# skim0119/gym-softrobot

Measured on AMD Instinct MI355X. Metric: env_steps_per_sec, higher is better.
Workload: dtype f64

## Files before the change

### gym_softrobot_amd/_capi.py

```python
from __future__ import annotations

import ctypes as C
import os
from pathlib import Path

ABI_VERSION = 17

FEAT_GRAVITY = 1 << 0
FEAT_POINT_FORCE_NODE0_X = 1 << 1
FEAT_PENDULUM_BC = 1 << 2
FEAT_ANALYTICAL_DAMPER = 1 << 3
FEAT_FIXED_BC = 1 << 4
FEAT_TIP_FORCE = 1 << 5
FEAT_MOVING_BASE_BC = 1 << 6
FEAT_LAPLACE_FILTER = 1 << 7
FEAT_PLANE_CONTACT_ANISO = 1 << 8
FEAT_REST_KAPPA_ACTION = 1 << 9
FEAT_OCTO_HEAD = 1 << 10
FEAT_SPLINE_MUSCLE_TORQUES = 1 << 11
FEAT_SUCKER_CONSTRAINT = 1 << 12
FEAT_COOMM_MUSCLES = 1 << 13
MAX_SUCKERS = 4
MAX_MUSCLES = 4
MUSCLE_LONGITUDINAL = 0
# ... 886 lines not shown
            raise ValueError(f"{what}: {name} must hold integers, got dtype {a.dtype}")
        if a.ndim > 1:
            raise ValueError(f"{what}: {name} must be a scalar or one-dimensional, got shape {a.shape}")
        if a.size and (a.min() < -2**31 or a.max() >= 2**31):
            raise ValueError(f"{what}: {name} does not fit an int32")
        out.append(a.astype(np.int32))
    s, d = out
    if d.ndim == 0:
        d = d.reshape(1)
    if s.ndim == 0:
        s = np.full(d.shape, s, np.int32)
    if s.shape != d.shape:
        raise ValueError(f"{what}: {names[0]} has {s.size} entries, {names[1]} has {d.size}")
    return np.ascontiguousarray(s), np.ascontiguousarray(d)


_VP = C.c_void_p
_EXPORTS = {
    "softrod_abi_version": (C.c_int, []),
    "softrod_source_hash": (C.c_char_p, []),
    "softrod_action_dim": (C.c_int, [C.c_int]),
    "softrod_obs_dim": (C.c_int, [C.c_int]),
    "softrod_aux_dim": (C.c_int, [C.c_int]),
    "softrod_config_softpendulum": (C.c_int, [C.POINTER(SoftrodConfig), C.c_int]),
    "softrod_config_softpendulum3d": (C.c_int, [C.POINTER(SoftrodConfig), C.c_int]),
    "softrod_config_arm_single": (C.c_int, [C.POINTER(SoftrodConfig), C.c_int]),
    "softrod_config_octo_flat": (C.c_int, [C.POINTER(SoftrodConfig), C.c_int]),
    "softrod_config_soft_arm": (C.c_int, [C.POINTER(SoftrodConfig), C.c_int]),
    "softrod_config_arm_push": (C.c_int, [C.POINTER(SoftrodConfig), C.c_int, C.c_int]),
    "softrod_config_arm_pull_weight": (C.c_int, [C.POINTER(SoftrodConfig), C.c_int]),
    "softrod_config_muscle_octopus": (C.c_int, [C.POINTER(SoftrodConfig), C.c_int, C.c_int]),
    "softrod_set_muscle_layers": (C.c_int, [_VP, _VP, _VP]),
    "softrod_set_spline_table": (C.c_int, [_VP, _VP, _VP]),
    "softrod_config_action_dim": (C.c_int, [C.POINTER(SoftrodConfig)]),
    "softrod_config_obs_dim": (C.c_int, [C.POINTER(SoftrodConfig)]),
    "softrod_reset_octo": (C.c_int, [_VP, _VP, _VP, _VP, _VP, _VP]),
    "softrod_autoreset_enable": (C.c_int, [_VP, C.c_int]),
    "softrod_autoreset_same_step": (C.c_int, [_VP, C.c_int]),
    "softrod_final_view": (C.c_int, [_VP, C.POINTER(C.c_void_p), C.POINTER(C.c_void_p), C.POINTER(C.c_void_p)]),
    "softrod_queue_push": (C.c_int, [_VP, _VP, _VP, C.c_int, _VP]),
    "softrod_queue_push_straight": (C.c_int, [_VP, _VP, _VP, _VP, _VP, C.c_int, _VP]),
    "softrod_queue_push_octo": (C.c_int, [_VP, _VP, _VP, _VP, _VP, C.c_int, _VP]),
    "softrod_queue_status": (C.c_int, [_VP, _VP, _VP, _VP]),
    "softrod_queue_status_begin": (C.c_int, [_VP, _VP]),
    "softrod_queue_status_poll": (C.c_int, [_VP, C.c_int, _VP, _VP]),
    "softrod_queue_advance": (C.c_int, [_VP, _VP, _VP]),
    "softrod_set_action_basis": (C.c_int, [_VP, _VP]),
    "softrod_set_radius_profile": (C.c_int, [_VP, _VP]),
    "softrod_create": (C.c_int, [C.POINTER(SoftrodConfig), C.c_int, C.POINTER(C.c_void_p)]),
    "softrod_reset": (C.c_int, [_VP, _VP, _VP, _VP]),
    "softrod_reset_straight": (C.c_int, [_VP, _VP, _VP, _VP, _VP, _VP]),
    "softrod_step": (C.c_int, [_VP, _VP, _VP, _VP, _VP, _VP, _VP, _VP]),
    "softrod_step_packed": (C.c_int, [_VP, _VP, _VP, _VP, _VP]),
    "softrod_scatter_rows": (C.c_int, [_VP, _VP, _VP, C.c_int, C.c_int, C.c_int64, C.c_int64, C.c_uint32, _VP]),
    "softrod_exchange_alloc": (C.c_int, [C.c_int, C.c_uint64, C.POINTER(C.c_void_p), _VP, C.POINTER(C.c_int)]),
    "softrod_exchange_open": (C.c_int, [C.c_int, _VP, C.c_int, C.POINTER(C.c_void_p)]),
    "softrod_exchange_close": (C.c_int, [C.c_int, _VP]),
    "softrod_exchange_free": (C.c_int, [C.c_int, _VP]),
    "softrod_observe": (C.c_int, [_VP, _VP, _VP, _VP]),
    "softrod_rod_energies": (C.c_int, [_VP, _VP, _VP]),
    "softrod_ground_reaction": (C.c_int, [_VP, _VP, _VP]),
    "softrod_rod_strains": (C.c_int, [_VP, _VP, _VP]),
    "softrod_muscle_loads": (C.c_int, [_VP, _VP, _VP]),
    "softrod_joint_loads": (C.c_int, [_VP, _VP, _VP]),
    "softrod_rod_dynamics": (C.c_int, [_VP, _VP, _VP]),
    "softrod_set_env_material": (C.c_int, [_VP, _VP, _VP, _VP]),
    "softrod_set_env_contact": (C.c_int, [_VP, _VP, _VP, _VP]),
    "softrod_copy_envs": (C.c_int, [_VP, _VP, _VP, C.c_int, _VP]),
    "softrod_bank_create": (C.c_int, [_VP, C.c_int]),
    "softrod_bank_save": (C.c_int, [_VP, _VP, _VP, C.c_int, _VP]),
    "softrod_bank_load": (C.c_int, [_VP, _VP, _VP, C.c_int, _VP]),
    "softrod_bank_info": (C.c_int, [_VP, C.POINTER(C.c_int32), C.POINTER(C.c_uint64), _VP]),
    "softrod_camera_default": (C.c_int, [C.POINTER(SoftrodConfig), C.POINTER(SoftrodCamera)]),
    "softrod_camera_check": (C.c_int, [C.POINTER(SoftrodCamera)]),
    "softrod_render": (C.c_int, [_VP, C.POINTER(SoftrodCamera), _VP, _VP, _VP]),
    "softrod_rod_clearance": (C.c_int, [_VP, C.c_int, _VP, _VP]),
    "softrod_set_rod_shape": (C.c_int, [_VP, _VP, _VP, _VP, _VP, _VP, _VP]),
    "softrod_set_reset_shapes": (C.c_int, [_VP, C.c_int, _VP, _VP, _VP, _VP, C.c_uint64, _VP]),
    "softrod_apply_reset_shapes": (C.c_int, [_VP, _VP, _VP]),
    "softrod_reset_shapes_view": (C.c_int, [_VP, C.POINTER(C.c_void_p), C.POINTER(C.c_void_p)]),
    "softrod_reset_shape_index": (C.c_uint32, [C.c_uint64, C.c_uint32, C.c_uint32, C.c_uint32]),
    "softrod_substeps": (C.c_int, [_VP, _VP, C.c_int, _VP]),
    "softrod_state_view_get": (C.c_int, [_VP, C.POINTER(SoftrodStateView)]),
    "softrod_set_timing": (C.c_int, [_VP, C.c_int]),
    "softrod_kernel_times_ms": (C.c_int, [_VP, _VP, C.c_int, C.POINTER(C.c_int)]),
    "softrod_last_kernel_ms": (C.c_int, [_VP, C.POINTER(C.c_float)]),
    "softrod_kernel_tier": (C.c_char_p, [_VP]),
    "softrod_last_error": (C.c_char_p, [_VP]),
    "softrod_destroy": (C.c_int, [_VP]),
}

EXPORTED_SYMBOLS = tuple(_EXPORTS)

_lib = None


def library_path() -> Path:
    env = os.environ.get("SOFTROD_HIP_LIB")
    if env:
        return Path(env)
    return Path(__file__).resolve().parent / "csrc" / "libsoftrod_hip.so"


def load_library() -> C.CDLL:
    global _lib
    if _lib is not None:
        return _lib
    try:
        import torch
    except ImportError:
        pass
    path = library_path()
    if not path.exists():
        raise SoftrodError(
            f"{path} not found: build it with `python __graft_entry__.py build` "
            "(hipcc --offload-arch=gfx950).  There is no CPU fallback."
        )
    lib = C.CDLL(str(path))
    for name, (restype, argtypes) in _EXPORTS.items():
        fn = getattr(lib, name)
        fn.restype = restype
        fn.argtypes = argtypes
    if lib.softrod_abi_version() != ABI_VERSION:
        raise SoftrodError("libsoftrod_hip.so ABI version mismatch")
    _lib = lib
    return lib


def library_source_hash() -> str:
    return load_library().softrod_source_hash().decode()


def source_hash() -> str:
    import hashlib

    csrc = Path(__file__).resolve().parent / "csrc"
    files = sorted(csrc.glob("*.hpp"), key=lambda f: f.name) + [csrc / "softrod_capi.hip",
                                                                 csrc.parents[1] / "include" / "softrod.h"]
    h = hashlib.sha256()
    for f in files:
        h.update(f.read_bytes())
    return h.hexdigest()[:16]


def check(rc: int, handle=None) -> None:
    if rc == 0:
        return
    msg = ""
    if _lib is not None:
        raw = _lib.softrod_last_error(handle)
        msg = raw.decode() if raw else ""
    raise SoftrodError(f"softrod call failed with code {rc}: {msg}")
```

### gym_softrobot_amd/backend.py

```python
from __future__ import annotations

import ctypes as C
from typing import Dict, Optional, Tuple

import numpy as np
import torch

from . import _capi
from ._capi import LANE_STRIDE, SoftrodConfig, SoftrodStateView, check, load_library
from .diagnostics import (JointLoads, MuscleLoads, RodClearance, RodDynamics, RodStrains, joint_loads_views,
                          muscle_loads_views, rod_clearance_views, rod_dynamics_views, rod_strains_views)


class _DevArray:

    def __init__(self, ptr: int, shape, typestr: str, owner):
        self._owner = owner
        self.__cuda_array_interface__ = {
            "shape": tuple(shape),
            "typestr": typestr,
            "data": (int(ptr), False),
            "version": 2,
            "strides": None,
        }


def _set_env_table(self, name: str, width: int, values, mask) -> None:
    why = getattr(_capi, f"env_{name}_refusal")(self.cfg, tapered="radius_profile" in self._tables)
    if why is not None:
        raise NotImplementedError(why)
    v = np.ascontiguousarray(values, dtype=np.float64).reshape(self.n_envs, width)
    k = None if mask is None else np.ascontiguousarray(mask, dtype=np.uint8).reshape(self.n_envs)
    check(getattr(self._lib, f"softrod_set_env_{name}")(self._h, v.ctypes.data, None if k is None else k.ctypes.data,
                                                        self._stream()), self._h)
    cur = _env_table(self, name)
    setattr(self, f"_env_{name}", np.where(k[:, None] != 0, v, cur) if k is not None else v.copy())

def _env_table(self, name: str) -> np.ndarray:
    cur = getattr(self, f"_env_{name}", None)
    if cur is None:
        return np.tile(getattr(_capi, f"env_{name}_defaults")(self.cfg), (self.n_envs, 1))
    return cur.copy()


class HipRodBackend:

    def __init__(self, cfg: SoftrodConfig, device: int = 0):
        if not torch.cuda.is_available():
            raise _capi.SoftrodError(
                "HipRodBackend needs a ROCm device (torch.cuda.is_available() is False); "
                "the hot path has no CPU fallback"
            )
        self._lib = load_library()
        self.cfg = cfg.copy()
        self.n_envs = int(cfg.n_envs)
        self.action_dim = _capi.config_action_dim(cfg)
        self.obs_dim = _capi.config_obs_dim(cfg)
        self.is_octo = bool(cfg.features & _capi.FEAT_OCTO_HEAD) and int(cfg.env_kind) == _capi.ENV_OCTO_FLAT
        self.is_mocto = int(cfg.env_kind) in _capi.MUSCLE_OCTOPUS_ENVS
        self.aux_dim = _capi.aux_dim(cfg.env_kind)
        self.device_index = int(device)
        self.device = torch.device("cuda", self.device_index)
        self._h = C.c_void_p()
        self._tables: Dict[str, bytes] = {}
        self._readouts: Dict[str, torch.Tensor] = {}
        self._frames: Dict[tuple, torch.Tensor] = {}
        check(self._lib.softrod_create(C.byref(self.cfg), self.device_index, C.byref(self._h)))
        if self.cfg.features & _capi.FEAT_REST_KAPPA_ACTION:
            if self.is_octo:
                basis = _capi.octo_action_basis(int(cfg.n_elem), int(cfg.n_knots))
            else:
                basis = _capi.action_basis(int(cfg.n_elem), self.action_dim)
            check(self._lib.softrod_set_action_basis(self._h, basis.ctypes.data), self._h)
            self._tables["action_basis"] = basis.tobytes()
        if int(cfg.env_kind) == _capi.ENV_ARM_TWO:
            basis, _ = _capi.arm_two_activation_basis(int(cfg.n_elem), 3)
            check(self._lib.softrod_set_action_basis(self._h, basis.ctypes.data), self._h)
            self._tables["action_basis"] = basis.tobytes()
        if self.cfg.features & _capi.FEAT_SPLINE_MUSCLE_TORQUES:
            breaks, coef = _capi.spline_table(float(cfg.base_length), int(cfg.n_ctrl))
            if len(breaks) != int(cfg.n_spline_pieces) + 1:
                raise _capi.SoftrodError("n_spline_pieces does not match the interpolant")
            check(self._lib.softrod_set_spline_table(self._h, breaks.ctypes.data, coef.ctypes.data), self._h)
            self._tables["spline_table"] = breaks.tobytes() + coef.tobytes()
# ... 352 lines not shown
            z = self._frames.get(key + ("depth",))
            if z is None:
                z = self._frames[key + ("depth",)] = torch.empty((self.n_envs, h, w), dtype=torch.float32, device=self.device)
        check(self._lib.softrod_render(self._h, C.byref(camera), rgb.data_ptr(), z.data_ptr() if depth else None,
                                       self._stream()), self._h)
        return (rgb, z) if depth else rgb

    def time_limit(self) -> torch.Tensor:
        return self.state()["env_aux"][0] != 0.0

    def step_packed(self, actions, out: Optional[torch.Tensor] = None) -> torch.Tensor:
        from .distributed import packed_width

        a = self._actions(actions)
        if out is None:
            if getattr(self, "packed", None) is None:
                self.packed = torch.empty((self.n_envs, packed_width(self.obs_dim)), dtype=torch.float32,
                                          device=self.device)
            out = self.packed
        check(
            self._lib.softrod_step_packed(
                self._h, a.data_ptr(), out.data_ptr(),
                self.aux.data_ptr() if self.aux is not None else None, self._stream(),
            ),
            self._h,
        )
        return out

    def scatter_rows(self, packed: torch.Tensor, peer_ptrs, first_row: int, tag_word: int = -1, tag: int = 0) -> None:
        tab = np.ascontiguousarray(peer_ptrs, dtype=np.uint64)
        check(
            self._lib.softrod_scatter_rows(
                self._h, packed.data_ptr(), tab.ctypes.data, int(tab.size), int(packed.shape[1]), int(first_row),
                int(tag_word), int(tag) & 0xFFFFFFFF, self._stream(),
            ),
            self._h,
        )

    def exchange_alloc(self, n_words: int):
        ptr, kind = C.c_void_p(), C.c_int()
        handle = (C.c_uint8 * 64)()
        check(self._lib.softrod_exchange_alloc(self.device_index, int(n_words) * 4, C.byref(ptr), handle, C.byref(kind)))
        t = torch.as_tensor(_DevArray(ptr.value, (int(n_words),), "<f4", self), device=self.device)
        return t, int(ptr.value), bytes(handle), {1: "uncached", 2: "fine-grained"}[int(kind.value)]

    def exchange_open(self, handle: bytes, owner_device: int) -> int:
        ptr = C.c_void_p()
        buf = (C.c_uint8 * 64).from_buffer_copy(handle)
        check(self._lib.softrod_exchange_open(self.device_index, buf, int(owner_device), C.byref(ptr)))
        return int(ptr.value)

    def exchange_close(self, ptr: int) -> None:
        check(self._lib.softrod_exchange_close(self.device_index, C.c_void_p(ptr)))

    def exchange_free(self, ptr: int) -> None:
        check(self._lib.softrod_exchange_free(self.device_index, C.c_void_p(ptr)))

    def substeps(self, actions, n: int) -> None:
        a = self._actions(actions) if actions is not None else None
        check(
            self._lib.softrod_substeps(
                self._h, a.data_ptr() if a is not None else None, int(n), self._stream()
            ),
            self._h,
        )

    def set_timing(self, n_launches: int) -> None:
        check(self._lib.softrod_set_timing(self._h, int(n_launches)), self._h)

    def kernel_times_ms(self) -> np.ndarray:
        cap = 1 << 16
        out = np.zeros(cap, np.float32)
        cnt = C.c_int()
        check(self._lib.softrod_kernel_times_ms(self._h, out.ctypes.data, cap, C.byref(cnt)), self._h)
        return out[: cnt.value].copy()

    def last_kernel_ms(self) -> float:
        ms = C.c_float()
        check(self._lib.softrod_last_kernel_ms(self._h, C.byref(ms)), self._h)
        return float(ms.value)

    def prev_action_rows(self) -> torch.Tensor:
        if getattr(self, "_prev_rows", None) is None:
            self._prev_rows = self.state()["prev_action"]
            if not self.is_octo and not self.is_mocto:
                self._prev_rows = self._prev_rows[:, : self.action_dim]
        return self._prev_rows

    def state(self) -> Dict[str, torch.Tensor]:
        v = SoftrodStateView()
        check(self._lib.softrod_state_view_get(self._h, C.byref(v)), self._h)
        n, s = self.n_envs, int(v.lane_stride)

        def view(ptr, comps):
            return torch.as_tensor(_DevArray(ptr, (comps, n, s), "<f8", self), device=self.device)

        extra = {}
        ns = n * (int(self.cfg.n_arm) if self.is_mocto else 1)
        if v.env_aux:
            extra["env_aux"] = torch.as_tensor(_DevArray(v.env_aux, (8, n), "<f8", self), device=self.device)
        if v.prev_kappa:
            extra["prev_kappa"] = torch.as_tensor(
                _DevArray(v.prev_kappa, (n, int(self.cfg.n_arm) * (int(self.cfg.n_elem) - 1)), "<f4", self), device=self.device)
        if v.muscle_activation:
            extra["muscle_activation"] = torch.as_tensor(
                _DevArray(v.muscle_activation, (_capi.MAX_MUSCLES, n, s), "<f8", self), device=self.device)
        return {
            **extra,
            "sucker_index": torch.as_tensor(_DevArray(v.sucker_index, (_capi.MAX_SUCKERS, ns), "<i4", self),
                                            device=self.device),
            "position": view(v.position, 3),
            "velocity": view(v.velocity, 3),
            "director": view(v.director, 9),
            "omega": view(v.omega, 3),
            "tangents": view(v.tangents, 3),
            "time": torch.as_tensor(_DevArray(v.time, (n,), "<f8", self), device=self.device),
            "control": torch.as_tensor(_DevArray(v.control, (4, n), "<f8", self), device=self.device),
            "kappa": view(v.kappa, 3),
            "rest_kappa": view(v.rest_kappa, 3),
            "env_memory": torch.as_tensor(_DevArray(v.env_memory, (n, s), "<f8", self), device=self.device),
            "prev_action": torch.as_tensor(_DevArray(v.prev_action, (n, max(7, self.action_dim)), "<f4", self),
                                           device=self.device),
            "head": torch.as_tensor(_DevArray(v.head, (20, n), "<f8", self), device=self.device),
            "bc_targets": torch.as_tensor(_DevArray(v.bc_targets, (12, n), "<f8", self), device=self.device),
            "sucker_ratio": torch.as_tensor(_DevArray(v.sucker_ratio, (_capi.MAX_SUCKERS, ns), "<f8", self),
                                            device=self.device),
            "arm_stride": int(v.arm_stride),
        }

    _SNAPSHOT_KEYS = ("position", "velocity", "director", "omega", "tangents", "time", "control", "kappa",
                      "rest_kappa", "env_memory", "prev_action", "head", "bc_targets", "sucker_ratio", "sucker_index")

    def _snapshot_keys(self):
        return (self._SNAPSHOT_KEYS + (("muscle_activation",) if self.cfg.features & _capi.FEAT_COOMM_MUSCLES else ())
                + (("env_aux", "prev_kappa") if self.is_mocto else ()))

    def config_fingerprint(self) -> bytes:
        import hashlib

        c = self.cfg.copy()
        c.n_envs = 0
        d = hashlib.sha256()
        for k in sorted(self._tables):
            d.update(k.encode() + b"\0" + self._tables[k])
        return bytes([_capi.ABI_VERSION]) + bytes(memoryview(c).cast("B")) + d.digest()

    def snapshot(self) -> Dict[str, torch.Tensor]:
        if getattr(self, "queue_depth", 0):
            raise _capi.SoftrodError("snapshot/restore of a handle with device-side auto-reset is not supported: "
                                     "the pending-reset flags and the staged queue are not part of the state view")
        st = self.state()
        torch.cuda.synchronize(self.device)
        snap = {k: st[k].cpu().clone() for k in self._snapshot_keys()}
        if getattr(self, "_env_material", None) is not None:
            snap["env_material"] = torch.from_numpy(self._env_material.copy())
        if getattr(self, "_env_contact", None) is not None:
            snap["env_contact"] = torch.from_numpy(self._env_contact.copy())
        if self.reset_shapes_count:
            snap["reset_shape_index"] = self.reset_shape_index.cpu().clone()
            snap["reset_shape_episode"] = self.reset_shape_episode.cpu().clone()
        snap["config_fingerprint"] = torch.frombuffer(bytearray(self.config_fingerprint()), dtype=torch.uint8).clone()
        return snap

    def restore(self, snap: Dict[str, torch.Tensor]) -> None:
        if getattr(self, "queue_depth", 0):
            raise _capi.SoftrodError("snapshot/restore of a handle with device-side auto-reset is not supported: "
                                     "stale needs_reset / skip flags would reset or skip the wrong envs")
        fp = snap.get("config_fingerprint")
        if fp is None or bytes(fp.numpy().tobytes()) != self.config_fingerprint():
            raise ValueError("snapshot was taken under a different softrod_config / ABI version / table set "
                             "(dt, n_substeps, features, env_kind, material, radius profile, spline table, "
                             "action basis ...): refusing to load it")
        st = self.state()
        for k in self._snapshot_keys():
            if tuple(snap[k].shape) != tuple(st[k].shape):
                raise ValueError(f"snapshot field {k!r} has shape {tuple(snap[k].shape)}, expected {tuple(st[k].shape)}")
            st[k].copy_(snap[k].to(self.device))
        if "env_material" in snap:
            self.set_env_material(snap["env_material"].numpy())
        elif getattr(self, "_env_material", None) is not None:
            self.set_env_material(np.tile(_capi.env_material_defaults(self.cfg), (self.n_envs, 1)))
        if self.reset_shapes_count and "reset_shape_index" in snap:
            self.reset_shape_index.copy_(snap["reset_shape_index"].to(self.device))
            self.reset_shape_episode.copy_(snap["reset_shape_episode"].to(self.device))
        if "env_contact" in snap:
            self.set_env_contact(snap["env_contact"].numpy())
        elif getattr(self, "_env_contact", None) is not None:
            self.set_env_contact(np.tile(_capi.env_contact_defaults(self.cfg), (self.n_envs, 1)))
        torch.cuda.synchronize(self.device)

    def rod_snapshot(self, env_indices) -> Dict[str, np.ndarray]:
        st = self.state()
        idx = torch.as_tensor(list(env_indices), dtype=torch.long, device=self.device)
        ne = int(self.cfg.n_elem)

        def rows(name, width):
            return st[name].index_select(1, idx)[:, :, :width].permute(1, 0, 2).cpu().numpy()

        return {
            "x": rows("position", ne + 1), "v": rows("velocity", ne + 1), "w": rows("omega", ne),
            "Q": rows("director", ne).reshape(len(env_indices), 3, 3, ne),
            "time": st["time"].index_select(0, idx).cpu().numpy(),
        }

    def kernel_tier(self) -> str:
        return self._lib.softrod_kernel_tier(self._h).decode()

    def octo_state_numpy(self) -> Dict[str, np.ndarray]:
        st = self.state()
        ne, na, seg = int(self.cfg.n_elem), int(self.cfg.n_arm), int(st["arm_stride"])
        torch.cuda.synchronize(self.device)

        def arms(t, comps, width):
            a = t[:, :, : na * seg].reshape(comps, self.n_envs, na, seg)[..., :width]
            return a.permute(1, 2, 0, 3).cpu().numpy()

        hd = st["head"].cpu().numpy()
        return {
            "x": arms(st["position"], 3, ne + 1),
            "v": arms(st["velocity"], 3, ne + 1),
            "w": arms(st["omega"], 3, ne),
            "Q": arms(st["director"], 9, ne).reshape(self.n_envs, na, 3, 3, ne),
            "kappa": arms(st["kappa"], 3, ne - 1),
            "rest_kappa": arms(st["rest_kappa"], 3, ne - 1),
            "head_x": hd[0:3].T.copy(), "head_v": hd[3:6].T.copy(),
            "head_Q": hd[6:15].T.reshape(self.n_envs, 3, 3).copy(), "head_w": hd[15:18].T.copy(),
            "target": hd[18:20].T.copy(),
            "time": st["time"].cpu().numpy(),
        }

    def state_numpy(self) -> Dict[str, np.ndarray]:
        st = self.state()
        ne = int(self.cfg.n_elem)
        torch.cuda.synchronize(self.device)
        out = {
            "x": st["position"][:, :, : ne + 1].permute(1, 0, 2).cpu().numpy(),
            "v": st["velocity"][:, :, : ne + 1].permute(1, 0, 2).cpu().numpy(),
            "w": st["omega"][:, :, :ne].permute(1, 0, 2).cpu().numpy(),
            "tangents": st["tangents"][:, :, :ne].permute(1, 0, 2).cpu().numpy(),
            "time": st["time"].cpu().numpy(),
            "control": st["control"].permute(1, 0).cpu().numpy(),
            "kappa": st["kappa"][:, :, : ne - 1].permute(1, 0, 2).cpu().numpy(),
            "rest_kappa": st["rest_kappa"][:, :, : ne - 1].permute(1, 0, 2).cpu().numpy(),
        }
        q = st["director"][:, :, :ne].permute(1, 0, 2).cpu().numpy()
        out["Q"] = q.reshape(self.n_envs, 3, 3, ne)
        return out
```

### gym_softrobot_amd/csrc/softrod_capi.hip

```cpp
#include <hip/hip_runtime.h>
#include <hip/hip_ext.h>

#include <cmath>
#include <cstdio>
#include <cstdlib>
#include <cstring>
#include <new>
#include <string>
#include <vector>

#include "softrod_kernels.hpp"
#include "softrod_dynamics_readout.hpp"
#include "softrod_copy_envs.hpp"
#include "softrod_state_bank.hpp"
#include "softrod_shape.hpp"
#include "softrod_reset_shapes.hpp"

using namespace softrod;

template <class Row>
struct EnvTable {
    Row* dev = nullptr;
    Row* host = nullptr;
    hipEvent_t ev = nullptr;
// ... 17 lines not shown
    hipEvent_t ev_pairs = nullptr;
    unsigned char* twin_of(const void* base) const {
        for (const Twin& t : twins) if (t.of == base) return t.dev;
        return nullptr;
    }
    void release() {
        for (const Twin& t : twins) (void)hipFree(t.dev);
        (void)hipFree(d_pairs);
        if (h_pairs) (void)hipHostFree(h_pairs);
        if (ev_pairs) (void)hipEventDestroy(ev_pairs);
        *this = StateBank{};
    }
};

struct softrod_handle {
    softrod_config cfg;
    int device = 0;
    int epl = 1;
    int nw = 1;
    size_t init_stride = 18;
    int window_refresh = 0;
    bool window_paired = true;
    std::string tier;
    RodParams P{};
    StatePtrs S{};
    std::vector<void*> owned;
    double* d_init = nullptr;
    uint8_t* d_mask = nullptr;
    double* d_basis = nullptr;
    double* d_spline = nullptr;
    bool spline_set = false;
    RodParams* d_params = nullptr;
    StatePtrs* d_state = nullptr;
    double* d_time_tab = nullptr;
    double* d_mat = nullptr;
    double* d_render_radius = nullptr;
    double* d_mtab = nullptr;
    bool muscles_set = false;
    unsigned* d_ticket = nullptr;
    bool tapered = false;
    bool was_reset = false;
    bool basis_set = false;
    double* h_init = nullptr;
    uint8_t* h_mask = nullptr;
    std::vector<hipEvent_t> ev_start, ev_stop;
    int timed = 0;
    hipEvent_t ev_reset = nullptr;
    int q_depth = 0;
    double* d_queue = nullptr;
    double* h_queue = nullptr;
    int* d_consumed = nullptr;
    int* d_produced = nullptr;
    int* d_underflow = nullptr;
    uint8_t* d_flags = nullptr;
    int* h_produced = nullptr;
    std::vector<int> seen_consumed;
    std::vector<int2> pending;
    double* h_stage = nullptr;
    int2* h_where = nullptr;
    double* d_stage = nullptr;
    int2* d_where = nullptr;
    size_t stage_cap = 0;
    int* h_status = nullptr;
    hipEvent_t ev_status = nullptr;
    bool status_pending = false;
    hipEvent_t ev_queue = nullptr;
    bool same_step = false;
    float* d_final_obs = nullptr;
    double* d_final_time = nullptr;
    double* d_final_aux = nullptr;
    int rs_count = 0;
    unsigned long long rs_seed = 0;
    double* d_rs_field[4] = {nullptr, nullptr, nullptr, nullptr};
    int* d_rs_index = nullptr;
    int* d_rs_episode = nullptr;
    uint8_t* d_rs_picked = nullptr;
    EnvTable<EnvMaterial> env_mat;
    EnvTable<EnvContact> env_contact;
    int2* d_pairs = nullptr;
    int2* h_pairs = nullptr;
    hipEvent_t ev_pairs = nullptr;
    std::vector<uint8_t> is_dst;
    StateBank bank;
    std::string err;
};

namespace {

thread_local std::string g_err;

int fail(softrod_handle* h, int code, const std::string& msg) {
    if (h) h->err = msg; else g_err = msg;
    return code;
}

struct DeviceGuard {
    int prev = -1, want = -1;
    hipError_t err = hipSuccess;
    explicit DeviceGuard(int device) : want(device) {
        err = hipGetDevice(&prev);
        if (err == hipSuccess && prev != want) err = hipSetDevice(want);
    }
    ~DeviceGuard() {
        if (prev >= 0 && prev != want) (void)hipSetDevice(prev);
    }
    DeviceGuard(const DeviceGuard&) = delete;
    DeviceGuard& operator=(const DeviceGuard&) = delete;
};
#define SR_ON_DEVICE(h)                                                                  \
    DeviceGuard guard_((h)->device);                                                     \
    if (guard_.err != hipSuccess)                                                        \
        return fail(h, SOFTROD_EHIP, std::string("hipSetDevice: ") + hipGetErrorString(guard_.err))

#define SR_HIP(h, call)                                                                 \
    do {                                                                                \
        hipError_t e_ = (call);                                                         \
        if (e_ != hipSuccess)                                                           \
            return fail(h, SOFTROD_EHIP, std::string(#call) + ": " + hipGetErrorString(e_)); \
    } while (0)

void fill_params(const softrod_config& c, RodParams& P) {
    std::memset(&P, 0, sizeof(P));
    P.n_envs = c.n_envs;
    P.n_elem = c.n_elem;
    P.time_two_half_adds = c.time_two_half_adds;
    P.features = c.features;
    P.env_kind = c.env_kind;
    P.filter_order = c.filter_order;
    P.damp_before_constrain = c.damp_before_constrain;
    P.dt = c.dt;
    P.half_dt = 0.5 * c.dt;
    P.final_time = c.final_time;
    const int n = c.n_elem;
    const double rest_len = c.base_length / (double)n;
    P.rest_len = rest_len;
    P.inv_rest_len = 1.0 / rest_len;
    P.rest_vor = 0.5 * (rest_len + rest_len);
    P.inv_rest_vor = 1.0 / P.rest_vor;
    const double r = c.base_radius;
    const double A0 = M_PI * r * r;
    const double I1 = A0 * A0 / (4.0 * M_PI);
    const double I[3] = {I1, I1, 2.0 * I1};
    for (int i = 0; i < 3; ++i) {
        P.J[i] = I[i] * (c.density * rest_len);
        P.invJ[i] = 1.0 / P.J[i];
    }
    P.shear[0] = c.alpha_c * c.shear_modulus * A0;
    P.shear[1] = c.alpha_c * c.shear_modulus * A0;
    P.shear[2] = c.youngs_modulus * A0;
    P.bend[0] = c.youngs_modulus * I[0];
    P.bend[1] = c.youngs_modulus * I[1];
    P.bend[2] = c.shear_modulus * I[2];
    const double volume = M_PI * (r * r) * rest_len;
    P.mass_node = c.density * volume;
    for (int i = 0; i < 3; ++i) { P.gravity[i] = c.gravity[i]; P.tip_force[i] = c.tip_force[i]; }
    const double ddt = c.damper_time_step > 0.0 ? c.damper_time_step : c.dt;
    P.damp_t = std::exp(-c.damping_constant * ddt);
    const double me = P.mass_node;
    for (int i = 0; i < 3; ++i) {
        P.damp_logr[i] = c.damper_protocol == 1 ? -c.damping_constant * ddt : -c.damping_constant * ddt * me * P.invJ[i];
        P.damp_r[i] = std::exp(P.damp_logr[i]);
    }
    P.eps_length = c.eps_length;
    P.eps_rot_axis = c.eps_rot_axis;
    P.acos_shift = c.acos_shift;
    P.eps_sin = c.eps_sin;
// ... 36 lines not shown
        P.n_action = c.n_knots;
        if (c.env_kind == SOFTROD_ENV_ARM_PULL_WEIGHT) P.seg_shift = 6, P.seg = 64;
        P.head_fixed = c.head_fixed;
        const double hl = c.head_length > 0.0 ? c.head_length : 2.0 * c.base_radius, hr = c.head_radius;
        for (int i = 0; i < 3; ++i) P.head_center[i] = c.head_length > 0.0 ? c.head_center[i] : 0.0;
        P.joint_angle0 = c.head_length > 0.0 ? c.joint_angle0 : 0.0;
        P.joint_angle_step = c.head_length > 0.0 ? c.joint_angle_step : 360 / (double)c.n_arm;
        const double harea = M_PI * hr * hr;
        P.head_mass = (M_PI * hr * hr * hl) * c.head_density;
        const double s1 = harea * harea / (4.0 * M_PI);
        const double smoa[3] = {s1, s1, 2.0 * s1};
        for (int i = 0; i < 3; ++i) {
            P.head_invJ[i] = 1.0 / (smoa[i] * c.head_density * hl);
        }
        P.head_radius = hr;
        P.joint_k = c.joint_k;
        P.joint_nu = c.joint_nu;
        P.joint_kt = c.joint_kt;
    }
    P.n_ctrl = c.n_ctrl;
    P.n_pieces = c.n_spline_pieces;
    P.muscle_scale = c.muscle_torque_scale;
    P.max_rate = c.max_activation_rate;
    P.base_length = c.base_length;
    for (int i = 0; i < 3; ++i) P.arm_target[i] = c.arm_target[i];
    P.n_suckers = c.n_suckers;
    for (int j = 0; j < SOFTROD_MAX_SUCKERS; ++j) P.sucker_index[j] = c.sucker_index[j];
    if (c.early_termination) P.features |= kFeatEarlyTerm;
    P.sucker_ratio0 = c.sucker_reduction_ratio;
    P.n_muscles = (c.features & SOFTROD_FEAT_COOMM_MUSCLES) ? c.n_muscles : 0;
    for (int m = 0; m < SOFTROD_MAX_MUSCLES; ++m) P.muscle_kind[m] = c.muscle_kind[m];
    P.fl_degree = c.muscle_fl_degree;
    for (int k = 0; k < SOFTROD_MAX_FL_COEF; ++k) P.fl_coef[k] = c.muscle_fl_coef[k];
    P.muscle_form = c.muscle_equiv_load_form;
    P.muscle_cur_radius = c.muscle_position_current_radius;
    P.muscle_tm_law = c.muscle_tm_length_law;
    P.push_mode = c.arm_push_mode;
}

bool is_octo(const softrod_handle* h) { return (h->cfg.features & SOFTROD_FEAT_OCTO_HEAD) != 0; }
bool is_flat(const softrod_handle* h) { return h->cfg.env_kind == SOFTROD_ENV_OCTO_FLAT; }
bool is_pull(const softrod_handle* h) { return h->cfg.env_kind == SOFTROD_ENV_ARM_PULL_WEIGHT; }
bool mocto_kind(int e) { return e == SOFTROD_ENV_CRAWL || e == SOFTROD_ENV_ARM_TWO || e == SOFTROD_ENV_REACH; }
bool is_mocto(const softrod_handle* h) { return mocto_kind(h->cfg.env_kind); }
bool restarts_as_body(const softrod_handle* h) { return is_octo(h); }
bool observes_as_body(const softrod_handle* h) { return is_mocto(h) || (is_octo(h) && !is_pull(h)); }
template <class K> K by_epl(const softrod_handle* h, K one, K two) { return h->epl == 2 ? two : one; }
template <class T>
hipError_t alloc_owned(softrod_handle* h, T*& p, size_t bytes) {
    const hipError_t e = hipMalloc((void**)&p, bytes);
    if (e != hipSuccess) { p = nullptr; return e; }
    h->owned.push_back(p);
    return hipMemset(p, 0, bytes);
}
struct RodLayout { int rods, lane_stride, arm_stride; };
RodLayout rod_layout(const softrod_handle* h) {
    const bool arms = is_flat(h) || is_mocto(h);
    return {arms ? h->cfg.n_arm : 1, kLanes * h->epl * h->nw, arms ? h->P.seg : 0};
}
void env_material_row(const softrod_config& c, const double m[4], EnvMaterial& R) {
    softrod_config ci = c;
    ci.youngs_modulus = m[0];
    ci.shear_modulus = m[1];
    ci.density = m[2];
    ci.damping_constant = m[3];
    RodParams Q;
    fill_params(ci, Q);
    std::memset(&R, 0, sizeof(R));
    for (int i = 0; i < 3; ++i) {
        R.J[i] = Q.J[i]; R.invJ[i] = Q.invJ[i]; R.shear[i] = Q.shear[i]; R.bend[i] = Q.bend[i];
        R.damp_r[i] = Q.damp_r[i]; R.damp_logr[i] = Q.damp_logr[i];
    }
    R.mass_node = Q.mass_node; R.mass_total = Q.mass_total; R.damp_t = Q.damp_t;
}
void env_contact_row(const double c[8], EnvContact& R) {
    std::memset(&R, 0, sizeof(R));
    R.k = c[0];
    R.nu = c[1];
    for (int i = 0; i < 3; ++i) { R.kin_mu[i] = c[2 + i]; R.stat_mu[i] = c[5 + i]; }
    R.kin_am[0] = 0.5 * (R.kin_mu[0] + R.kin_mu[1]); R.kin_am[1] = 0.5 * (R.kin_mu[0] - R.kin_mu[1]);
    R.stat_am[0] = 0.5 * (R.stat_mu[0] + R.stat_mu[1]); R.stat_am[1] = 0.5 * (R.stat_mu[0] - R.stat_mu[1]);
}

int launch_autoreset(softrod_handle* h, float* obs, double* reward, uint8_t* term, uint8_t* trunc, double* aux, int pack,
                     hipStream_t st) {
    const dim3 grid((unsigned)h->cfg.n_envs), block(kLanes * h->nw);
    if (restarts_as_body(h))
        hipLaunchKernelGGL(softrod_octo_autoreset_kernel, grid, block, 0, st, h->P, h->S, obs, reward, term, trunc, pack);
    else
        hipLaunchKernelGGL(by_epl(h, softrod_autoreset_kernel<1>, softrod_autoreset_kernel<2>), grid, block, 0, st, h->P, h->S,
                           obs, reward, term, trunc, aux, pack);
    SR_HIP(h, hipGetLastError());
    return SOFTROD_OK;
}

int launch_autoreset_same_step(softrod_handle* h, float* obs, double* aux, int pack, hipStream_t st) {
    const dim3 grid((unsigned)h->cfg.n_envs), block(kLanes * h->nw);
    if (restarts_as_body(h))
        hipLaunchKernelGGL(softrod_octo_autoreset_same_step_kernel, grid, block, 0, st, h->P, h->S, obs, pack, h->d_final_obs,
                           h->d_final_time);
    else
        hipLaunchKernelGGL(by_epl(h, softrod_autoreset_same_step_kernel<1>, softrod_autoreset_same_step_kernel<2>), grid, block,
                           0, st, h->P, h->S, obs, aux, pack, h->d_final_obs, h->d_final_time, h->d_final_aux);
    SR_HIP(h, hipGetLastError());
    return SOFTROD_OK;
}

int launch_reset_shapes(softrod_handle* h, int mode, const uint8_t* mask, float* obs, const uint8_t* term, const uint8_t* trunc,
                        double* aux, int pack, hipStream_t st) {
    const int N = h->cfg.n_envs;
    ResetShapesPick pick{};
    pick.index = h->d_rs_index; pick.episode = h->d_rs_episode; pick.picked = h->d_rs_picked;
    pick.seed = h->rs_seed; pick.count = h->rs_count; pick.mode = mode; pick.mask = mask;
    pick.terminated = pack ? nullptr : term; pick.truncated = pack ? nullptr : trunc;
    pick.packed = (mode == kPickFinished && pack) ? obs : nullptr;
    pick.od = softrod_config_obs_dim(&h->cfg);
    hipLaunchKernelGGL(softrod_reset_shapes_pick_kernel, dim3((unsigned)((N + kPickThreads - 1) / kPickThreads)), dim3(kPickThreads),
                       0, st, h->P, h->S, pick);
    const RodLayout y = rod_layout(h);
    const RodShapeArgs args{h->d_rs_field[0], h->d_rs_field[1], h->d_rs_field[2], h->d_rs_field[3], h->d_rs_picked, h->d_rs_index};
    hipLaunchKernelGGL(by_epl(h, softrod_rod_shape_kernel<1>, softrod_rod_shape_kernel<2>), dim3((unsigned)(N * y.rods)),
                       dim3(kLanes), 0, st, h->P, h->S, y.rods, y.lane_stride, y.arm_stride, args);
    if (obs) {
        if (observes_as_body(h))
            hipLaunchKernelGGL(softrod_reset_shapes_octo_observe_kernel, dim3((unsigned)N), dim3(kLanes * h->nw), 0, st, h->P, h->S,
                               h->d_rs_picked, obs, pack);
        else
            hipLaunchKernelGGL(by_epl(h, softrod_observe_kernel<1>, softrod_observe_kernel<2>), dim3((unsigned)N), dim3(kLanes), 0,
                               st, h->P, h->S, h->d_rs_picked, nullptr, obs, aux, pack);
    }
    SR_HIP(h, hipGetLastError());
    return SOFTROD_OK;
}

enum : unsigned { kOptMuscles = SOFTROD_FEAT_COOMM_MUSCLES, kOptEarlyTerm = kFeatEarlyTerm, kOptEnvMaterial = kFeatEnvMaterial,
                  kOptEnvContact = kFeatEnvContact, kOptCompiledFor = kOptEarlyTerm | kOptEnvMaterial | kOptEnvContact };
constexpr int kAny = -1, kMoctoEnvs = -2;
constexpr unsigned kAnyFeatures = kRuntimeFeatures;
using StepKernel = void (*)(RodParams, StatePtrs, const float*, float*, double*, uint8_t*, uint8_t*, double*, int, int, int);
using OctoKernel = void (*)(RodParams, StatePtrs, const float*, float*, double*, uint8_t*, uint8_t*, int, int, int);
using WindowKernel = void (*)(RodParams, StatePtrs, const float*, int, int);

struct StepRow {
    unsigned feats;
    int env;
    int math, epl;
    int taper, zup;
    int nw_min, nw_max;
    bool windowed;
    unsigned needs, honours;
    StepKernel step; OctoKernel octo; WindowKernel window;
    int epb, waves;
    const char* label;
};

constexpr StepRow compiled_row(unsigned F, int env, int epl, int taper, int nw_min, int nw_max, const char* label) {
    const bool rt = F == kRuntimeFeatures;
    StepRow r{};
    r.feats = rt ? kAnyFeatures : F & ~(kFeatPlaneZup | kOptCompiledFor);
    r.env = env; r.math = SOFTROD_MATH_FAST; r.epl = epl; r.taper = taper; r.nw_min = nw_min; r.nw_max = nw_max;
    r.zup = rt ? kAny : (F & kFeatPlaneZup) != 0;
    r.needs = rt ? 0u : F & kOptCompiledFor;
    r.honours = rt ? 0u : F & (kOptCompiledFor | kOptMuscles);
    r.epb = 1; r.label = label;
    return r;
}
template <unsigned F, int E, int EPL, bool TAPER = false>
constexpr StepRow fast_row(const char* label) {
    StepRow r = compiled_row(F, E, EPL, TAPER, 1, 1, label);
    r.step = softrod_step_fast_kernel<F, E, EPL, TAPER>;
    return r;
}
template <unsigned F, int MAXW, int EPB>
constexpr StepRow octo_row(int env, int nw_min, int nw_max, const char* label) {
    StepRow r = compiled_row(F, env, 1, kAny, nw_min, nw_max, label);
    r.octo = softrod_octo_step_kernel<F, MAXW, EPB>;
    r.epb = EPB; r.waves = EPB == 1 ? 0 : MAXW * EPB;
    return r;
}
template <unsigned F, int RPB>
constexpr StepRow window_row(const char* label) {
    StepRow r = compiled_row(F, SOFTROD_ENV_ARM_SINGLE, 2, 0, 1, 1, label);
    r.window = softrod_step_window_kernel<F, RPB>;
    r.windowed = true; r.epb = RPB; r.waves = 2 * RPB;
    return r;
}
template <bool ET>
constexpr StepRow libm_row(unsigned feats, int env, int zup, int taper, unsigned honours) {
    StepRow r{};
    r.feats = feats; r.env = env; r.math = SOFTROD_MATH_LIBM; r.epl = 1; r.taper = taper; r.zup = zup;
    r.nw_min = r.nw_max = r.epb = 1;
    r.needs = ET ? kOptEarlyTerm : 0u; r.honours = r.needs | kOptMuscles | honours;
    r.step = softrod_step_libm_kernel<ET>;
    r.label = "softrod_step_libm_kernel";
    return r;
}

constexpr unsigned kArmSingleZup = SOFTROD_FEATURES_ARM_SINGLE | kFeatPlaneZup, kOctoFlatZup = SOFTROD_FEATURES_OCTO_FLAT | kFeatPlaneZup;
const StepRow kStepRows[] = {
    octo_row<SOFTROD_FEATURES_ARM_PULL_WEIGHT | kFeatEarlyTerm, 2, 1>(SOFTROD_ENV_ARM_PULL_WEIGHT, 1, 1, "softrod_octo_step_kernel<ArmPullWeight,1 wave,1 env/wg,taper>"),
    octo_row<SOFTROD_FEATURES_ARM_PULL_WEIGHT, 2, 1>(SOFTROD_ENV_ARM_PULL_WEIGHT, 1, 1, "softrod_octo_step_kernel<ArmPullWeight,1 wave,1 env/wg,taper>"),
    octo_row<SOFTROD_FEATURES_ARM_PULL_WEIGHT, 4, 1>(kMoctoEnvs, 1, 4, "softrod_mocto_action_kernel | softrod_octo_step_kernel<muscle arms,"
                                                                       "{waves},1 env/wg,taper> | softrod_mocto_epilogue_kernel"),
    octo_row<kOctoFlatZup | kFeatEnvContact, 2, 4>(SOFTROD_ENV_OCTO_FLAT, 2, 2, "softrod_octo_step_kernel<zup,2 waves,4 envs/wg>"),
    octo_row<kOctoFlatZup | kFeatEnvContact, 2, 1>(SOFTROD_ENV_OCTO_FLAT, 1, 1, "softrod_octo_step_kernel<zup,2 waves max,1 env/wg>"),
    octo_row<kOctoFlatZup, 2, 4>(SOFTROD_ENV_OCTO_FLAT, 2, 2, "softrod_octo_step_kernel<zup,2 waves,4 envs/wg>"),
    octo_row<kOctoFlatZup, 2, 1>(SOFTROD_ENV_OCTO_FLAT, 1, 1, "softrod_octo_step_kernel<zup,2 waves max,1 env/wg>"),
    octo_row<kOctoFlatZup, 8, 1>(SOFTROD_ENV_OCTO_FLAT, 3, 8, "softrod_octo_step_kernel<zup,8 waves max,1 env/wg>"),
    octo_row<SOFTROD_FEATURES_OCTO_FLAT, 2, 1>(SOFTROD_ENV_OCTO_FLAT, 1, 2, "softrod_octo_step_kernel<general plane,2 waves max,1 env/wg>"),
    octo_row<SOFTROD_FEATURES_OCTO_FLAT, 8, 1>(SOFTROD_ENV_OCTO_FLAT, 3, 8, "softrod_octo_step_kernel<general plane,8 waves max,1 env/wg>"),
    window_row<kArmSingleZup, 4>("softrod_step_window_kernel<ArmSingle,4 rods/wg> refresh={refresh}"),
    window_row<kArmSingleZup, 1>("softrod_step_window_kernel<ArmSingle,1 rod/wg,s_barrier> refresh={refresh}"),
    fast_row<kArmSingleZup, SOFTROD_ENV_ARM_SINGLE, 2>("softrod_step_fast_kernel<ArmSingle,epl=2>"),
    fast_row<SOFTROD_FEATURES_ARM_PUSH | kFeatEarlyTerm, SOFTROD_ENV_ARM_PUSH, 2, true>("softrod_step_fast_kernel<ArmPush,epl=2,taper>"),
    fast_row<SOFTROD_FEATURES_ARM_PUSH, SOFTROD_ENV_ARM_PUSH, 2, true>("softrod_step_fast_kernel<ArmPush,epl=2,taper>"),
    fast_row<kArmSingleZup, SOFTROD_ENV_ARM_SINGLE, 1, true>("softrod_step_fast_kernel<ArmSingle,epl=1,taper>"),
    fast_row<kFeaturesTaperedSuckerArm, SOFTROD_ENV_NONE, 1, true>("softrod_step_fast_kernel<damped sucker arm,epl=1,taper>"),
    fast_row<SOFTROD_FEATURES_ARM_PUSH | kFeatEarlyTerm, SOFTROD_ENV_ARM_PUSH, 1, true>("softrod_step_fast_kernel<ArmPush,epl=1,taper>"),
    fast_row<SOFTROD_FEATURES_ARM_PUSH, SOFTROD_ENV_ARM_PUSH, 1, true>("softrod_step_fast_kernel<ArmPush,epl=1,taper>"),
    fast_row<kRuntimeFeatures, kRuntimeEnv, 1, true>("softrod_step_fast_kernel<runtime mask,epl=1,taper>"),
    fast_row<SOFTROD_FEATURES_SOFTPENDULUM, SOFTROD_ENV_SOFTPENDULUM, 2>("softrod_step_fast_kernel<SoftPendulum,epl=2>"),
    fast_row<SOFTROD_FEATURES_SOFTPENDULUM3D, SOFTROD_ENV_SOFTPENDULUM3D, 2>("softrod_step_fast_kernel<SoftPendulum3D,epl=2>"),
    fast_row<SOFTROD_FEATURES_SOFT_ARM, SOFTROD_ENV_SOFT_ARM, 2>("softrod_step_fast_kernel<SoftArm,epl=2>"),
    fast_row<kFeaturesMuscleRod, SOFTROD_ENV_NONE, 1>("softrod_step_fast_kernel<muscle rod,epl=1>"),
    fast_row<kRuntimeFeatures, kRuntimeEnv, 2>("softrod_step_fast_kernel<runtime mask,epl=2>"),
    fast_row<kArmSingleZup | kFeatEnvContact | kFeatEnvMaterial, SOFTROD_ENV_ARM_SINGLE, 1>("softrod_step_fast_kernel<ArmSingle,epl=1>"),
    fast_row<kArmSingleZup | kFeatEnvContact, SOFTROD_ENV_ARM_SINGLE, 1>("softrod_step_fast_kernel<ArmSingle,epl=1>"),
    fast_row<SOFTROD_FEATURES_SOFTPENDULUM | kFeatEnvMaterial, SOFTROD_ENV_SOFTPENDULUM, 1>("softrod_step_fast_kernel<SoftPendulum,epl=1>"),
    fast_row<SOFTROD_FEATURES_SOFTPENDULUM3D | kFeatEnvMaterial, SOFTROD_ENV_SOFTPENDULUM3D, 1>("softrod_step_fast_kernel<SoftPendulum3D,epl=1>"),
    fast_row<kArmSingleZup | kFeatEnvMaterial, SOFTROD_ENV_ARM_SINGLE, 1>("softrod_step_fast_kernel<ArmSingle,epl=1>"),
    fast_row<SOFTROD_FEATURES_SOFTPENDULUM, SOFTROD_ENV_SOFTPENDULUM, 1>("softrod_step_fast_kernel<SoftPendulum,epl=1>"),
    fast_row<SOFTROD_FEATURES_SOFTPENDULUM3D, SOFTROD_ENV_SOFTPENDULUM3D, 1>("softrod_step_fast_kernel<SoftPendulum3D,epl=1>"),
    fast_row<kArmSingleZup, SOFTROD_ENV_ARM_SINGLE, 1>("softrod_step_fast_kernel<ArmSingle,epl=1>"),
    fast_row<SOFTROD_FEATURES_SOFT_ARM, SOFTROD_ENV_SOFT_ARM, 1>("softrod_step_fast_kernel<SoftArm,epl=1>"),
    fast_row<kRuntimeFeatures, kRuntimeEnv, 1>("softrod_step_fast_kernel<runtime mask,epl=1>"),
    libm_row<true>(kAnyFeatures, kAny, kAny, kAny, 0u),
    libm_row<false>(SOFTROD_FEATURES_SOFTPENDULUM, SOFTROD_ENV_SOFTPENDULUM, kAny, 0, kOptEnvMaterial),
    libm_row<false>(SOFTROD_FEATURES_SOFTPENDULUM3D, SOFTROD_ENV_SOFTPENDULUM3D, kAny, 0, kOptEnvMaterial),
    libm_row<false>(SOFTROD_FEATURES_ARM_SINGLE, SOFTROD_ENV_ARM_SINGLE, 1, 0, kOptEnvMaterial | kOptEnvContact),
    libm_row<false>(kAnyFeatures, kAny, kAny, kAny, 0u),
};

unsigned active_options(const softrod_handle* h) {
    return (h->cfg.features & kOptMuscles) | (h->cfg.early_termination ? kOptEarlyTerm : 0u) |
           (h->env_mat.dev ? kOptEnvMaterial : 0u) | (h->env_contact.dev ? kOptEnvContact : 0u);
}

const char* material_why_not(const softrod_handle* h) {
    const unsigned f = h->cfg.features;
    const int e = h->cfg.env_kind;
    if (is_octo(h) || is_mocto(h)) return "per-env material: not for OctoFlat or the muscle octopus envs";
    if (f & SOFTROD_FEAT_COOMM_MUSCLES) return "per-env material: not for the muscle envs";
    if (e == SOFTROD_ENV_SOFT_ARM) return "per-env material: not for SoftArmTracking (its muscle torque scale depends on E)";
// ... 53 lines not shown
    const unsigned opts = active_options(h) | with;
    const int e = h->cfg.env_kind, zup = (h->P.features & kFeatPlaneZup) != 0;
    const bool windowed = h->window_refresh > 0 && epilogue;
    for (const StepRow& r : kStepRows)
        if (r.math == h->cfg.math_mode && (r.feats == kAnyFeatures || r.feats == h->cfg.features) &&
            (r.env == kAny || (r.env == kMoctoEnvs ? mocto_kind(e) : r.env == e)) && r.epl == h->epl &&
            (r.taper == kAny || r.taper == (int)h->tapered) && (r.zup == kAny || r.zup == zup) &&
            r.nw_min <= h->nw && h->nw <= r.nw_max && r.windowed == windowed &&
            (!r.window || r.epb == (h->window_paired ? 4 : 1)) && !(r.needs & ~opts) && !(opts & ~r.honours))
            return {&r, nullptr};
    const char* why = why_no_row(h, with);
    if (!why) why = why_no_row(h, opts);
    return {nullptr, why ? why : "no step kernel is compiled for this handle's feature set, env kind and options"};
}

template <class Row>
hipError_t bank_adopt_table(softrod_handle* h, const Row* table, const Row& row);

template <int W, class Row, class Bad, class Build>
int set_env_table(softrod_handle* h, EnvTable<Row>& T, const Row*& slot, unsigned option, const char* what,
                  const double* values, const double (&own)[W], const uint8_t* mask, void* stream, Bad bad, Build build) {
    const StepChoice serves = select_step(h, 1, option);
    if (!serves.row) return fail(h, SOFTROD_EINVAL, serves.why);
    const size_t N = (size_t)h->cfg.n_envs;
    for (size_t i = 0; i < N; ++i) {
        if (mask && !mask[i]) continue;
        if (const char* why = bad(values + W * i)) return fail(h, SOFTROD_EINVAL, what + std::to_string(i) + why);
    }
    SR_ON_DEVICE(h);
    hipStream_t st = (hipStream_t)stream;
    if (!T.dev) {
        SR_HIP(h, hipMalloc((void**)&T.dev, N * sizeof(Row)));
        SR_HIP(h, hipHostMalloc((void**)&T.host, N * sizeof(Row), hipHostMallocDefault));
        SR_HIP(h, hipEventCreateWithFlags(&T.ev, hipEventDisableTiming));
        Row R0;
        build(own, R0);
        for (size_t i = 0; i < N; ++i) T.host[i] = R0;
        if (const hipError_t e = bank_adopt_table(h, T.dev, R0)) {
            T.release();
            T = EnvTable<Row>{};
            return fail(h, SOFTROD_EHIP, std::string("state bank: ") + hipGetErrorString(e));
        }
        slot = T.dev;
        SR_HIP(h, hipMemcpy(h->d_state, &h->S, sizeof(StatePtrs), hipMemcpyHostToDevice));
    } else {
        SR_HIP(h, hipEventSynchronize(T.ev));
    }
    for (size_t i = 0; i < N; ++i)
        if (!mask || mask[i]) build(values + W * i, T.host[i]);
    SR_HIP(h, hipMemcpyAsync(T.dev, T.host, N * sizeof(Row), hipMemcpyHostToDevice, st));
    SR_HIP(h, hipEventRecord(T.ev, st));
    return SOFTROD_OK;
}

template <class K, class... A>
void launch_stamped(K kernel, const dim3& grid, const dim3& block, hipStream_t st, hipEvent_t t0, hipEvent_t t1, A... args) {
    if (t0 || t1) hipExtLaunchKernelGGL(kernel, grid, block, 0, st, t0, t1, 0, args...);
    else hipLaunchKernelGGL(kernel, grid, block, 0, st, args...);
}

int launch_step(softrod_handle* h, const float* actions, float* obs, double* reward,
                uint8_t* term, uint8_t* trunc, double* aux, int n_sub, int epilogue, int pack,
                hipStream_t st) {
    if (h->q_depth > 0 && epilogue && !h->same_step) {
        if (const int rc = launch_autoreset(h, obs, reward, term, trunc, aux, pack, st)) return rc;
        if (h->rs_count > 0)
            if (const int rc = launch_reset_shapes(h, kPickSkipped, nullptr, obs, term, trunc, aux, pack, st)) return rc;
    }
    if ((h->cfg.features & SOFTROD_FEAT_COOMM_MUSCLES) && h->cfg.math_mode == SOFTROD_MATH_FAST) {
        const bool push = h->cfg.env_kind == SOFTROD_ENV_ARM_PUSH || is_pull(h) || is_mocto(h);
        if (is_mocto(h) && (!h->tapered || !h->muscles_set || (h->cfg.env_kind == SOFTROD_ENV_ARM_TWO && !h->basis_set)))
            return fail(h, SOFTROD_EINVAL, "the muscle octopus needs softrod_set_radius_profile and softrod_set_muscle_layers "
                                           "(and SOFTROD_ENV_ARM_TWO softrod_set_action_basis) before it steps");
        if (push && !h->tapered)
            return fail(h, SOFTROD_EINVAL, "SOFTROD_ENV_ARM_PUSH (SOFTROD_MATH_FAST): call softrod_set_radius_profile first "
                                           "(the reference's arm is tapered, arm_push_env.py:160-179)");
        if (!push && h->tapered)
            return fail(h, SOFTROD_EINVAL, "a tapered muscle rod outside SOFTROD_ENV_ARM_PUSH runs under SOFTROD_MATH_LIBM only");
    }
    const StepChoice c = select_step(h, epilogue);
    if (!c.row) return fail(h, SOFTROD_EINVAL, c.why);
    const StepChoice after = c.row->windowed ? select_step(h, 0) : StepChoice{nullptr, nullptr};
    if (c.row->windowed && !after.row) return fail(h, SOFTROD_EINVAL, after.why);
    auto launch = [&](const StepRow& r, int n, int epi, hipEvent_t t0, hipEvent_t t1) {
        const dim3 grid((unsigned)((h->cfg.n_envs + r.epb - 1) / r.epb)), block(kLanes * (r.waves ? r.waves : h->nw));
        if (r.window) launch_stamped(r.window, grid, block, st, t0, t1, h->P, h->S, actions, n, h->window_refresh);
        else if (r.octo) launch_stamped(r.octo, grid, block, st, t0, t1, h->P, h->S, actions, obs, reward, term, trunc, n, epi, pack);
        else launch_stamped(r.step, grid, block, st, t0, t1, h->P, h->S, actions, obs, reward, term, trunc, aux, n, epi, pack);
    };
    const bool timing = h->timed < (int)h->ev_start.size();
    const hipEvent_t t0 = timing ? h->ev_start[h->timed] : nullptr, t1 = timing ? h->ev_stop[h->timed] : nullptr;
    const bool mocto = c.row->env == kMoctoEnvs;
    const bool action_first = mocto && epilogue && actions, epilogue_last = mocto && epilogue;
    const dim3 grid((unsigned)h->cfg.n_envs), block(kLanes * h->nw);
    if (action_first)
        launch_stamped(softrod_mocto_action_kernel, grid, block, st, t0, nullptr, h->P, h->S, actions, n_sub);
    launch(*c.row, n_sub, epilogue, action_first ? nullptr : t0, (after.row || epilogue_last) ? nullptr : t1);
    if (after.row) launch(*after.row, 0, 1, nullptr, epilogue_last ? nullptr : t1);
    if (epilogue_last)
        launch_stamped(softrod_mocto_epilogue_kernel, grid, block, st, nullptr, t1, h->P, h->S, obs, reward, term, trunc, 1, pack);
    SR_HIP(h, hipGetLastError());
    if (timing) ++h->timed;
    if (h->q_depth > 0 && epilogue && h->same_step) {
        if (const int rc = launch_autoreset_same_step(h, obs, aux, pack, st)) return rc;
        if (h->rs_count > 0)
            if (const int rc = launch_reset_shapes(h, kPickFinished, nullptr, obs, term, trunc, aux, pack, st)) return rc;
    }
    return SOFTROD_OK;
}

int upload_and_reset(softrod_handle* h, hipStream_t st, bool use_mask) {
    const size_t N = (size_t)h->cfg.n_envs;
    SR_HIP(h, hipMemcpyAsync(h->d_init, h->h_init, N * h->init_stride * sizeof(double), hipMemcpyHostToDevice, st));
    if (use_mask)
        SR_HIP(h, hipMemcpyAsync(h->d_mask, h->h_mask, N, hipMemcpyHostToDevice, st));
    ResetArgs A{h->d_init, use_mask ? h->d_mask : nullptr};
    if (is_octo(h)) {
        OctoResetArgs OA{h->d_init, h->d_init + N * (size_t)h->cfg.n_arm * 18, use_mask ? h->d_mask : nullptr};
        hipLaunchKernelGGL(softrod_octo_reset_kernel, dim3((unsigned)N), dim3(kLanes * h->nw), 0, st, h->P, h->S, OA);
    } else
        hipLaunchKernelGGL(by_epl(h, softrod_reset_kernel<1>, softrod_reset_kernel<2>), dim3((unsigned)N), dim3(kLanes), 0, st,
                           h->P, h->S, A);
    SR_HIP(h, hipGetLastError());
    SR_HIP(h, hipEventRecord(h->ev_reset, st));
    h->was_reset = true;
    return SOFTROD_OK;
}

void straight_init(const softrod_config& c, const double start[3], const double direction[3],
                   const double normal_in[3], double out[18]) {
    const int n = c.n_elem;
    double end[3], normal[3], t[3], d[3];
    for (int i = 0; i < 3; ++i) end[i] = start[i] + direction[i] * c.base_length;
    const double nn = std::sqrt(normal_in[0] * normal_in[0] + normal_in[1] * normal_in[1] +
                                normal_in[2] * normal_in[2]);
    for (int i = 0; i < 3; ++i) normal[i] = normal_in[i] / nn;
    for (int i = 0; i < 3; ++i) {
        out[i] = start[i];
        out[3 + i] = (end[i] - start[i]) / (double)n;
        out[6 + i] = end[i];
        d[i] = (start[i] + 1.0 * out[3 + i]) - start[i];
    }
    const double l = std::sqrt(d[0] * d[0] + d[1] * d[1] + d[2] * d[2]);
    for (int i = 0; i < 3; ++i) t[i] = d[i] / l;
    for (int i = 0; i < 3; ++i) out[9 + i] = normal[i];
    out[12] = t[1] * normal[2] - t[2] * normal[1];
    out[13] = t[2] * normal[0] - t[0] * normal[2];
    out[14] = t[0] * normal[1] - t[1] * normal[0];
    for (int i = 0; i < 3; ++i) out[15 + i] = t[i];
}

void theta_record(const softrod_handle* h, double th, double* frames) {
    const double start[3] = {0.0, 0.0, 0.0};
    const double direction[3] = {1.0 * std::cos(th), 1.0 * std::sin(th), 0.0};
    const double normal[3] = {1.0 * std::sin(th), -1.0 * std::cos(th), 0.0};
    straight_init(h->cfg, start, direction, normal, frames);
}
void straight_record(const softrod_handle* h, const double* start, const double* direction, const double* normal,
                     double* frames, double* tgt) {
    straight_init(h->cfg, start, direction, normal, frames);
    if (is_pull(h)) { tgt[0] = 0.0; tgt[1] = 0.0; }
}
size_t octo_target_dim(const softrod_handle* h) { return is_mocto(h) ? 4 : 2; }
void octo_record(const softrod_handle* h, const double* arm_start, const double* arm_direction, const double* target,
                 double* frames, double* tgt) {
    const double normal[3] = {0.0, 0.0, 1.0};
    for (int a = 0; a < h->cfg.n_arm; ++a)
        straight_init(h->cfg, arm_start + 3 * a, arm_direction + 3 * a, normal, frames + (size_t)a * 18);
    for (size_t i = 0; i < octo_target_dim(h); ++i) tgt[i] = target[i];
}

void config_common(softrod_config* cfg, int n_envs) {
    std::memset(cfg, 0, sizeof(*cfg));
    cfg->struct_size = (uint32_t)sizeof(softrod_config);
    cfg->n_envs = n_envs;
    cfg->n_elem = 50;
    cfg->dt = 1.0e-4;
    cfg->n_substeps = (int)(1.0 / (25 * cfg->dt));
    cfg->math_mode = SOFTROD_MATH_FAST;
    cfg->final_time = 5.0;
    cfg->alpha_c = 27.0 / 28.0;
    cfg->eps_length = 1e-14;
    cfg->eps_rot_axis = 1e-14;
    cfg->acos_shift = 1e-10;
    cfg->eps_sin = 1e-14;
    cfg->time_two_half_adds = 1;
    cfg->damp_before_constrain = 0;
}

const char* config_why_not(const softrod_config& c) {
    if (c.n_envs < 1 || c.n_elem < 2 || c.n_elem > 2 * kLanes - 2)
        return "need n_envs >= 1 and 2 <= n_elem <= 126";
    if (c.n_elem > kLanes - 1 && c.math_mode != SOFTROD_MATH_FAST)
        return "rods longer than 63 elements (two per lane) exist for SOFTROD_MATH_FAST only";
    if (c.n_substeps < 0 || !(c.dt > 0.0))
// ... 105 lines not shown
    std::vector<double> tab(1024);
    double t = 0.0;
    const double half = 0.5 * c.dt;
    for (double& at : tab) {
        at = t;
        for (int s = 0; s < c.n_substeps; ++s) {
            if (c.time_two_half_adds) { t = t + half; t = t + half; }
            else t = t + c.dt;
        }
    }
    return tab;
}

void shape_handle(softrod_handle* h) {
    const softrod_config* cfg = &h->cfg;
    h->epl = cfg->n_elem > kLanes - 1 ? 2 : 1;
    fill_params(h->cfg, h->P);
    if (is_octo(h)) {
        h->nw = (cfg->n_arm * h->P.seg + kLanes - 1) / kLanes;
        h->init_stride = (size_t)cfg->n_arm * 18 + (is_mocto(h) ? 4 : 2);
    }
    const char* dbg = std::getenv("SOFTROD_DEBUG_SWITCHES");
    const bool debug_switches = dbg && dbg[0] == '1';
    auto debug_env = [&](const char* name) -> const char* { return debug_switches ? std::getenv(name) : nullptr; };
    if (const char* one = debug_env("SOFTROD_WINDOW_PAIRED"))
        h->window_paired = one[0] != '0';
    {
        const int halo = kLanes - (cfg->n_elem + 2) / 2;
        const char* off = debug_env("SOFTROD_NO_WINDOW");
        if (h->epl == 2 && cfg->features == SOFTROD_FEATURES_ARM_SINGLE && cfg->env_kind == SOFTROD_ENV_ARM_SINGLE &&
            cfg->math_mode == SOFTROD_MATH_FAST && (h->P.features & kFeatPlaneZup) && !(off && off[0] == '1') &&
            halo >= 3 * kWindowRho)
            h->window_refresh = halo / kWindowRho;
        if (const char* r = debug_env("SOFTROD_WINDOW_REFRESH")) if (h->window_refresh > 0) h->window_refresh = std::atoi(r);
    }
}


std::string copy_envs_why_not(softrod_handle* h, const int32_t* src, const int32_t* dst, int count) {
    const int N = h->cfg.n_envs;
    if (h->q_depth > 0)
        return "copy envs: not on a handle with device-side auto-reset (the pending-reset flags and the staged queue "
               "belong to each env's RNG future)";
    if (count < 0 || count > N) return "copy envs: count " + std::to_string(count) + " is outside 0 .. n_envs = " + std::to_string(N);
    if (count > 0 && (!src || !dst)) return "copy envs: null src or dst";
    for (int i = 0; i < count; ++i)
        for (const int e : {src[i], dst[i]})
            if (e < 0 || e >= N)
                return "copy envs: env index " + std::to_string(e) + " (pair " + std::to_string(i) + ") is outside 0 .. " + std::to_string(N - 1);
    std::string why;
    for (int i = 0; i < count && why.empty(); ++i) {
        if (h->is_dst[dst[i]]) why = "copy envs: env " + std::to_string(dst[i]) + " appears twice in dst";
        h->is_dst[dst[i]] = 1;
    }
    for (int i = 0; i < count && why.empty(); ++i)
        if (src[i] != dst[i] && h->is_dst[src[i]])
            why = "copy envs: env " + std::to_string(src[i]) + " is the dst of one pair and the src of another";
    for (int i = 0; i < count; ++i) h->is_dst[dst[i]] = 0;
    return why;
}

CopyTable copy_table(const softrod_handle* h) {
    CopyTable T{};
    T.n_envs = h->cfg.n_envs;
    auto add = [&T](const void* p, size_t comps, size_t row_bytes) {
        if (p) T.a[T.n++] = CopyArray{(unsigned char*)const_cast<void*>(p), (unsigned)comps, (unsigned)row_bytes};
    };
    const StatePtrs& S = h->S;
    const softrod_config& c = h->cfg;
    const size_t W = (size_t)rod_layout(h).lane_stride * sizeof(double);
    const size_t adim = (size_t)softrod_config_action_dim(&c);
    const size_t per = is_mocto(h) ? (size_t)c.n_arm : 1;
    add(S.pos, 3, W); add(S.vel, 3, W); add(S.dir, 9, W); add(S.omg, 3, W); add(S.tan, 3, W);
    add(S.kap, 3, W); add(S.rkap, 3, W); add(S.envmem, 1, W); add(S.mact, SOFTROD_MAX_MUSCLES, W);
    add(S.time, 1, sizeof(double)); add(S.ctrl, 4, sizeof(double)); add(S.head, 20, sizeof(double));
    add(S.bc, 12, sizeof(double)); add(S.aux, 8, sizeof(double));
    add(S.prev_action, 1, (adim > 7 ? adim : 7) * sizeof(float));
    add(S.prev_kappa, 1, (size_t)c.n_arm * (size_t)(c.n_elem - 1) * sizeof(float));
    add(S.sucker, SOFTROD_MAX_SUCKERS, per * sizeof(double));
    add(S.sucker_idx, SOFTROD_MAX_SUCKERS, per * sizeof(int));
    add(h->env_mat.dev, 1, sizeof(EnvMaterial));
    add(h->env_contact.dev, 1, sizeof(EnvContact));
    add(h->d_rs_index, 1, sizeof(int)); add(h->d_rs_episode, 1, sizeof(int));
    static_assert(kCopyMaxArrays >= 22, "copy_table adds up to 22 arrays");
    return T;
}

template <class Row>
hipError_t copy_table_rows(EnvTable<Row>& T, const int2* pairs, int n) {
    if (!T.dev) return hipSuccess;
    const hipError_t e = hipEventSynchronize(T.ev);
    if (e != hipSuccess) return e;
    for (int i = 0; i < n; ++i) T.host[pairs[i].y] = T.host[pairs[i].x];
    return hipSuccess;
}

bool bank_table(const StateBank& bank, const CopyTable& batch, CopyTable& out) {
    out = batch;
    out.n_envs = bank.slots;
    for (int k = 0; k < batch.n; ++k)
        if (!(out.a[k].base = bank.twin_of(batch.a[k].base))) return false;
    return true;
}

hipError_t bank_adopt(const softrod_handle* h, StateBank& bank) {
    const CopyTable T = copy_table(h);
    const size_t had = bank.twins.size();
    hipError_t e = hipSuccess;
    for (int k = 0; k < T.n && e == hipSuccess; ++k) {
        if (bank.twin_of(T.a[k].base)) continue;
        const size_t bytes = (size_t)T.a[k].comps * (size_t)bank.slots * (size_t)T.a[k].row_bytes;
        unsigned char* p = nullptr;
        e = hipMalloc((void**)&p, bytes);
        if (e == hipSuccess) {
            bank.twins.push_back({T.a[k].base, p});
            e = hipMemset(p, 0, bytes);
        }
    }
    if (e != hipSuccess) {
        for (size_t i = had; i < bank.twins.size(); ++i) (void)hipFree(bank.twins[i].dev);
        bank.twins.resize(had);
    }
    return e;
}

std::vector<EnvMaterial>& bank_host_rows(StateBank& b, const EnvMaterial*) { return b.mat; }
std::vector<EnvContact>& bank_host_rows(StateBank& b, const EnvContact*) { return b.contact; }

template <class Row>
hipError_t bank_adopt_table(softrod_handle* h, const Row* table, const Row& row) {
    StateBank& bank = h->bank;
    if (!bank.slots) return hipSuccess;
    hipError_t e = bank_adopt(h, bank);
    if (e != hipSuccess) return e;
    std::vector<Row>& rows = bank_host_rows(bank, table);
    rows.assign((size_t)bank.slots, row);
    return hipMemcpy(bank.twin_of(table), rows.data(), rows.size() * sizeof(Row), hipMemcpyHostToDevice);
}

template <class Row>
hipError_t bank_table_rows(StateBank& bank, EnvTable<Row>& T, const int2* pairs, int n, bool load) {
    if (!T.dev) return hipSuccess;
    std::vector<Row>& rows = bank_host_rows(bank, T.dev);
    if (!load) {
        for (int i = 0; i < n; ++i) rows[pairs[i].y] = T.host[pairs[i].x];
        return hipSuccess;
    }
    const hipError_t e = hipEventSynchronize(T.ev);
    if (e != hipSuccess) return e;
    for (int i = 0; i < n; ++i) T.host[pairs[i].y] = rows[pairs[i].x];
    return hipSuccess;
}

std::string bank_why_not(softrod_handle* h, const int32_t* envs, const int32_t* slots, int count, bool load) {
    const std::string what = load ? "bank load: " : "bank save: ";
    StateBank& bank = h->bank;
    const int N = h->cfg.n_envs, K = bank.slots;
    if (!K) return what + "the handle has no state bank (softrod_bank_create)";
    if (h->q_depth > 0)
        return what + "not on a handle with device-side auto-reset (the pending-reset flags and the staged queue "
                      "belong to each env's RNG future)";
    const int limit = load ? N : K;
    if (count < 0 || count > limit)
        return what + "count " + std::to_string(count) + " is outside 0 .. " + (load ? "n_envs = " : "slots = ") + std::to_string(limit);
    if (count > 0 && (!envs || !slots)) return what + "null envs or slots";
    for (int i = 0; i < count; ++i) {
        if (envs[i] < 0 || envs[i] >= N)
            return what + "env index " + std::to_string(envs[i]) + " (pair " + std::to_string(i) + ") is outside 0 .. " + std::to_string(N - 1);
        if (slots[i] < 0 || slots[i] >= K)
            return what + "slot index " + std::to_string(slots[i]) + " (pair " + std::to_string(i) + ") is outside 0 .. " + std::to_string(K - 1);
    }
    if (load)
        for (int i = 0; i < count; ++i)
            if (!bank.filled[slots[i]]) return what + "slot " + std::to_string(slots[i]) + " holds no state";
    const int32_t* written = load ? envs : slots;
    std::string why;
    for (int i = 0; i < count && why.empty(); ++i) {
        if (bank.seen[written[i]])
            why = what + (load ? "env " : "slot ") + std::to_string(written[i]) + " appears twice";
        bank.seen[written[i]] = 1;
    }
    for (int i = 0; i < count; ++i) bank.seen[written[i]] = 0;
    return why;
}

int bank_copy(softrod_handle* h, const int32_t* envs, const int32_t* slots, int count, bool load, void* stream) {
    const std::string why = bank_why_not(h, envs, slots, count, load);
    if (!why.empty()) return fail(h, SOFTROD_EINVAL, why);
    if (count == 0) return SOFTROD_OK;
    StateBank& bank = h->bank;
    CopyTable batch = copy_table(h), twin;
    if (!bank_table(bank, batch, twin))
        return fail(h, SOFTROD_EINVAL, std::string(load ? "bank load" : "bank save") + ": a per-env array of the handle has no twin in the bank");
    SR_ON_DEVICE(h);
    hipStream_t st = (hipStream_t)stream;
    SR_HIP(h, hipEventSynchronize(bank.ev_pairs));
    for (int i = 0; i < count; ++i) bank.h_pairs[i] = load ? make_int2(slots[i], envs[i]) : make_int2(envs[i], slots[i]);
    SR_HIP(h, bank_table_rows(bank, h->env_mat, bank.h_pairs, count, load));
    SR_HIP(h, bank_table_rows(bank, h->env_contact, bank.h_pairs, count, load));
    SR_HIP(h, hipMemcpyAsync(bank.d_pairs, bank.h_pairs, (size_t)count * sizeof(int2), hipMemcpyHostToDevice, st));
    SR_HIP(h, hipEventRecord(bank.ev_pairs, st));
    hipLaunchKernelGGL(softrod_bank_copy_kernel, dim3((unsigned)count), dim3(kCopyThreads), 0, st,
                       load ? twin : batch, load ? batch : twin, bank.d_pairs);
    SR_HIP(h, hipGetLastError());
    if (!load)
        for (int i = 0; i < count; ++i) bank.filled[slots[i]] = 1;
    return SOFTROD_OK;
}
}

extern "C" {

int softrod_abi_version(void) { return SOFTROD_ABI_VERSION; }

#ifndef SOFTROD_SOURCE_HASH
#define SOFTROD_SOURCE_HASH "unhashed"
#endif
const char* softrod_source_hash(void) { return SOFTROD_SOURCE_HASH; }

int softrod_action_dim(int env_kind) {
    return env_kind == SOFTROD_ENV_SOFTPENDULUM3D ? 2 : env_kind == SOFTROD_ENV_ARM_SINGLE ? 7
         : env_kind == SOFTROD_ENV_OCTO_FLAT ? 24 : env_kind == SOFTROD_ENV_SOFT_ARM ? 8
         : (env_kind == SOFTROD_ENV_ARM_PUSH || env_kind == SOFTROD_ENV_ARM_PULL_WEIGHT) ? 2
         : env_kind == SOFTROD_ENV_CRAWL ? 24 : env_kind == SOFTROD_ENV_ARM_TWO ? 18 : env_kind == SOFTROD_ENV_REACH ? 480 : 1;
}
int softrod_obs_dim(int env_kind) {
    return env_kind == SOFTROD_ENV_SOFTPENDULUM3D ? 9 : env_kind == SOFTROD_ENV_ARM_SINGLE ? 25
         : env_kind == SOFTROD_ENV_OCTO_FLAT ? 8 * 56 + 13 : env_kind == SOFTROD_ENV_SOFT_ARM ? 14
         : (env_kind == SOFTROD_ENV_ARM_PUSH || env_kind == SOFTROD_ENV_ARM_PULL_WEIGHT) ? 84
         : env_kind == SOFTROD_ENV_CRAWL ? 8 * 131 : env_kind == SOFTROD_ENV_ARM_TWO ? 2 * 52 : env_kind == SOFTROD_ENV_REACH ? 8 * 189 : 4;
}
int softrod_config_action_dim(const softrod_config* cfg) {
    if (!cfg) return 0;
    if (cfg->env_kind == SOFTROD_ENV_SOFT_ARM) return 2 * cfg->n_ctrl;
    if (cfg->env_kind == SOFTROD_ENV_ARM_PUSH || cfg->env_kind == SOFTROD_ENV_ARM_PULL_WEIGHT)
        return cfg->arm_push_mode == 0 ? 1 : 2;
    if (mocto_kind(cfg->env_kind)) return cfg->n_arm * cfg->n_knots;
    return cfg->env_kind == SOFTROD_ENV_OCTO_FLAT ? cfg->n_arm * cfg->n_knots : softrod_action_dim(cfg->env_kind);
}
int softrod_config_obs_dim(const softrod_config* cfg) {
    if (!cfg) return 0;
    if (cfg->env_kind == SOFTROD_ENV_SOFT_ARM) return 2 * cfg->n_ctrl + 6;
    if (cfg->env_kind == SOFTROD_ENV_ARM_PUSH || cfg->env_kind == SOFTROD_ENV_ARM_PULL_WEIGHT)
        return 2 * (cfg->n_elem + 1) + 2;
    if (mocto_kind(cfg->env_kind)) {
        const int n = cfg->n_elem, na = cfg->n_arm, nk = cfg->n_knots;
        if (cfg->env_kind == SOFTROD_ENV_ARM_TWO) return na * ((n - 1) * 2 + nk + na + 3);
        return na * ((n - 1) + (n + 1) * 4 + nk + na + (cfg->env_kind == SOFTROD_ENV_CRAWL ? 17 : 18));
    }
    if (cfg->env_kind != SOFTROD_ENV_OCTO_FLAT) return softrod_obs_dim(cfg->env_kind);
    return cfg->n_arm * ((cfg->n_elem - 1) + 4 * (cfg->n_elem + 1) + cfg->n_knots) + 13;
}
int softrod_aux_dim(int env_kind) { return env_kind == SOFTROD_ENV_SOFTPENDULUM3D ? 1 : 0; }

int softrod_config_softpendulum(softrod_config* cfg, int n_envs) {
    if (!cfg || n_envs < 1) return SOFTROD_EINVAL;
    config_common(cfg, n_envs);
    cfg->features = SOFTROD_FEATURES_SOFTPENDULUM;
    cfg->env_kind = SOFTROD_ENV_SOFTPENDULUM;
    cfg->base_length = 1.0;
    cfg->base_radius = 0.05;
    cfg->density = 1000.0;
    cfg->youngs_modulus = 1e6;
    cfg->shear_modulus = 1e6 / (2.0 * (1.0 + 0.5));
    cfg->gravity[0] = 0.0; cfg->gravity[1] = -9.80665; cfg->gravity[2] = 0.0;
    cfg->damping_constant = 2e-3;
    return SOFTROD_OK;
}

int softrod_config_softpendulum3d(softrod_config* cfg, int n_envs) {
    if (!cfg || n_envs < 1) return SOFTROD_EINVAL;
    config_common(cfg, n_envs);
    cfg->features = SOFTROD_FEATURES_SOFTPENDULUM3D;
    cfg->env_kind = SOFTROD_ENV_SOFTPENDULUM3D;
    cfg->filter_order = 7;
    cfg->base_length = 1.0;
    cfg->base_radius = 0.1;
    cfg->density = 4000.0;
    cfg->youngs_modulus = 1e6;
    cfg->shear_modulus = 1e6 / (2.0 * (1.0 + 0.5));
    cfg->gravity[0] = 0.0; cfg->gravity[1] = 0.0; cfg->gravity[2] = -9.80665;
    cfg->damping_constant = 1.0;
    cfg->base_step = 1e-3;
    cfg->base_limit = 0.5;
    return SOFTROD_OK;
}

// ... 137 lines not shown
int softrod_config_muscle_octopus(softrod_config* cfg, int n_envs, int env_kind) {
    if (!cfg || n_envs < 1 || !mocto_kind(env_kind)) return fail(nullptr, SOFTROD_EINVAL, "bad argument");
    const int rc = softrod_config_arm_push(cfg, n_envs, 1);
    if (rc != SOFTROD_OK) return rc;
    cfg->features = SOFTROD_FEATURES_ARM_PULL_WEIGHT;
    cfg->env_kind = env_kind;
    cfg->n_elem = 20;
    cfg->dt = 5.0e-5;
    cfg->n_substeps = (int)(1.0 / (25 * cfg->dt));
    cfg->final_time = env_kind == SOFTROD_ENV_CRAWL ? 10.0 : 5.0;
    cfg->base_length = 0.25;
    cfg->base_radius = 0.013;
    cfg->density = 1000.0;
    cfg->youngs_modulus = 1.5e4;
    cfg->shear_modulus = 1.5e4 / (1.0 + 0.5);
    cfg->damping_constant = 0.20 * 1e-2;
    cfg->damper_time_step = 7e-5;
    cfg->n_arm = env_kind == SOFTROD_ENV_ARM_TWO ? 2 : 8;
    cfg->n_knots = env_kind == SOFTROD_ENV_CRAWL ? 3 : (env_kind == SOFTROD_ENV_ARM_TWO ? 9 : 3 * cfg->n_elem);
    cfg->head_radius = 0.04;
    cfg->head_density = 50.0;
    cfg->head_length = 0.013 * 2;
    cfg->head_center[0] = 0.0; cfg->head_center[1] = 0.0; cfg->head_center[2] = -0.013 * 2 + 0.013 * 2 / 2;
    cfg->head_fixed = env_kind == SOFTROD_ENV_REACH ? 1 : 0;
    cfg->joint_k = 1e6; cfg->joint_kt = 1e2; cfg->joint_nu = 1e-3;
    if (env_kind == SOFTROD_ENV_ARM_TWO) {
        cfg->joint_angle0 = 90.0; cfg->joint_angle_step = 180.0;
        cfg->n_suckers = 3;
        for (int j = 0; j < 3; ++j) cfg->sucker_index[j] = cfg->n_elem / (3 * 2) * (2 * j + 1);
    } else {
        cfg->joint_angle0 = 45.0 / 2; cfg->joint_angle_step = 45.0;
        cfg->n_suckers = env_kind == SOFTROD_ENV_CRAWL ? 1 : 0;
        cfg->sucker_index[0] = 0;
    }
    cfg->sucker_reduction_ratio = 1.0;
    cfg->damp_before_constrain = 1;
    return SOFTROD_OK;
}

int softrod_create(const softrod_config* cfg, int device, softrod_handle** out) {
    if (!cfg || !out) return fail(nullptr, SOFTROD_EINVAL, "null argument");
    *out = nullptr;
    if (cfg->struct_size != sizeof(softrod_config))
        return fail(nullptr, SOFTROD_EINVAL, "softrod_config.struct_size mismatch");
    if (const char* why = config_why_not(*cfg)) return fail(nullptr, SOFTROD_EINVAL, why);
    int ndev = 0;
    const hipError_t cnt_err = hipGetDeviceCount(&ndev);
    if (cnt_err != hipSuccess || ndev < 1)
        return fail(nullptr, SOFTROD_ENODEV,
                    std::string("no HIP device visible: hipGetDeviceCount -> ") +
                        hipGetErrorString(cnt_err) + ", count " + std::to_string(ndev));
    if (device < 0 || device >= ndev) return fail(nullptr, SOFTROD_EINVAL, "device out of range");
    softrod_handle* h = new (std::nothrow) softrod_handle;
    if (!h) return fail(nullptr, SOFTROD_ENOMEM, "host allocation failed");
    h->cfg = *cfg;
    h->device = device;
    shape_handle(h);
    const bool mocto = is_mocto(h);
    const size_t N = (size_t)cfg->n_envs;
    const size_t adim = (size_t)softrod_config_action_dim(cfg);
    const size_t rowb = N * kLanes * h->epl * h->nw * sizeof(double);
    int rc = SOFTROD_OK;
    auto alloc = [&](auto*& p, size_t bytes) {
        if (rc == SOFTROD_OK && alloc_owned(h, p, bytes) != hipSuccess) rc = p ? SOFTROD_EHIP : SOFTROD_ENOMEM;
    };
    auto upload = [&](void* dst, const void* src, size_t bytes) {
        if (rc == SOFTROD_OK && hipMemcpy(dst, src, bytes, hipMemcpyHostToDevice) != hipSuccess) rc = SOFTROD_EHIP;
    };
    DeviceGuard guard_(device);
    if (guard_.err != hipSuccess) rc = SOFTROD_EHIP;
    alloc(h->S.pos, 3 * rowb);
    alloc(h->S.vel, 3 * rowb);
    alloc(h->S.dir, 9 * rowb);
    alloc(h->S.omg, 3 * rowb);
    alloc(h->S.tan, 3 * rowb);
    alloc(h->S.time, N * sizeof(double));
    alloc(h->S.bc, 12 * N * sizeof(double));
    alloc(h->S.ctrl, 4 * N * sizeof(double));
    alloc(h->S.kap, 3 * rowb);
    alloc(h->S.rkap, 3 * rowb);
    alloc(h->S.envmem, rowb);
    alloc(h->S.prev_action, N * (adim > 7 ? adim : 7) * sizeof(float));
    alloc(h->S.head, 20 * N * sizeof(double));
    alloc(h->d_spline, (size_t)(SOFTROD_MAX_SPLINE_PIECES + 1 + SOFTROD_MAX_SPLINE_PIECES * 4 * 4) * sizeof(double));
    h->P.spline = h->d_spline;
    alloc(h->d_ticket, sizeof(unsigned));
    alloc(h->d_params, sizeof(RodParams));
    h->S.params = h->d_params;
    alloc(h->d_state, sizeof(StatePtrs));
    h->S.self = h->d_state;
    if (cfg->n_substeps > 0) {
        const std::vector<double> tab = clock_table(*cfg);
        alloc(h->d_time_tab, tab.size() * sizeof(double));
        upload(h->d_time_tab, tab.data(), tab.size() * sizeof(double));
        h->S.time_tab = h->d_time_tab;
        h->P.tab_len = (int)tab.size();
        h->P.tab_n_sub = cfg->n_substeps;
        h->P.inv_step_time = 1.0 / ((double)cfg->n_substeps * cfg->dt);
    }
    upload(h->d_params, &h->P, sizeof(RodParams));
    const size_t NS = N * (size_t)(mocto ? cfg->n_arm : 1);
    alloc(h->S.sucker, (size_t)SOFTROD_MAX_SUCKERS * NS * sizeof(double));
    alloc(h->S.sucker_idx, (size_t)SOFTROD_MAX_SUCKERS * NS * sizeof(int));
    if (cfg->early_termination || mocto) alloc(h->S.aux, (size_t)8 * N * sizeof(double));
    if (mocto) alloc(h->S.prev_kappa, N * (size_t)cfg->n_arm * (size_t)(cfg->n_elem - 1) * sizeof(float));
    {
        std::vector<int> idx((size_t)SOFTROD_MAX_SUCKERS * NS, 0);
        for (int j = 0; j < SOFTROD_MAX_SUCKERS; ++j)
            for (size_t e = 0; e < NS; ++e) idx[(size_t)j * NS + e] = cfg->sucker_index[j];
        upload(h->S.sucker_idx, idx.data(), idx.size() * sizeof(int));
    }
    if (cfg->features & SOFTROD_FEAT_COOMM_MUSCLES) {
        alloc(h->S.mact, (size_t)SOFTROD_MAX_MUSCLES * rowb);
        alloc(h->d_mtab, (size_t)SOFTROD_MAX_MUSCLES * 4 * kLanes * h->epl * sizeof(double));
        h->S.mtab = h->d_mtab;
    }
    if (cfg->features & SOFTROD_FEAT_SUCKER_CONSTRAINT) {
        std::vector<double> init((size_t)SOFTROD_MAX_SUCKERS * NS, 0.0);
        for (int j = 0; j < cfg->n_suckers; ++j)
            for (size_t e = 0; e < NS; ++e) init[(size_t)j * NS + e] = cfg->sucker_reduction_ratio;
        upload(h->S.sucker, init.data(), init.size() * sizeof(double));
    }
    {
        const std::vector<double> radius((size_t)cfg->n_elem, cfg->base_radius);
        alloc(h->d_render_radius, radius.size() * sizeof(double));
        upload(h->d_render_radius, radius.data(), radius.size() * sizeof(double));
    }
    alloc(h->d_basis, (size_t)2 * kLanes * 7 * sizeof(double));
    h->S.basis = h->d_basis;
    alloc(h->d_init, N * h->init_stride * sizeof(double));
    alloc(h->d_mask, N);
    if (rc == SOFTROD_OK && hipHostMalloc((void**)&h->h_init, N * h->init_stride * sizeof(double)) != hipSuccess) rc = SOFTROD_ENOMEM;
    if (rc == SOFTROD_OK && hipHostMalloc((void**)&h->h_mask, N) != hipSuccess) rc = SOFTROD_ENOMEM;
    if (rc == SOFTROD_OK && hipEventCreateWithFlags(&h->ev_reset, hipEventDisableTiming) != hipSuccess)
        rc = SOFTROD_EHIP;
    alloc(h->d_pairs, N * sizeof(int2));
    if (rc == SOFTROD_OK && hipHostMalloc((void**)&h->h_pairs, N * sizeof(int2)) != hipSuccess) rc = SOFTROD_ENOMEM;
    if (rc == SOFTROD_OK && hipEventCreateWithFlags(&h->ev_pairs, hipEventDisableTiming) != hipSuccess)
        rc = SOFTROD_EHIP;
    h->is_dst.assign(N, 0);
    upload(h->d_state, &h->S, sizeof(StatePtrs));
    if (rc != SOFTROD_OK) {
        softrod_destroy(h);
        return fail(nullptr, rc, "device allocation failed");
    }
    *out = h;
    return SOFTROD_OK;
}

int softrod_reset_octo(softrod_handle* h, const double* arm_start, const double* arm_direction,
                       const double* target, const uint8_t* mask, void* stream) {
    if (!h || !arm_start || !arm_direction || !target) return fail(h, SOFTROD_EINVAL, "null argument");
    if (!is_flat(h) && !is_mocto(h)) return fail(h, SOFTROD_EINVAL, "softrod_reset_octo is for SOFTROD_ENV_OCTO_FLAT and the muscle octopus envs");
    SR_ON_DEVICE(h);
    SR_HIP(h, hipEventSynchronize(h->ev_reset));
    const size_t N = (size_t)h->cfg.n_envs, na = (size_t)h->cfg.n_arm, td = octo_target_dim(h);
    double* tgt = h->h_init + N * na * 18;
    for (size_t e = 0; e < N; ++e) {
        if (mask) h->h_mask[e] = mask[e];
        if (mask && !mask[e]) continue;
        octo_record(h, arm_start + 3 * na * e, arm_direction + 3 * na * e, target + td * e, h->h_init + e * na * 18, tgt + td * e);
    }
    return upload_and_reset(h, (hipStream_t)stream, mask != nullptr);
}

namespace {
// ... 606 lines not shown
        if (prev_action) return fail(h, SOFTROD_EINVAL, "the muscle octopus envs observe with their resident prev_action (pass NULL)");
        hipLaunchKernelGGL(softrod_mocto_epilogue_kernel, grid, dim3(kLanes * h->nw), 0, (hipStream_t)stream, h->P, h->S, obs,
                           nullptr, nullptr, nullptr, 0, 0);
    } else if (observes_as_body(h))
        hipLaunchKernelGGL(softrod_octo_observe_kernel, grid, dim3(kLanes * h->nw), 0, (hipStream_t)stream,
                           h->P, h->S, prev_action, obs);
    else
        hipLaunchKernelGGL(by_epl(h, softrod_observe_kernel<1>, softrod_observe_kernel<2>), grid, block, 0,
                           (hipStream_t)stream, h->P, h->S, nullptr, prev_action, obs, nullptr, 0);
    SR_HIP(h, hipGetLastError());
    return SOFTROD_OK;
}

namespace {
using ReadoutKernel = void (*)(RodParams, StatePtrs, int, int, int, double*);
enum class ReadoutGrid { kPerRod, kPerEnv };
int launch_readout(softrod_handle* h, ReadoutKernel kernel, double* out, void* stream, ReadoutGrid grid = ReadoutGrid::kPerRod) {
    SR_ON_DEVICE(h);
    const RodLayout y = rod_layout(h);
    const int waves = h->cfg.n_envs * (grid == ReadoutGrid::kPerEnv ? 1 : y.rods);
    hipLaunchKernelGGL(kernel, dim3((unsigned)waves), dim3(kLanes), 0, (hipStream_t)stream, h->P, h->S,
                       y.rods, y.lane_stride, y.arm_stride, out);
    SR_HIP(h, hipGetLastError());
    return SOFTROD_OK;
}
}

int softrod_rod_energies(softrod_handle* h, double* out, void* stream) {
    if (!h || !out) return fail(h, SOFTROD_EINVAL, "null argument");
    return launch_readout(h, by_epl(h, softrod_rod_energies_kernel<1>, softrod_rod_energies_kernel<2>), out, stream);
}

int softrod_ground_reaction(softrod_handle* h, double* out, void* stream) {
    if (!h || !out) return fail(h, SOFTROD_EINVAL, "null argument");
    if (const char* why = ground_reaction_why_not(h)) return fail(h, SOFTROD_EINVAL, why);
    return launch_readout(h, softrod_ground_reaction_kernel, out, stream);
}

int softrod_rod_strains(softrod_handle* h, double* out, void* stream) {
    if (!h) return fail(h, SOFTROD_EINVAL, "rod strains: null handle");
    if (!out) return fail(h, SOFTROD_EINVAL, "rod strains: null output buffer");
    return launch_readout(h, by_epl(h, softrod_rod_strains_kernel<1>, softrod_rod_strains_kernel<2>), out, stream);
}

int softrod_muscle_loads(softrod_handle* h, double* out, void* stream) {
    if (!h) return fail(h, SOFTROD_EINVAL, "muscle loads: null handle");
    if (!out) return fail(h, SOFTROD_EINVAL, "muscle loads: null output buffer");
    if (!(h->cfg.features & SOFTROD_FEAT_COOMM_MUSCLES)) return fail(h, SOFTROD_EINVAL, "muscle loads: this handle has no COOMM muscles");
    if (!h->muscles_set) return fail(h, SOFTROD_EINVAL, "muscle loads: softrod_set_muscle_layers has not been called");
    return launch_readout(h, by_epl(h, softrod_muscle_loads_kernel<1>, softrod_muscle_loads_kernel<2>), out, stream);
}

int softrod_joint_loads(softrod_handle* h, double* out, void* stream) {
    if (!h) return fail(h, SOFTROD_EINVAL, "joint loads: null handle");
    if (!out) return fail(h, SOFTROD_EINVAL, "joint loads: null output buffer");
    if (!(h->cfg.features & SOFTROD_FEAT_OCTO_HEAD)) return fail(h, SOFTROD_EINVAL, "joint loads: this handle has no rigid body");
    return launch_readout(h, softrod_joint_loads_kernel, out, stream, ReadoutGrid::kPerEnv);
}

int softrod_rod_dynamics(softrod_handle* h, double* out, void* stream) {
    if (!h) return fail(h, SOFTROD_EINVAL, "rod dynamics: null handle");
    if (!out) return fail(h, SOFTROD_EINVAL, "rod dynamics: null output buffer");
    if (const char* why = rod_dynamics_why_not(h)) return fail(h, SOFTROD_EINVAL, why);
    return launch_readout(h, softrod_rod_dynamics_kernel, out, stream);
}

int softrod_copy_envs(softrod_handle* h, const int32_t* src, const int32_t* dst, int count, void* stream) {
    if (!h) return fail(h, SOFTROD_EINVAL, "copy envs: null handle");
    const std::string why = copy_envs_why_not(h, src, dst, count);
    if (!why.empty()) return fail(h, SOFTROD_EINVAL, why);
    SR_ON_DEVICE(h);
    hipStream_t st = (hipStream_t)stream;
    SR_HIP(h, hipEventSynchronize(h->ev_pairs));
    int n = 0;
    for (int i = 0; i < count; ++i)
        if (src[i] != dst[i]) h->h_pairs[n++] = make_int2(src[i], dst[i]);
    if (n == 0) return SOFTROD_OK;
    SR_HIP(h, copy_table_rows(h->env_mat, h->h_pairs, n));
    SR_HIP(h, copy_table_rows(h->env_contact, h->h_pairs, n));
    SR_HIP(h, hipMemcpyAsync(h->d_pairs, h->h_pairs, (size_t)n * sizeof(int2), hipMemcpyHostToDevice, st));
    SR_HIP(h, hipEventRecord(h->ev_pairs, st));
    hipLaunchKernelGGL(softrod_copy_envs_kernel, dim3((unsigned)n), dim3(kCopyThreads), 0, st, copy_table(h), h->d_pairs);
    SR_HIP(h, hipGetLastError());
    return SOFTROD_OK;
}

int softrod_bank_create(softrod_handle* h, int slots) {
    if (!h) return fail(h, SOFTROD_EINVAL, "bank create: null handle");
    if (h->q_depth > 0)
        return fail(h, SOFTROD_EINVAL, "bank create: not on a handle with device-side auto-reset (the pending-reset flags and "
                                       "the staged queue belong to each env's RNG future)");
    if (h->bank.slots)
        return fail(h, SOFTROD_EINVAL, "bank create: the handle already has a state bank of " + std::to_string(h->bank.slots) + " slots");
    if (slots < 1) return fail(h, SOFTROD_EINVAL, "bank create: slots " + std::to_string(slots) + " is not positive");
    SR_ON_DEVICE(h);
    StateBank bank;
    bank.slots = slots;
    const size_t most = (size_t)(slots > h->cfg.n_envs ? slots : h->cfg.n_envs);
    hipError_t e = bank_adopt(h, bank);
    if (e == hipSuccess) e = hipMalloc((void**)&bank.d_pairs, most * sizeof(int2));
    if (e == hipSuccess) e = hipHostMalloc((void**)&bank.h_pairs, most * sizeof(int2), hipHostMallocDefault);
    if (e == hipSuccess) e = hipEventCreateWithFlags(&bank.ev_pairs, hipEventDisableTiming);
    if (e != hipSuccess) {
        (void)hipGetLastError();
        bank.release();
        return fail(h, e == hipErrorOutOfMemory ? SOFTROD_ENOMEM : SOFTROD_EHIP, std::string("bank create: ") + hipGetErrorString(e));
    }
    try {
        bank.filled.assign((size_t)slots, 0);
        bank.seen.assign(most, 0);
        if (h->env_mat.dev) bank.mat.assign((size_t)slots, EnvMaterial{});
        if (h->env_contact.dev) bank.contact.assign((size_t)slots, EnvContact{});
    } catch (const std::bad_alloc&) {
        bank.release();
        return fail(h, SOFTROD_ENOMEM, "bank create: out of host memory");
    }
    h->bank = std::move(bank);
    return SOFTROD_OK;
}

int softrod_bank_save(softrod_handle* h, const int32_t* envs, const int32_t* slots, int count, void* stream) {
    if (!h) return fail(h, SOFTROD_EINVAL, "bank save: null handle");
    return bank_copy(h, envs, slots, count, false, stream);
}

int softrod_bank_load(softrod_handle* h, const int32_t* slots, const int32_t* envs, int count, void* stream) {
    if (!h) return fail(h, SOFTROD_EINVAL, "bank load: null handle");
    return bank_copy(h, envs, slots, count, true, stream);
}

int softrod_bank_info(softrod_handle* h, int32_t* slots, uint64_t* bytes_per_slot, uint8_t* filled) {
    if (!h) return fail(h, SOFTROD_EINVAL, "bank info: null handle");
    if (!slots || !bytes_per_slot) return fail(h, SOFTROD_EINVAL, "bank info: null argument");
    const CopyTable T = copy_table(h);
    uint64_t bytes = 0;
    for (int k = 0; k < T.n; ++k) bytes += (uint64_t)T.a[k].comps * T.a[k].row_bytes;
    *slots = h->bank.slots;
    *bytes_per_slot = bytes;
    if (filled && h->bank.slots) std::memcpy(filled, h->bank.filled.data(), h->bank.filled.size());
    return SOFTROD_OK;
}

namespace {
EnvTarget env_target(const softrod_handle* h) {
    const softrod_config& c = h->cfg;
    const size_t N = (size_t)c.n_envs;
    EnvTarget T{};
    switch (c.env_kind) {
        case SOFTROD_ENV_ARM_SINGLE: T.kind = 1; T.constant[0] = c.target[0]; T.constant[1] = c.target[1]; break;
        case SOFTROD_ENV_OCTO_FLAT: T.kind = 2; T.rows = h->S.head + 18 * N; T.dims = 2; break;
        case SOFTROD_ENV_CRAWL: case SOFTROD_ENV_ARM_TWO: T.kind = 2; T.rows = h->S.aux; T.dims = 2; break;
        case SOFTROD_ENV_REACH: T.kind = 2; T.rows = h->S.aux; T.dims = 3; break;
        case SOFTROD_ENV_SOFT_ARM: T.kind = 2; T.rows = h->S.ctrl + N; T.dims = 3; break;
        default: break;
    }
    return T;
}
}

int softrod_camera_default(const softrod_config* cfg, softrod_camera* cam) {
    if (!cfg || !cam) return fail(nullptr, SOFTROD_EINVAL, "render: null argument");
    std::memset(cam, 0, sizeof(*cam));
    cam->struct_size = (uint32_t)sizeof(softrod_camera);
    cam->width = 84;
    cam->height = 84;
    const double L = cfg->base_length;
// ... 20 lines not shown

int softrod_camera_check(const softrod_camera* cam) {
    if (!cam) return fail(nullptr, SOFTROD_EINVAL, "render: null camera");
    if (cam->struct_size != sizeof(softrod_camera)) return fail(nullptr, SOFTROD_EINVAL, "render: softrod_camera.struct_size mismatch");
    if (cam->width < 1 || cam->width > 1024 || cam->height < 1 || cam->height > 1024)
        return fail(nullptr, SOFTROD_EINVAL, "render: width and height must be 1 .. 1024");
    const double* fields[] = {cam->center, cam->right, cam->up, cam->light};
    bool finite = std::isfinite(cam->half_width) && std::isfinite(cam->target_radius) && std::isfinite(cam->ambient);
    for (const double* f : fields)
        for (int i = 0; i < 3; ++i) finite = finite && std::isfinite(f[i]);
    if (!finite) return fail(nullptr, SOFTROD_EINVAL, "render: a camera field is not finite");
    if (!(cam->half_width > 0.0)) return fail(nullptr, SOFTROD_EINVAL, "render: half_width must be positive");
    auto dot = [](const double* x, const double* y) { return x[0] * y[0] + x[1] * y[1] + x[2] * y[2]; };
    const double tol = 1e-6;
    if (std::fabs(std::sqrt(dot(cam->right, cam->right)) - 1.0) > tol || std::fabs(std::sqrt(dot(cam->up, cam->up)) - 1.0) > tol)
        return fail(nullptr, SOFTROD_EINVAL, "render: right and up must be unit vectors (to 1e-6)");
    if (std::fabs(dot(cam->right, cam->up)) > tol) return fail(nullptr, SOFTROD_EINVAL, "render: right and up must be orthogonal (to 1e-6)");
    if (std::fabs(std::sqrt(dot(cam->light, cam->light)) - 1.0) > tol)
        return fail(nullptr, SOFTROD_EINVAL, "render: light must be a unit vector (to 1e-6)");
    if (cam->ambient < 0.0 || cam->ambient > 1.0) return fail(nullptr, SOFTROD_EINVAL, "render: ambient must be in [0, 1]");
    if (cam->target_radius < 0.0) return fail(nullptr, SOFTROD_EINVAL, "render: target_radius must not be negative");
    if (cam->follow != 0 && cam->follow != 1) return fail(nullptr, SOFTROD_EINVAL, "render: follow must be 0 or 1");
    return SOFTROD_OK;
}

int softrod_render(softrod_handle* h, const softrod_camera* cam, uint8_t* rgb, float* depth, void* stream) {
    if (!h) return fail(h, SOFTROD_EINVAL, "render: null handle");
    if (!cam) return fail(h, SOFTROD_EINVAL, "render: null camera");
    if (!rgb) return fail(h, SOFTROD_EINVAL, "render: null rgb buffer");
    if (softrod_camera_check(cam) != SOFTROD_OK) return fail(h, SOFTROD_EINVAL, g_err);
    const softrod_config& c = h->cfg;
    const RodLayout y = rod_layout(h);
    RenderScene sc{};
    sc.pos = h->S.pos;
    sc.head = is_octo(h) ? h->S.head : nullptr;
    sc.radius = h->d_render_radius;
    sc.head_radius = (float)c.head_radius;
    sc.n_envs = c.n_envs; sc.n_elem = c.n_elem; sc.rods = y.rods; sc.lane_stride = y.lane_stride; sc.arm_stride = y.arm_stride;
    sc.target = env_target(h);
    sc.n_prims = y.rods * c.n_elem + (sc.head ? 1 : 0) + (sc.target.kind ? 1 : 0);
    if (sc.n_prims > kRenderMaxPrims)
        return fail(h, SOFTROD_EINVAL, "render: more than " + std::to_string(kRenderMaxPrims) + " primitives per env");
    RenderCamera rc{};
    for (int i = 0; i < 3; ++i) {
        rc.c[i] = cam->center[i]; rc.a[i] = cam->right[i]; rc.b[i] = cam->up[i];
        rc.light[i] = (float)cam->light[i];
    }
    rc.n[0] = rc.a[1] * rc.b[2] - rc.a[2] * rc.b[1];
    rc.n[1] = rc.a[2] * rc.b[0] - rc.a[0] * rc.b[2];
    rc.n[2] = rc.a[0] * rc.b[1] - rc.a[1] * rc.b[0];
    rc.half_width = (float)cam->half_width; rc.target_radius = (float)cam->target_radius; rc.ambient = (float)cam->ambient;
    rc.width = cam->width; rc.height = cam->height; rc.follow = cam->follow;
    const int tiles_x = (cam->width + kRenderTileW - 1) / kRenderTileW, tiles_y = (cam->height + kRenderTileH - 1) / kRenderTileH;
    if ((size_t)c.n_envs * (size_t)tiles_x * (size_t)tiles_y > (size_t)INT32_MAX)
        return fail(h, SOFTROD_EINVAL, "render: n_envs x tiles exceeds the grid (render a smaller frame)");
    const int wide = cam->width % kRenderPx == 0 && ((uintptr_t)rgb & 3u) == 0 && ((uintptr_t)depth & 15u) == 0;
    SR_ON_DEVICE(h);
    hipLaunchKernelGGL(softrod_render_kernel, dim3((unsigned)(c.n_envs * tiles_x * tiles_y)), dim3(kRenderThreads),
                       render_lds_bytes(sc.n_prims), (hipStream_t)stream, sc, rc, rgb, depth, tiles_x, tiles_y, wide);
    SR_HIP(h, hipGetLastError());
    return SOFTROD_OK;
}

int softrod_rod_clearance(softrod_handle* h, int self_gap, double* out, void* stream) {
    if (!h) return fail(h, SOFTROD_EINVAL, "rod clearance: null handle");
    if (!out) return fail(h, SOFTROD_EINVAL, "rod clearance: null output buffer");
    if (self_gap < 2 || self_gap > 126) return fail(h, SOFTROD_EINVAL, "rod clearance: self_gap must be 2 .. 126");
    const softrod_config& c = h->cfg;
    const RodLayout y = rod_layout(h);
    const size_t waves = (size_t)c.n_envs * (size_t)(y.rods * (y.rods + 1) / 2 + y.rods);
    if (waves > (size_t)INT32_MAX) return fail(h, SOFTROD_EINVAL, "rod clearance: n_envs x record pairs exceeds the grid");
    SR_ON_DEVICE(h);
    hipLaunchKernelGGL(by_epl(h, softrod_rod_clearance_kernel<1>, softrod_rod_clearance_kernel<2>), dim3((unsigned)waves),
                       dim3(kLanes), 0, (hipStream_t)stream, h->S.pos, h->d_render_radius, env_target(h), c.n_envs, c.n_elem,
                       y.rods, y.lane_stride, y.arm_stride, self_gap, out);
    SR_HIP(h, hipGetLastError());
    return SOFTROD_OK;
}

int softrod_set_rod_shape(softrod_handle* h, const double* kappa, const double* sigma, const double* velocity,
                          const double* omega, const uint8_t* mask, void* stream) {
    if (!h) return fail(h, SOFTROD_EINVAL, "set rod shape: null handle");
    SR_ON_DEVICE(h);
    const RodLayout y = rod_layout(h);
    const RodShapeArgs args{kappa, sigma, velocity, omega, mask, nullptr};
    hipLaunchKernelGGL(by_epl(h, softrod_rod_shape_kernel<1>, softrod_rod_shape_kernel<2>), dim3((unsigned)(h->cfg.n_envs * y.rods)),
                       dim3(kLanes), 0, (hipStream_t)stream, h->P, h->S, y.rods, y.lane_stride, y.arm_stride, args);
    SR_HIP(h, hipGetLastError());
    return SOFTROD_OK;
}

uint32_t softrod_reset_shape_index(uint64_t seed, uint32_t env, uint32_t episode, uint32_t count) {
    return count ? reset_shape_index(seed, env, episode, count) : 0u;
}

int softrod_set_reset_shapes(softrod_handle* h, int count, const double* kappa, const double* sigma, const double* velocity,
                             const double* omega, uint64_t seed, void* stream) {
    if (!h) return fail(h, SOFTROD_EINVAL, "set reset shapes: null handle");
    if (count < 0) return fail(h, SOFTROD_EINVAL, "set reset shapes: negative count");
    SR_ON_DEVICE(h);
    hipStream_t st = (hipStream_t)stream;
    const size_t N = (size_t)h->cfg.n_envs;
    const int n = h->cfg.n_elem;
    const size_t rows = (size_t)count * (size_t)rod_layout(h).rods * 3;
    const size_t width[4] = {(size_t)(n - 1), (size_t)n, (size_t)(n + 1), (size_t)n};
    const double* given[4] = {kappa, sigma, velocity, omega};
    double* fresh[4] = {nullptr, nullptr, nullptr, nullptr};
    for (int f = 0; f < 4; ++f) {
        if (!count || !given[f]) continue;
        const size_t bytes = rows * width[f] * sizeof(double);
        hipError_t e = hipMalloc((void**)&fresh[f], bytes);
        if (e == hipSuccess) e = hipMemcpyAsync(fresh[f], given[f], bytes, hipMemcpyDeviceToDevice, st);
        if (e != hipSuccess) {
            for (double* p : fresh) if (p) (void)hipFree(p);
            return fail(h, SOFTROD_EHIP, std::string("set reset shapes: ") + hipGetErrorString(e));
        }
    }
    if (count && !h->d_rs_index) {
        int *ix = nullptr, *ep = nullptr;
        uint8_t* pk = nullptr;
        hipError_t e = alloc_owned(h, ix, N * sizeof(int));
        if (e == hipSuccess) e = alloc_owned(h, ep, N * sizeof(int));
        if (e == hipSuccess) e = alloc_owned(h, pk, N);
        if (e != hipSuccess) {
            for (double* p : fresh) if (p) (void)hipFree(p);
            return fail(h, SOFTROD_EHIP, std::string("set reset shapes: ") + hipGetErrorString(e));
        }
        h->d_rs_index = ix; h->d_rs_episode = ep; h->d_rs_picked = pk;
        if (h->bank.slots && (e = bank_adopt(h, h->bank)) != hipSuccess) {
            h->d_rs_index = h->d_rs_episode = nullptr; h->d_rs_picked = nullptr;
            for (double* p : fresh) if (p) (void)hipFree(p);
            return fail(h, SOFTROD_EHIP, std::string("set reset shapes: state bank: ") + hipGetErrorString(e));
        }
    }
    if (h->d_rs_index) {
        SR_HIP(h, hipMemsetAsync(h->d_rs_index, 0xFF, N * sizeof(int), st));
        SR_HIP(h, hipMemsetAsync(h->d_rs_episode, 0, N * sizeof(int), st));
        if (h->bank.slots) {
            const size_t K = (size_t)h->bank.slots;
            SR_HIP(h, hipMemsetAsync(h->bank.twin_of(h->d_rs_index), 0xFF, K * sizeof(int), st));
            SR_HIP(h, hipMemsetAsync(h->bank.twin_of(h->d_rs_episode), 0, K * sizeof(int), st));
        }
    }
    for (int f = 0; f < 4; ++f) {
        if (h->d_rs_field[f]) (void)hipFree(h->d_rs_field[f]);
        h->d_rs_field[f] = fresh[f];
    }
    h->rs_count = count;
    h->rs_seed = seed;
    return SOFTROD_OK;
}

int softrod_apply_reset_shapes(softrod_handle* h, const uint8_t* mask, void* stream) {
    if (!h) return fail(h, SOFTROD_EINVAL, "apply reset shapes: null handle");
    if (!h->rs_count) return fail(h, SOFTROD_EINVAL, "apply reset shapes: no pool is set (softrod_set_reset_shapes)");
    SR_ON_DEVICE(h);
    return launch_reset_shapes(h, kPickMask, mask, nullptr, nullptr, nullptr, nullptr, 0, (hipStream_t)stream);
}

int softrod_reset_shapes_view(softrod_handle* h, int32_t** index, int32_t** episode) {
    if (!h) return fail(h, SOFTROD_EINVAL, "reset shapes view: null handle");
    if (!index || !episode) return fail(h, SOFTROD_EINVAL, "reset shapes view: null argument");
    if (!h->rs_count) return fail(h, SOFTROD_EINVAL, "reset shapes view: no pool is set (softrod_set_reset_shapes)");
    *index = h->d_rs_index;
    *episode = h->d_rs_episode;
    return SOFTROD_OK;
}

int softrod_state_view_get(softrod_handle* h, softrod_state_view* out) {
    if (!h || !out) return fail(h, SOFTROD_EINVAL, "null argument");
    out->n_envs = h->cfg.n_envs;
    out->n_elem = h->cfg.n_elem;
    const RodLayout y = rod_layout(h);
    out->lane_stride = y.lane_stride;
    out->arm_stride = y.arm_stride;
    out->position = h->S.pos;
    out->velocity = h->S.vel;
    out->director = h->S.dir;
    out->omega = h->S.omg;
    out->tangents = h->S.tan;
    out->time = h->S.time;
    out->control = h->S.ctrl;
    out->kappa = h->S.kap;
    out->rest_kappa = h->S.rkap;
    out->env_memory = h->S.envmem;
    out->prev_action = h->S.prev_action;
    out->head = h->S.head;
    out->bc_targets = h->S.bc;
    out->sucker_ratio = h->S.sucker;
    out->muscle_activation = h->S.mact;
    out->sucker_index = h->S.sucker_idx;
    out->material = h->d_mat;
    out->env_aux = h->S.aux;
    out->prev_kappa = h->S.prev_kappa;
    return SOFTROD_OK;
}

int softrod_set_timing(softrod_handle* h, int n_launches) {
    if (!h || n_launches < 0 || n_launches > (1 << 20)) return fail(h, SOFTROD_EINVAL, "bad argument");
    SR_ON_DEVICE(h);
    while ((int)h->ev_start.size() < n_launches) {
        hipEvent_t a = nullptr, b = nullptr;
        SR_HIP(h, hipEventCreate(&a));
        SR_HIP(h, hipEventCreate(&b));
        h->ev_start.push_back(a);
        h->ev_stop.push_back(b);
    }
    while ((int)h->ev_start.size() > n_launches) {
        (void)hipEventDestroy(h->ev_start.back());
        (void)hipEventDestroy(h->ev_stop.back());
        h->ev_start.pop_back();
        h->ev_stop.pop_back();
    }
    h->timed = 0;
    return SOFTROD_OK;
}

int softrod_kernel_times_ms(softrod_handle* h, float* out_ms, int cap, int* count) {
    if (!h || !out_ms || !count || cap < 0) return fail(h, SOFTROD_EINVAL, "bad argument");
    SR_ON_DEVICE(h);
    const int n = h->timed < cap ? h->timed : cap;
    for (int i = 0; i < n; ++i) {
        SR_HIP(h, hipEventSynchronize(h->ev_stop[i]));
        SR_HIP(h, hipEventElapsedTime(out_ms + i, h->ev_start[i], h->ev_stop[i]));
    }
    *count = n;
    return SOFTROD_OK;
}

int softrod_last_kernel_ms(softrod_handle* h, float* ms) {
    if (!h || !ms) return fail(h, SOFTROD_EINVAL, "null argument");
    if (h->timed < 1) return fail(h, SOFTROD_EINVAL, "timing not enabled or no timed launch yet");
    SR_ON_DEVICE(h);
    SR_HIP(h, hipEventSynchronize(h->ev_stop[h->timed - 1]));
    SR_HIP(h, hipEventElapsedTime(ms, h->ev_start[h->timed - 1], h->ev_stop[h->timed - 1]));
    return SOFTROD_OK;
}

const char* softrod_last_error(softrod_handle* h) { return h ? h->err.c_str() : g_err.c_str(); }

const char* softrod_kernel_tier(softrod_handle* h) {
    if (!h) return "";
    const StepChoice c = select_step(h);
    std::string t = c.row ? c.row->label : std::string("none: ") + c.why;
    auto fill = [&t](const char* token, const std::string& with) {
        const size_t at = t.find(token);
        if (at != std::string::npos) t.replace(at, std::strlen(token), with);
    };
    fill("{waves}", std::to_string(h->nw) + (h->nw == 1 ? " wave" : " waves"));
    fill("{refresh}", std::to_string(h->window_refresh));
    if (c.row && c.row->windowed)
        if (const StepRow* after = select_step(h, 0).row) t += std::string(" + ") + after->label + " epilogue";
    if (h->env_mat.dev) t += ",env material";
    if (h->env_contact.dev) t += ",env contact";
    h->tier = t;
    return h->tier.c_str();
}

int softrod_destroy(softrod_handle* h) {
    if (!h) return SOFTROD_OK;
    DeviceGuard guard_(h->device);
    (void)hipDeviceSynchronize();
    autoreset_release(h);
    for (void* p : h->owned) (void)hipFree(p);
    for (double* p : h->d_rs_field) if (p) (void)hipFree(p);
    if (h->h_init) (void)hipHostFree(h->h_init);
    h->env_mat.release();
    h->env_contact.release();
    if (h->h_mask) (void)hipHostFree(h->h_mask);
    for (hipEvent_t e : h->ev_start) (void)hipEventDestroy(e);
    for (hipEvent_t e : h->ev_stop) (void)hipEventDestroy(e);
    if (h->ev_reset) (void)hipEventDestroy(h->ev_reset);
    if (h->h_pairs) (void)hipHostFree(h->h_pairs);
    if (h->ev_pairs) (void)hipEventDestroy(h->ev_pairs);
    h->bank.release();
    delete h;
    return SOFTROD_OK;
}

}
// ... 7 lines not shown
```

### gym_softrobot_amd/csrc/softrod_copy_envs.hpp

```cpp
#pragma once

namespace softrod {

constexpr int kCopyThreads = 256;
constexpr int kCopyMaxArrays = 24;

struct CopyArray {
    unsigned char* base;
    unsigned comps;
    unsigned row_bytes;
};
struct CopyTable {
    int n, n_envs;
    CopyArray a[kCopyMaxArrays];
};

__global__ void __launch_bounds__(kCopyThreads)
softrod_copy_envs_kernel(const CopyTable T, const int2* __restrict__ pairs) {
    const int2 p = pairs[blockIdx.x];
    const size_t N = (size_t)T.n_envs, src = (size_t)p.x, dst = (size_t)p.y;
    for (int k = 0; k < T.n; ++k) {
        const CopyArray A = T.a[k];
        const size_t comp_stride = N * (size_t)A.row_bytes;
        const unsigned char* from = A.base + src * (size_t)A.row_bytes;
        unsigned char* to = A.base + dst * (size_t)A.row_bytes;
        if ((A.row_bytes & 15u) == 0) {
            const unsigned per = A.row_bytes >> 4, total = A.comps * per;
            for (unsigned i = threadIdx.x; i < total; i += kCopyThreads) {
                const unsigned c = i / per, u = i - c * per;
                const size_t off = (size_t)c * comp_stride + ((size_t)u << 4);
                *reinterpret_cast<uint4*>(to + off) = *reinterpret_cast<const uint4*>(from + off);
            }
        } else {
            const unsigned per = A.row_bytes >> 2, total = A.comps * per;
            for (unsigned i = threadIdx.x; i < total; i += kCopyThreads) {
                const unsigned c = i / per, u = i - c * per;
                const size_t off = (size_t)c * comp_stride + ((size_t)u << 2);
                *reinterpret_cast<unsigned*>(to + off) = *reinterpret_cast<const unsigned*>(from + off);
            }
        }
    }
}

}
```

### gym_softrobot_amd/csrc/softrod_fast.hpp

```cpp
#pragma once

namespace softrod {

__device__ __forceinline__ bool wave_any(bool p) { return __builtin_amdgcn_ballot_w64(p) != 0ull; }
__device__ __forceinline__ bool wave_any_of(unsigned long long lanes, bool p) {
    return (__builtin_amdgcn_ballot_w64(p) & lanes) != 0ull;
}

__device__ __forceinline__ double horner(double g, double y, double c) {
    double d;
    asm("v_fma_f64 %0, %1, %2, %3" : "=v"(d) : "v"(g), "v"(y), "v"(c));
    return d;
}
__device__ __forceinline__ void fma_over(double& d, double a, double b, double c) {
    asm("v_fma_f64 %0, %1, %2, %3" : "+v"(d) : "v"(a), "v"(b), "v"(c));
}
__device__ __forceinline__ void fma_inplace_u(double& x, double m, double a) {
    asm("v_fma_f64 %0, %1, %0, %2" : "+v"(x) : "s"(m), "v"(a));
}

template <bool LEAN = true, bool ON_CIRCLE = false>
__device__ __forceinline__ void sinc_cosc(double t, double& sc, double& cc) {
    if (!wave_any(t >= 1.0e-3)) {
        if constexpr (LEAN) {
// ... 492 lines not shown
        poison_rod<EPL>(L);
        time = S.time[rod];
    } else {
        load_lane<EPL, F>(S, N, rod, lane, L);
        BcTargets B;
        load_bc(S, N, rod, B);
        EnvAction A;
        set_action_n<F, E, EPL>(P, S, N, rod, lane, actions, A, B, L);
        constrain_rates_n<F, EPL>(P, B, lane, L);
        constrain_values_n<F, EPL>(P, B, lane, L);
        time = S.time[rod];
        if (n_sub > 0) {
            ConstN<EPL> C;
            if constexpr (kEnvMaterial<F>) build_const_m<F, EPL>(P, S.env_mat[rod], lane, A, C);
            else build_const<F, EPL>(P, lane, A, C);
            if constexpr (kEnvContact<F>) C.ct = S.env_contact[rod];
            RodParams Pk = P;
            if (!has<F>(P, SOFTROD_FEAT_ANALYTICAL_DAMPER)) Pk.damp_t = 1.0;
            general_substeps<F, EPL>(P, Pk, C, B, lane, L, n_sub);
        }
    }
    time = clock_after(P, S, time, n_sub);
    store_lane<EPL, F>(S, N, rod, lane, L);
    if (lane == 0) S.time[rod] = time;
}

#ifndef SOFTROD_FAST_WAVES
#define SOFTROD_FAST_WAVES 3
#endif
#ifndef SOFTROD_PLANAR_WAVES
#define SOFTROD_PLANAR_WAVES 4
#endif
#ifndef SOFTROD_PLANAR_EXEC_MASK
#define SOFTROD_PLANAR_EXEC_MASK 1
#endif
#ifndef SOFTROD_CONTACT_WAVES
#define SOFTROD_CONTACT_WAVES 2
#endif
#ifndef SOFTROD_RUNTIME_WAVES
#define SOFTROD_RUNTIME_WAVES 2
#endif
#ifdef SOFTROD_PHASE_CLOCKS
__device__ unsigned long long g_phase_clock[16384][8];
#define SR_PHASE(i) do { __builtin_amdgcn_s_waitcnt(0); if (threadIdx.x == 0 && blockIdx.x < 16384) \
        g_phase_clock[blockIdx.x][i] = wall_clock64(); } while (0)
#else
#define SR_PHASE(i) do {} while (0)
#endif

template <unsigned F, int EPL, bool TAPER>
constexpr int fast_kernel_waves() {
    if (EPL > 1) return 1;
    if (F == kRuntimeFeatures) return SOFTROD_RUNTIME_WAVES;
    if (F & (SOFTROD_FEAT_PLANE_CONTACT_ANISO | SOFTROD_FEAT_LAPLACE_FILTER | SOFTROD_FEAT_SPLINE_MUSCLE_TORQUES |
             SOFTROD_FEAT_COOMM_MUSCLES))
        return SOFTROD_CONTACT_WAVES;
    if (TAPER) return SOFTROD_CONTACT_WAVES;
    return (F & ~kFeatEnvMaterial) == SOFTROD_FEATURES_SOFTPENDULUM ? SOFTROD_PLANAR_WAVES : SOFTROD_FAST_WAVES;
}

template <unsigned F, int E, int EPL, bool TAPER = false>
__global__ void __launch_bounds__(kLanes, (fast_kernel_waves<F, EPL, TAPER>()))
softrod_step_fast_kernel(const RodParams P, const StatePtrs S, const float* __restrict__ actions,
                         float* __restrict__ obs, double* __restrict__ reward,
                         uint8_t* __restrict__ terminated, uint8_t* __restrict__ truncated,
                         double* __restrict__ aux, const int n_sub, const int epilogue, const int pack) {
    const int rod = blockIdx.x;
    const int lane = threadIdx.x;
    const size_t N = (size_t)P.n_envs;
    [[maybe_unused]] EnvMaterial M;
    if constexpr (kEnvMaterial<F>) M = S.env_mat[rod];
    [[maybe_unused]] EnvContact CT;
    if constexpr (kEnvContact<F>) CT = S.env_contact[rod];
    if (epilogue && S.skip && S.skip[rod]) {
        if (lane == 0) S.skip[rod] = 0;
        if (lane == 0 && early_term_on<F>(P)) S.aux[rod] = 0.0;
        return;
    }

    __builtin_amdgcn_s_setprio(3);
    SR_PHASE(0);
    constexpr bool kPlanarKernel = (F & ~kFeatEnvMaterial) == SOFTROD_FEATURES_SOFTPENDULUM;
    LaneN<EPL> L;
    load_lane<EPL, F, !kPlanarKernel>(S, N, rod, lane, L);
    SR_PHASE(1);
    if (has<F>(P, SOFTROD_FEAT_LAPLACE_FILTER)) sanitize_unused_rates<EPL>(P, lane, L);
    if (has<F>(P, SOFTROD_FEAT_PLANE_CONTACT_ANISO)) sanitize_unused_slots<EPL>(P, lane, L);
    BcTargets B;
    load_bc(S, N, rod, B);
    load_suckers<F>(P, S, N, rod, B);
    EnvAction A;
    set_action_n<F, E, EPL>(P, S, N, rod, lane, actions, A, B, L);
    if (epilogue) push_store_prev_com<F, E, EPL>(P, S, N, rod, lane, L, n_sub);
    if (has<F>(P, SOFTROD_FEAT_SPLINE_MUSCLE_TORQUES)) muscle_load<EPL>(P, S, rod, actions != nullptr, A, L);
    {
        BcTargets B0 = B;
        if (has<F>(P, SOFTROD_FEAT_MOVING_BASE_BC)) {
            B0.vel[0] = __shfl(L.v[0][0], 0); B0.vel[1] = __shfl(L.v[0][1], 0); B0.vel[2] = __shfl(L.v[0][2], 0);
        }
        constrain_rates_n<F, EPL>(P, B0, lane, L);
        constrain_values_n<F, EPL>(P, B, lane, L);
    }
    double time = S.time[rod];
    ConstN<EPL> C;
    if constexpr (kEnvMaterial<F>) build_const_m<F, EPL, TAPER>(P, M, lane, A, C, S.mat);
    else build_const_m<F, EPL, TAPER>(P, P, lane, A, C, S.mat);
    if constexpr (kEnvContact<F>) C.ct = CT;
    if constexpr (kMusclesCompiled<F>) build_muscle_const<F, EPL, true>(P, S, N, rod, lane, A, C);
    RodParams Pk = P;
    if (!has<F>(P, SOFTROD_FEAT_ANALYTICAL_DAMPER)) Pk.damp_t = 1.0;

    bool blown_up = false;
    if (n_sub > 0 && epilogue && rod_has_nan<EPL>(P, lane, L)) {
        blown_up = true;
        if constexpr (!kPlanarKernel) {
            poison_rod<EPL>(L);
            time = clock_after(P, S, time, n_sub);
        }
    }
    if constexpr (kPlanarKernel) {
        PlanarN<EPL> Z;
        if (n_sub > 0 && !blown_up && planar_from_lane<EPL>(P, B, lane, L, Z)) {
            PlanarC<EPL> K;
            planar_build_const<EPL, kEnvMaterial<F>>(Pk, C, lane, K);
            const double ta = P.time_two_half_adds ? P.half_dt : P.dt;
            const double tb = P.time_two_half_adds ? P.half_dt : 0.0;
            int tk = -1;
            if (S.time_tab && n_sub == P.tab_n_sub) {
                const double kf = rint(time * P.inv_step_time);
                const int k = (kf >= 0.0 && kf < (double)(P.tab_len - 1)) ? (int)kf : -1;
                tk = (k >= 0 && S.time_tab[k] == time) ? k : -1;
            }
            const double step_dt = EPL > 1 ? opaque_v(P.dt) : P.dt;
            SR_PHASE(2);
#if SOFTROD_PLANAR_EXEC_MASK
            if (lane * EPL <= P.n_elem) {
#endif
                planar_kinematic_n<EPL>(P.half_dt, K.hq_hdt, C, K, Z);
                {
                    int s = 0;
#pragma unroll
                    for (int q = 0; q < 4; ++q) {
                        if (q == 1) __builtin_amdgcn_s_setprio(2);
                        if (q == 2) __builtin_amdgcn_s_setprio(1);
                        if (q == 3) __builtin_amdgcn_s_setprio(0);
                        const int end = ProgressPriority::bound(n_sub - 1, q);
                        for (; s < end; ++s) {
                            planar_dynamic_n<EPL>(Pk, C, K, lane, Z);
#ifdef SOFTROD_DIAG_TWO_HALF_STEPS
                            planar_kinematic_n<EPL>(P.half_dt, K.hq_hdt, C, K, Z);
                            planar_kinematic_n<EPL>(P.half_dt, K.hq_hdt, C, K, Z);
#else
                            planar_kinematic_n<EPL>(step_dt, K.hq_dt, C, K, Z);
#endif
                        }
                    }
                }
                planar_dynamic_n<EPL>(Pk, C, K, lane, Z);
                planar_kinematic_n<EPL>(P.half_dt, K.hq_hdt, C, K, Z);
#if SOFTROD_PLANAR_EXEC_MASK
            }
#endif
            if (__builtin_amdgcn_readfirstlane(tk) >= 0) time = S.time_tab[tk + 1];
            else
                for (int s = 0; s < n_sub; ++s) time = (time + ta) + tb;
            SR_PHASE(3);
            planar_store<EPL>(S, N, rod, lane, Z, !SOFTROD_PLANAR_EXEC_MASK || lane * EPL <= P.n_elem);
#pragma unroll
            for (int s = 0; s < EPL; ++s) {
#pragma unroll
                for (int c = 0; c < 3; ++c) { L.x[s][c] = 0.0; L.v[s][c] = 0.0; L.w[s][c] = 0.0; L.t[s][c] = 0.0; }
#pragma unroll
                for (int c = 0; c < 9; ++c) L.Q[s][c] = 0.0;
            }
            planar_to_lane<EPL>(Z, L);
        } else {
            general_step_cold<F, E, EPL>(S.params, S.self, rod, lane, actions, n_sub, blown_up);
            __builtin_amdgcn_fence(__ATOMIC_ACQUIRE, "wavefront");
            load_lane<EPL, F>(S, N, rod, opaque_lane(lane), L);
            time = S.time[rod];
        }
    } else {
        if (n_sub > 0 && !blown_up) {
            general_substeps<F, EPL, TAPER>(P, Pk, C, B, lane, L, n_sub);
            time = clock_after(P, S, time, n_sub);
        }
        store_lane<EPL, F>(S, N, rod, lane, L);
    }
    if (has<F>(P, SOFTROD_FEAT_SPLINE_MUSCLE_TORQUES)) muscle_store<EPL>(P, S, rod, lane, L);
    if (env_of<E>(P) == SOFTROD_ENV_SOFT_ARM && lane == 0)
        S.ctrl[(size_t)0 * N + rod] += (double)n_sub;
    if (lane == 0) S.time[rod] = time;
    SR_PHASE(4);
    if (epilogue)
        env_epilogue_n<E, EPL, F>(P, S, N, rod, lane, C, L, time, A, obs, reward, terminated, truncated, aux, pack);
    SR_PHASE(5);
}


}
```

### gym_softrobot_amd/csrc/softrod_kernels.hpp

```cpp
#pragma once
#include <hip/hip_runtime.h>
#include <stdint.h>

#include "../../include/softrod.h"

namespace softrod {

constexpr int kLanes = 64;

constexpr unsigned kRuntimeFeatures = 0xFFFFFFFFu;
constexpr unsigned kFeaturesTaperedSuckerArm = SOFTROD_FEAT_ANALYTICAL_DAMPER | SOFTROD_FEAT_SUCKER_CONSTRAINT;
constexpr unsigned kFeatPlaneZup = 1u << 30;
constexpr unsigned kFeatEarlyTerm = 1u << 29;
constexpr unsigned kFeatEnvMaterial = 1u << 28;
template <unsigned F>
constexpr bool kEnvMaterial = F != kRuntimeFeatures && (F & kFeatEnvMaterial) != 0;
constexpr unsigned kFeatEnvContact = 1u << 27;
template <unsigned F>
constexpr bool kEnvContact = F != kRuntimeFeatures && (F & kFeatEnvContact) != 0;
constexpr int kRuntimeEnv = -1;
constexpr unsigned kFeaturesMuscleRod = SOFTROD_FEAT_FIXED_BC | SOFTROD_FEAT_ANALYTICAL_DAMPER | SOFTROD_FEAT_COOMM_MUSCLES;
template <unsigned F>
constexpr bool kMusclesCompiled = F != kRuntimeFeatures && (F & SOFTROD_FEAT_COOMM_MUSCLES) != 0;

// ... 13 lines not shown
    double damp_t;
    double damp_r[3];
    double damp_logr[3];
    double eps_length, eps_rot_axis, acos_shift, eps_sin;
    double two_acos_shift, neg_eps_sin;
    double base_limit, step_time;
    float base_step, control_penalty_coeff;
    int contact_before_forcing, n_action;
    double mass_total;
    double target[2], kappa_range[2], kappa_rate_range[2];
    double plane_origin[3], plane_normal[3];
    double contact_k, contact_nu, slip_tol, surface_tol;
    double kin_mu[3], stat_mu[3];
    double r0_sqrt_rest_len;
    int seg, n_arm, seg_shift, head_fixed;
    double head_mass, head_invJ[3], head_radius;
    double head_center[3], joint_angle0, joint_angle_step;
    int n_ctrl, n_pieces;
    double muscle_scale, max_rate, base_length, arm_target[3];
    const double* spline;
    double joint_k, joint_nu, joint_kt;
    int n_suckers, sucker_index[SOFTROD_MAX_SUCKERS], pad2;
    double sucker_ratio0;
    int tab_len, tab_n_sub;
    double inv_step_time;
    int n_muscles, muscle_kind[SOFTROD_MAX_MUSCLES], fl_degree, muscle_form, muscle_cur_radius, muscle_tm_law, push_mode, pad3;
    double fl_coef[SOFTROD_MAX_FL_COEF];
};

enum MatRow { kMatMass = 0, kMatShear01, kMatShear2, kMatBend01, kMatBend2, kMatJ0, kMatJ2, kMatInvJ0, kMatInvJ2,
              kMatDampLog0, kMatDampLog2, kMatDampR0, kMatDampR2, kMatR0s, kMatInvR0s, kMatRows = SOFTROD_MATERIAL_ROWS };

struct EnvMaterial {
    double J[3], invJ[3];
    double shear[3], bend[3];
    double mass_node, mass_total, damp_t;
    double damp_r[3], damp_logr[3];
    double pad[3];
};
static_assert(sizeof(EnvMaterial) == 192, "EnvMaterial: three 64-byte lines");

struct EnvContact {
    double k, nu;
    double kin_am[2], stat_am[2];
    double kin_mu[3], stat_mu[3];
    double pad[4];
};
static_assert(sizeof(EnvContact) == 128, "EnvContact: two 64-byte lines");

struct StatePtrs {
    double* pos;
    double* vel;
    double* dir;
    double* omg;
    double* tan;
    double* time;
    double* bc;
    double* ctrl;
    double* kap;
    double* rkap;
    float* prev_action;
    double* envmem;
    const double* basis;
    double* head;
    uint8_t* needs_reset;
    uint8_t* skip;
    const double* queue;
    int* q_consumed;
    const int* q_produced;
    int* q_underflow;
    int q_depth, q_record;
    const struct RodParams* params;
    const struct StatePtrs* self;
    const double* time_tab;
    const double* mat;
    double* sucker;
    int* sucker_idx;
    double* mact;
    const double* mtab;
    double* aux;
    float* prev_kappa;
    const EnvMaterial* env_mat;
    const EnvContact* env_contact;
};

__device__ __forceinline__ double from_next(double x) {
    int lo = __double2loint(x), hi = __double2hiint(x);
    lo = __builtin_amdgcn_mov_dpp(lo, 0x130, 0xf, 0xf, true);
    hi = __builtin_amdgcn_mov_dpp(hi, 0x130, 0xf, 0xf, true);
    return __hiloint2double(hi, lo);
}
__device__ __forceinline__ double from_prev(double x) {
    int lo = __double2loint(x), hi = __double2hiint(x);
    lo = __builtin_amdgcn_mov_dpp(lo, 0x138, 0xf, 0xf, true);
    hi = __builtin_amdgcn_mov_dpp(hi, 0x138, 0xf, 0xf, true);
    return __hiloint2double(hi, lo);
}

__device__ __forceinline__ double wave_sum(double x) {
#pragma unroll
    for (int off = 32; off >= 1; off >>= 1) x += __shfl_xor(x, off);
    return x;
}

template <unsigned F>
__device__ __forceinline__ bool has(const RodParams& P, unsigned bit) {
    if constexpr (F == kRuntimeFeatures) return (P.features & bit) != 0;
    else return (F & bit) != 0;
}
template <unsigned F, bool RT = false>
__device__ __forceinline__ bool early_term_on(const RodParams& P) {
    if constexpr (F != kRuntimeFeatures) return (F & kFeatEarlyTerm) != 0;
    else return RT && (P.features & kFeatEarlyTerm) != 0;
}
template <int E>
__device__ __forceinline__ int env_of(const RodParams& P) {
    if constexpr (E == kRuntimeEnv) return P.env_kind;
    else return E;
}
__device__ __forceinline__ bool is_push_env(int env) { return env == SOFTROD_ENV_ARM_PUSH || env == SOFTROD_ENV_ARM_PULL_WEIGHT; }
template <unsigned F = kRuntimeFeatures>
__device__ __forceinline__ int slot_local(const RodParams& P, int raw) {
    if constexpr (F != kRuntimeFeatures) {
        if constexpr ((F & SOFTROD_FEAT_OCTO_HEAD) != 0)
            return (raw & (P.seg - 1)) | (raw >= P.n_arm * P.seg ? (1 << 20) : 0);
        else return raw;
    } else {
        return P.seg ? ((raw & (P.seg - 1)) | (raw >= P.n_arm * P.seg ? (1 << 20) : 0)) : raw;
    }
}

template <int EPL>
struct LaneN {
    double x[EPL][3], v[EPL][3];
    double Q[EPL][9], w[EPL][3];
    double t[EPL][3];
    double kap[EPL][3], rk[EPL][3];
    double pc[8];
    float pin[8];
    int mflag;
};

template <int EPL>
struct ConstN {
    double hx[EPL], hq[EPL];
    double cf[EPL], ca[EPL][3];
    double cw01[EPL], cw2[EPL];
    double s01[EPL], s2[EPL];
    double b01[EPL], bd[EPL];
    double mass[EPL], mass_next[EPL], inv_mass_pair[EPL];
    double gm[EPL][3];
    double j01[EPL], j2[EPL], dlog0[EPL], dlog2[EPL], dr0[EPL], dr2[EPL], r0s[EPL], ir0s[EPL];
    double mr[EPL][SOFTROD_MAX_MUSCLES][3], amp[EPL][SOFTROD_MAX_MUSCLES];
    const double* mtab_lane;
    const double* mact_lane;
    double damp_t, mass_total;
    EnvContact ct;
};

template <int EPL>
__device__ __forceinline__ void shift_next(const double (&a)[EPL], double (&o)[EPL]) {
#pragma unroll
    for (int s = 0; s + 1 < EPL; ++s) o[s] = a[s + 1];
    o[EPL - 1] = from_next(a[0]);
}
template <int EPL>
// ... 1519 lines not shown
    for (int s = 0; s < EPL; ++s) {
        const double len = sqrt(t[s][0] * t[s][0] + t[s][1] * t[s][1] + t[s][2] * t[s][2]) + P.eps_length;
#pragma unroll
        for (int c = 0; c < 3; ++c) t[s][c] /= len;
    }
}

__device__ __forceinline__ const double* staged_record(const StatePtrs& S, size_t N, int env, int k) {
    if (k >= S.q_produced[env]) {
        if (threadIdx.x == 0) atomicAdd(S.q_underflow, 1);
        return nullptr;
    }
    return S.queue + ((size_t)(k % S.q_depth) * N + env) * (size_t)S.q_record;
}

template <int EPL>
__global__ void __launch_bounds__(kLanes)
softrod_observe_kernel(const RodParams P, const StatePtrs S, const uint8_t* __restrict__ picked,
                       const float* __restrict__ prev_action, float* __restrict__ obs, double* __restrict__ aux,
                       const int pack) {
    const int rod = blockIdx.x;
    if (picked && !picked[rod]) return;
    const int lane = threadIdx.x;
    const size_t N = (size_t)P.n_envs;
    LaneN<EPL> L;
    load_lane<EPL, kRuntimeFeatures>(S, N, rod, lane, L);
    const int adim = (P.env_kind == SOFTROD_ENV_SOFTPENDULUM3D) ? 2
                   : (P.env_kind == SOFTROD_ENV_ARM_SINGLE) ? 7 : (P.env_kind == SOFTROD_ENV_SOFT_ARM) ? 0
                   : is_push_env(P.env_kind) ? (P.push_mode == 0 ? 1 : 2) : 1;
    float pa[7] = {0.0f, 0.0f, 0.0f, 0.0f, 0.0f, 0.0f, 0.0f};
    for (int i = 0; i < adim; ++i)
        pa[i] = prev_action ? prev_action[adim * (size_t)rod + i] : S.prev_action[7 * (size_t)rod + i];
    observe_rod<EPL>(P, S, N, rod, lane, L, pa, obs, pack, aux);
}

template <int EPL>
__device__ __forceinline__ void reset_rod(const RodParams& P, const StatePtrs& S, size_t N, int rod, int lane,
                                          const double* __restrict__ in, LaneN<EPL>& L) {
    constexpr size_t W = (size_t)kLanes * EPL;
    const int n = P.n_elem;
#pragma unroll
    for (int s = 0; s < EPL; ++s) {
        const int idx = lane * EPL + s;
#pragma unroll
        for (int c = 0; c < 3; ++c) {
            double xv = in[c] + (double)idx * in[3 + c];
            if (idx == n) xv = in[6 + c];
            L.x[s][c] = xv;
            L.v[s][c] = 0.0; L.w[s][c] = 0.0; L.kap[s][c] = 0.0; L.rk[s][c] = 0.0;
        }
#pragma unroll
        for (int c = 0; c < 9; ++c) L.Q[s][c] = in[9 + c];
    }
    unit_tangents<EPL>(P, L.x, L.t);
    store_lane<EPL, kRuntimeFeatures>(S, N, rod, lane, L);
#pragma unroll
    for (int s = 0; s < EPL; ++s) {
        const size_t m = (size_t)rod * W + (size_t)lane * EPL + s;
#pragma unroll
        for (int c = 0; c < 3; ++c) S.rkap[c * N * W + m] = 0.0;
        S.envmem[m] = 0.0;
    }
    double com[2] = {0.0, 0.0};
    if (P.env_kind == SOFTROD_ENV_ARM_SINGLE) {
        ConstN<EPL> C;
        no_action_const<EPL>(P, S, rod, lane, C);
        com_xy_n<EPL>(P, C, lane, L, com);
    }
    if (P.features & SOFTROD_FEAT_COOMM_MUSCLES) {
        if (S.mact) {
#pragma unroll
            for (int m = 0; m < SOFTROD_MAX_MUSCLES; ++m)
#pragma unroll
                for (int s = 0; s < EPL; ++s) S.mact[((size_t)m * N + rod) * W + (size_t)lane * EPL + s] = 0.0;
        }
    }
    if (lane == 0 && is_push_env(P.env_kind)) {
        S.sucker_idx[rod] = P.sucker_index[0];
        S.sucker[rod] = P.sucker_ratio0;
    }
    if (lane == 0) {
        S.time[rod] = 0.0;
        if (S.needs_reset) S.needs_reset[rod] = 0;
        if (P.env_kind == SOFTROD_ENV_SOFTPENDULUM3D) {
#pragma unroll
            for (int i = 0; i < 7; ++i) S.prev_action[7 * (size_t)rod + i] = 0.0f;
        }
#pragma unroll
        for (int i = 0; i < 3; ++i) S.bc[(size_t)i * N + rod] = in[i];
#pragma unroll
        for (int i = 0; i < 9; ++i) S.bc[(size_t)(3 + i) * N + rod] = in[9 + i];
#pragma unroll
        for (int i = 0; i < 4; ++i) S.ctrl[(size_t)i * N + rod] = (i < 2) ? com[i] : 0.0;
        if (P.env_kind == SOFTROD_ENV_SOFT_ARM) {
#pragma unroll
            for (int i = 0; i < 3; ++i) S.ctrl[(size_t)(1 + i) * N + rod] = P.arm_target[i];
        }
    }
}

template <int EPL>
__global__ void __launch_bounds__(kLanes)
softrod_reset_kernel(const RodParams P, const StatePtrs S, const ResetArgs A) {
    const int rod = blockIdx.x;
    if (A.mask && !A.mask[rod]) return;
    LaneN<EPL> L;
    reset_rod<EPL>(P, S, (size_t)P.n_envs, rod, threadIdx.x, A.init + (size_t)rod * 18, L);
}

__global__ void __launch_bounds__(kLanes)
softrod_queue_scatter_kernel(double* __restrict__ queue, const double* __restrict__ staged,
                             const int2* __restrict__ where, const int n_envs, const int record) {
    const int m = blockIdx.x;
    const int2 w = where[m];
    double* dst = queue + ((size_t)w.y * (size_t)n_envs + (size_t)w.x) * (size_t)record;
    const double* src = staged + (size_t)m * (size_t)record;
    for (int i = threadIdx.x; i < record; i += kLanes) dst[i] = src[i];
}

template <int EPL>
__global__ void __launch_bounds__(kLanes)
softrod_autoreset_kernel(const RodParams P, const StatePtrs S, float* __restrict__ obs,
                         double* __restrict__ reward, uint8_t* __restrict__ terminated,
                         uint8_t* __restrict__ truncated, double* __restrict__ aux, const int pack) {
    const int rod = blockIdx.x;
    const int lane = threadIdx.x;
    if (!S.needs_reset[rod]) return;
    const size_t N = (size_t)P.n_envs;
    const int k = S.q_consumed[rod];
    const double* in = staged_record(S, N, rod, k);
    if (!in) return;
    LaneN<EPL> L;
    reset_rod<EPL>(P, S, N, rod, lane, in, L);
    float pa[7];
#pragma unroll
    for (int i = 0; i < 7; ++i) pa[i] = S.prev_action[7 * (size_t)rod + i];
    float* o = observe_rod<EPL>(P, S, N, rod, lane, L, pa, obs, pack, aux);
    if (lane == 0) {
        emit_scalars(o, env_obs_dim(P), pack, rod, 0.0, false, false, reward, terminated, truncated, S.needs_reset);
        S.skip[rod] = 1;
        S.q_consumed[rod] = k + 1;
    }
}

}

#include "softrod_fast.hpp"
#include "softrod_octo.hpp"
#include "softrod_window.hpp"
#include "softrod_literal.hpp"
#include "softrod_readout.hpp"
#include "softrod_reaction.hpp"
#include "softrod_strains.hpp"
#include "softrod_muscle_readout.hpp"
#include "softrod_joint_readout.hpp"
#include "softrod_render.hpp"
#include "softrod_clearance.hpp"
#include "softrod_autoreset.hpp"
```

### gym_softrobot_amd/csrc/softrod_planar.hpp

```cpp
#pragma once

namespace softrod {

template <int EPL>
struct PlanarN {
    double x[EPL][2], v[EPL][2];
    double c[EPL], s[EPL];
    double s2;
    double wz[EPL];
    double t[EPL][2];
    double dl[EPL];
    double d[EPL][2];
    double dv[EPL][2];
};

template <int EPL>
struct PlanarC {
    double cfy[EPL], cay[EPL];
    double cwl[EPL];
    double bk[EPL];
    double bke[EPL];
    double xl[EPL];
    double hq_dt[EPL], hq_hdt[EPL];
    double jr;
    double s3, s2, s1, c3, c2, e4, e3;
    double eps_length, rest_len, damp_t;
    double two_shift;
};

__device__ __forceinline__ double opaque_s(double k) { asm("" : "+s"(k)); return k; }
__device__ __forceinline__ double opaque_v(double k) { asm("" : "+v"(k)); return k; }
template <int EPL>
__device__ __forceinline__ double uniform_k(double k) { return EPL > 1 ? opaque_v(k) : opaque_s(k); }

__device__ __forceinline__ void fma_inplace(double& x, double m, double a) {
    asm("v_fma_f64 %0, %1, %0, %2" : "+v"(x) : "v"(m), "v"(a));
}

__device__ __forceinline__ double rcp3(double x) { return fast_rcp(x); }
__device__ __forceinline__ double rsqrt3(double x) { return fast_rsqrt(x); }

template <int EPL, bool EM = false>
__device__ __forceinline__ void planar_build_const(const RodParams& P, const ConstN<EPL>& C, int lane,
                                                   PlanarC<EPL>& K) {
#pragma unroll
    for (int s = 0; s < EPL; ++s) {
        const bool pinned = (lane * EPL + s) == 0;
        K.cfy[s] = pinned ? 0.0 : C.cf[s];
        K.cay[s] = pinned ? 0.0 : C.ca[s][1];
        K.cwl[s] = C.cw01[s] * P.inv_rest_len;
        const double two_vor = 2.0 * P.rest_vor;
        K.bk[s] = C.b01[s] * (P.inv_rest_vor * (1.0 + P.acos_shift * (1.0 / 3.0))) * (two_vor * two_vor * two_vor);
        K.bke[s] = P.neg_eps_sin * K.bk[s];
        K.xl[s] = (lane * EPL + s) < P.n_elem ? (EM ? C.dlog0[s] : P.damp_logr[0]) * P.inv_rest_len : 0.0;
        K.hq_dt[s] = C.hq[s] * P.dt;
        if (EPL > 1) K.hq_dt[s] = opaque_v(K.hq_dt[s]);
        K.hq_hdt[s] = C.hq[s] * P.half_dt;
    }
    K.jr = (EM ? C.j01[0] : P.J[0]) * P.rest_len;
    K.s3 = uniform_k<EPL>(-1.0 / 5040.0); K.s2 = opaque_v(1.0 / 120.0); K.s1 = uniform_k<EPL>(-1.0 / 6.0);
    K.c3 = uniform_k<EPL>(-1.0 / 720.0); K.c2 = opaque_v(1.0 / 24.0);
    K.e4 = uniform_k<EPL>(1.0 / 24.0); K.e3 = opaque_v(1.0 / 6.0);
    K.eps_length = EPL > 1 ? opaque_v(P.eps_length) : P.eps_length;
    K.rest_len = EPL > 1 ? opaque_v(P.rest_len) : P.rest_len;
    const double damp_t = EM ? C.damp_t : P.damp_t;
    K.damp_t = EPL > 1 ? opaque_v(damp_t) : damp_t;
    K.two_shift = EPL > 1 ? opaque_v(P.two_acos_shift) : P.two_acos_shift;
    if (EPL > 1) K.jr = opaque_v(K.jr);
}

template <int EPL>
__device__ __forceinline__ double exp_one(const PlanarC<EPL>& K, double x) {
#ifdef SOFTROD_DIAG_LIBM_TRIG
    return exp(x);
#endif
    if (__builtin_expect(!wave_any(!(fabs(x) < 1.0e-3)), 1))
        return fma(x, fma(x, fma(x, fma(x, K.e4, K.e3), 0.5), 1.0), 1.0);
    int k = 0;
    while (wave_any(!(fabs(x) < 1.0e-3)) && k < 24) { x *= 0.5; ++k; }
    double e = fma(x, fma(x, fma(x, fma(x, 1.0 / 24.0, 1.0 / 6.0), 0.5), 1.0), 1.0);
    for (; k > 0; --k) e *= e;
    return e;
}

template <int EPL>
__device__ __forceinline__ bool planar_from_lane(const RodParams& P, const BcTargets& B, int lane,
                                                 const LaneN<EPL>& L, PlanarN<EPL>& Z) {
    const int n = P.n_elem;
    bool ok = (P.gravity[2] == 0.0) && (B.pos[2] == 0.0) && (B.Q[2] == 0.0) && (B.Q[8] == 0.0);
    Z.s2 = __shfl((L.Q[0][5] < 0.0) ? -1.0 : 1.0, 0);
#pragma unroll
    for (int s = 0; s < EPL; ++s) {
        const int idx = lane * EPL + s;
        const double* Q = L.Q[s];
        const double s2 = (Q[5] < 0.0) ? -1.0 : 1.0, c = Q[6], sn = Q[7];
        const bool node_ok = (L.x[s][2] == 0.0) && (L.v[s][2] == 0.0);
        const bool elem_ok = (Q[2] == 0.0) && (Q[3] == 0.0) && (Q[4] == 0.0) && (Q[8] == 0.0) && (s2 == Z.s2) &&
                             (fabs(fabs(Q[5]) - 1.0) <= 1.0e-12) && (L.w[s][0] == 0.0) && (L.w[s][2] == 0.0) &&
                             (fabs(fma(s2, sn, Q[0])) <= 1.0e-12) && (fabs(fma(-s2, c, Q[1])) <= 1.0e-12) &&
                             (fabs(fma(c, c, fma(sn, sn, -1.0))) <= 1.0e-12);
        ok = ok && (idx > n || node_ok) && (idx >= n || elem_ok);
        Z.x[s][0] = L.x[s][0]; Z.x[s][1] = L.x[s][1];
        Z.v[s][0] = L.v[s][0]; Z.v[s][1] = L.v[s][1];
        Z.c[s] = c; Z.s[s] = sn;
        Z.wz[s] = (idx < n) ? Z.s2 * L.w[s][1] : 0.0;
        Z.t[s][0] = 0.0; Z.t[s][1] = 0.0;
    }
#pragma unroll
    for (int c = 0; c < 2; ++c) {
        double a[EPL], o[EPL], av[EPL], ov[EPL];
#pragma unroll
        for (int s = 0; s < EPL; ++s) { a[s] = Z.x[s][c]; av[s] = Z.v[s][c]; }
        shift_next<EPL>(a, o);
        shift_next<EPL>(av, ov);
#pragma unroll
        for (int s = 0; s < EPL; ++s) { Z.d[s][c] = o[s] - a[s]; Z.dv[s][c] = ov[s] - av[s]; }
    }
    {
        double cnx[EPL], snx[EPL];
        shift_next<EPL>(Z.c, cnx);
        shift_next<EPL>(Z.s, snx);
#pragma unroll
        for (int s = 0; s < EPL; ++s) {
            const bool vor_valid = (lane * EPL + s) < n - 1;
            const double sinD = fma(snx[s], Z.c[s], -cnx[s] * Z.s[s]);
            const double cosD = fma(cnx[s], Z.c[s], snx[s] * Z.s[s]);
            Z.dl[s] = vor_valid ? atan2(sinD, cosD) : 0.0;
        }
    }
#ifdef SOFTROD_DIAG_NO_PLANAR
    return false;
#endif
    return !__any(!ok);
}

template <int EPL>
__device__ __forceinline__ void planar_to_lane(const PlanarN<EPL>& Z, LaneN<EPL>& L) {
#pragma unroll
    for (int s = 0; s < EPL; ++s) {
        L.x[s][0] = Z.x[s][0]; L.x[s][1] = Z.x[s][1];
        L.v[s][0] = Z.v[s][0]; L.v[s][1] = Z.v[s][1];
        L.Q[s][0] = -Z.s2 * Z.s[s]; L.Q[s][1] = Z.s2 * Z.c[s];
        L.Q[s][6] = Z.c[s]; L.Q[s][7] = Z.s[s];
        L.w[s][1] = Z.s2 * Z.wz[s];
        L.t[s][0] = Z.t[s][0]; L.t[s][1] = Z.t[s][1]; L.t[s][2] = 0.0;
    }
}

template <int EPL>
__device__ __forceinline__ void planar_store(const StatePtrs& S, size_t N, int rod, int lane, const PlanarN<EPL>& Z,
                                             bool stepped) {
    constexpr size_t W = (size_t)kLanes * EPL;
    const size_t base = (size_t)rod * W + (size_t)opaque_lane(lane) * EPL;
#pragma unroll
    for (int s = 0; s < EPL; ++s) {
        S.tan[2 * N * W + base + s] = 0.0;
        S.dir[0 * N * W + base + s] = -Z.s2 * Z.s[s];
        S.dir[1 * N * W + base + s] = Z.s2 * Z.c[s];
        S.omg[1 * N * W + base + s] = Z.s2 * Z.wz[s];
    }
    if (stepped) {
#pragma unroll
        for (int s = 0; s < EPL; ++s) {
#pragma unroll
            for (int c = 0; c < 2; ++c) {
                S.pos[c * N * W + base + s] = Z.x[s][c];
                S.vel[c * N * W + base + s] = Z.v[s][c];
                S.tan[c * N * W + base + s] = Z.t[s][c];
            }
            S.dir[6 * N * W + base + s] = Z.c[s];
            S.dir[7 * N * W + base + s] = Z.s[s];
        }
    }
}

template <int EPL>
__device__ __forceinline__ void planar_kinematic_n(double h, const double (&hq_h)[EPL], const ConstN<EPL>& C,
                                                   const PlanarC<EPL>& K, PlanarN<EPL>& Z) {
    double ra[EPL], ran[EPL];
#pragma unroll
    for (int s = 0; s < EPL; ++s) {
        const double hp = h * C.hx[s];
        Z.x[s][0] = fma(hp, Z.v[s][0], Z.x[s][0]);
        Z.x[s][1] = fma(hp, Z.v[s][1], Z.x[s][1]);
        Z.d[s][0] = fma(h, Z.dv[s][0], Z.d[s][0]);
        Z.d[s][1] = fma(h, Z.dv[s][1], Z.d[s][1]);
        const double a = hq_h[s] * Z.wz[s];
        ra[s] = a;
        const double t = a * a;
        double sc, cs;
#ifdef SOFTROD_DIAG_LIBM_TRIG
        cs = cos(a);
        const double sn = sin(a);
        sc = 0.0;
        (void)sc;
#else
        if (__builtin_expect(!wave_any(t >= 1.0e-3), 1)) {
            sc = fma(t, fma(t, fma(t, K.s3, K.s2), K.s1), 1.0);
            cs = fma(t, fma(t, fma(t, K.c3, K.c2), -0.5), 1.0);
        } else {
            double cc;
            sinc_cosc<false>(t, sc, cc);
            cs = fma(-cc, t, 1.0);
        }
        const double sn = sc * a;
#endif
        const double p = cs * Z.c[s], q = sn * Z.c[s];
        Z.c[s] = fma(-sn, Z.s[s], p);
        fma_inplace(Z.s[s], cs, q);
    }
    shift_next<EPL>(ra, ran);
#pragma unroll
    for (int s = 0; s < EPL; ++s) Z.dl[s] += ran[s] - ra[s];
#ifdef SOFTROD_DIAG_RECOMPUTE_EDGES
#pragma unroll
    for (int c = 0; c < 2; ++c) {
        double a[EPL], o[EPL];
#pragma unroll
        for (int s = 0; s < EPL; ++s) a[s] = Z.x[s][c];
        shift_next<EPL>(a, o);
#pragma unroll
        for (int s = 0; s < EPL; ++s) Z.d[s][c] = o[s] - a[s];
    }
#endif
#ifdef SOFTROD_DIAG_RECOMPUTE_ANGLE
    {
        double cnx[EPL], snx[EPL];
        shift_next<EPL>(Z.c, cnx);
        shift_next<EPL>(Z.s, snx);
#pragma unroll
        for (int s = 0; s < EPL; ++s) {
            const double sinD = fma(snx[s], Z.c[s], -cnx[s] * Z.s[s]);
            const double cosD = fma(cnx[s], Z.c[s], snx[s] * Z.s[s]);
            Z.dl[s] = atan2(sinD, cosD);
        }
    }
#endif
}

// ... 76 lines not shown
```

### gym_softrobot_amd/csrc/softrod_shape.hpp

```cpp
#pragma once

namespace softrod {

struct RodShapeArgs {
    const double* kappa;
    const double* sigma;
    const double* velocity;
    const double* omega;
    const uint8_t* mask;
    const int* pool_index;
};

__device__ __forceinline__ void shape_mul(const double (&A)[9], const double (&B)[9], double (&C)[9]) {
#pragma unroll
    for (int i = 0; i < 3; ++i)
#pragma unroll
        for (int l = 0; l < 3; ++l)
            C[3 * i + l] = A[3 * i] * B[l] + A[3 * i + 1] * B[3 + l] + A[3 * i + 2] * B[6 + l];
}
__device__ __forceinline__ void shape_rotation(const double (&v)[3], double (&R)[9]) {
    const double t = v[0] * v[0] + v[1] * v[1] + v[2] * v[2];
    double a, b;
    if (t < 1.0e-6) {
        a = 1.0 - t * (1.0 / 6.0) + t * t * (1.0 / 120.0);
        b = 0.5 - t * (1.0 / 24.0) + t * t * (1.0 / 720.0);
    } else {
        const double th = sqrt(t);
        a = sin(th) / th;
        b = (1.0 - cos(th)) / t;
    }
    const double d = 1.0 - b * t;
    R[0] = d + b * v[0] * v[0];
    R[4] = d + b * v[1] * v[1];
    R[8] = d + b * v[2] * v[2];
    R[1] = b * v[0] * v[1] - a * v[2];
    R[3] = b * v[0] * v[1] + a * v[2];
    R[2] = b * v[0] * v[2] + a * v[1];
    R[6] = b * v[0] * v[2] - a * v[1];
    R[5] = b * v[1] * v[2] - a * v[0];
    R[7] = b * v[1] * v[2] + a * v[0];
}

template <int EPL>
__global__ void __launch_bounds__(kLanes)
softrod_rod_shape_kernel(const RodParams P, const StatePtrs S, const int rods, const int lane_stride,
                         const int arm_stride, const RodShapeArgs A) {
    const ReadoutRod R = readout_rod(P, rods, lane_stride, arm_stride);
    if (A.mask && !A.mask[R.env]) return;
    const int lane = threadIdx.x;
    const int n = P.n_elem;
    const size_t NW = R.N * R.W;
    const size_t rod = A.pool_index ? (size_t)A.pool_index[R.env] * (size_t)rods + (size_t)R.arm : (size_t)R.rod;

    double M[EPL][9];
#pragma unroll
    for (int s = 0; s < EPL; ++s) {
        const int j = lane * EPL + s;
#pragma unroll
        for (int c = 0; c < 9; ++c) M[s][c] = (c == 0 || c == 4 || c == 8) ? 1.0 : 0.0;
        if (j == 0) {
#pragma unroll
            for (int c = 0; c < 9; ++c) M[s][c] = S.dir[c * NW + R.base];
        } else if (j < n) {
            double v[3] = {0.0, 0.0, 0.0};
            if (A.kappa) {
#pragma unroll
                for (int c = 0; c < 3; ++c) v[c] = -A.kappa[(rod * 3 + c) * (size_t)(n - 1) + (size_t)(j - 1)] * P.rest_vor;
            }
            shape_rotation(v, M[s]);
        }
    }
    double Q[EPL][9];
    {
        double T[9];
#pragma unroll
        for (int c = 0; c < 9; ++c) T[c] = M[0][c];
#pragma unroll
        for (int s = 1; s < EPL; ++s) {
            double U[9];
            shape_mul(M[s], T, U);
#pragma unroll
            for (int c = 0; c < 9; ++c) T[c] = U[c];
        }
#pragma unroll
        for (int d = 1; d < kLanes; d <<= 1) {
            double O[9], U[9];
#pragma unroll
            for (int c = 0; c < 9; ++c) O[c] = __shfl_up(T[c], d);
            shape_mul(T, O, U);
#pragma unroll
            for (int c = 0; c < 9; ++c) T[c] = (lane >= d) ? U[c] : T[c];
        }
        double E[9];
#pragma unroll
        for (int c = 0; c < 9; ++c) {
            const double up = __shfl_up(T[c], 1);
            E[c] = (lane >= 1) ? up : ((c == 0 || c == 4 || c == 8) ? 1.0 : 0.0);
        }
        if (lane == 0) {
#pragma unroll
            for (int c = 0; c < 9; ++c) Q[0][c] = M[0][c];
        } else {
            shape_mul(M[0], E, Q[0]);
        }
#pragma unroll
        for (int s = 1; s < EPL; ++s) shape_mul(M[s], Q[s - 1], Q[s]);
    }
    double x[EPL][3];
    {
        double e[EPL][3];
#pragma unroll
        for (int s = 0; s < EPL; ++s) {
            const int j = lane * EPL + s;
            double sg[3] = {0.0, 0.0, 0.0};
            if (A.sigma && j < n) {
#pragma unroll
                for (int c = 0; c < 3; ++c) sg[c] = A.sigma[(rod * 3 + c) * (size_t)n + (size_t)j];
            }
            sg[2] += 1.0;
#pragma unroll
            for (int c = 0; c < 3; ++c)
                e[s][c] = (j < n) ? P.rest_len * (Q[s][c] * sg[0] + Q[s][3 + c] * sg[1] + Q[s][6 + c] * sg[2]) : 0.0;
        }
#pragma unroll
        for (int c = 0; c < 3; ++c) {
            double t = e[0][c];
#pragma unroll
            for (int s = 1; s < EPL; ++s) t += e[s][c];
#pragma unroll
            for (int d = 1; d < kLanes; d <<= 1) {
                const double o = __shfl_up(t, d);
                t = (lane >= d) ? t + o : t;
            }
            const double up = __shfl_up(t, 1);
            double run = (lane >= 1) ? up : 0.0;
// ... 75 lines not shown
```

### gym_softrobot_amd/csrc/softrod_state_bank.hpp

```cpp
#pragma once

#include "softrod_copy_envs.hpp"

namespace softrod {

__global__ void __launch_bounds__(kCopyThreads)
softrod_bank_copy_kernel(const CopyTable From, const CopyTable To, const int2* __restrict__ pairs) {
    const int2 p = pairs[blockIdx.x];
    const size_t src = (size_t)p.x, dst = (size_t)p.y;
    for (int k = 0; k < From.n; ++k) {
        const CopyArray A = From.a[k];
        const unsigned char* to_base = To.a[k].base;
        const size_t row = (size_t)A.row_bytes;
        const size_t from_stride = (size_t)From.n_envs * row, to_stride = (size_t)To.n_envs * row;
        const unsigned char* from = A.base + src * row;
        unsigned char* to = const_cast<unsigned char*>(to_base) + dst * row;
        if ((A.row_bytes & 15u) == 0) {
            const unsigned per = A.row_bytes >> 4, total = A.comps * per;
            for (unsigned i = threadIdx.x; i < total; i += kCopyThreads) {
                const unsigned c = i / per, u = i - c * per;
                const size_t in = ((size_t)u << 4);
                *reinterpret_cast<uint4*>(to + (size_t)c * to_stride + in) =
                    *reinterpret_cast<const uint4*>(from + (size_t)c * from_stride + in);
            }
        } else {
            const unsigned per = A.row_bytes >> 2, total = A.comps * per;
            for (unsigned i = threadIdx.x; i < total; i += kCopyThreads) {
                const unsigned c = i / per, u = i - c * per;
                const size_t in = ((size_t)u << 2);
                *reinterpret_cast<unsigned*>(to + (size_t)c * to_stride + in) =
                    *reinterpret_cast<const unsigned*>(from + (size_t)c * from_stride + in);
            }
        }
    }
}

}
```

### gym_softrobot_amd/envs/base.py

```python
from __future__ import annotations

import copy
from collections import deque
from typing import Any, Dict, List, Optional, Sequence, Union

import numpy as np

from .. import _capi
from ..seeding import np_random
from ..spaces import Box

try:
    from gymnasium import Env as GymEnv
except Exception:
    class GymEnv:
        metadata: Dict[str, Any] = {}
        render_mode = None
        _np_random = None

        def reset(self, *, seed=None, options=None):
            if seed is not None:
                self._np_random, self._np_random_seed = np_random(seed)

        @property
# ... 388 lines not shown
        return t.cpu().numpy() if self.numpy_output else t

    def _seed_rngs(self, seed, mask: np.ndarray) -> None:
        n = self.num_envs
        if seed is None or isinstance(seed, (int, np.integer)):
            seeds = [None if seed is None else int(seed) + i for i in range(n)]
        else:
            seeds = list(seed)
            if len(seeds) != n:
                raise ValueError("need one seed per env")
        reseeded = np.zeros(n, bool)
        for i in range(n):
            if mask[i] and (seeds[i] is not None or self._rngs[i] is None):
                self._rngs[i], _ = np_random(seeds[i])
                reseeded[i] = True
        return reseeded

    def reset(
        self,
        *,
        seed: Optional[Union[int, Sequence[Optional[int]]]] = None,
        options: Optional[dict] = None,
        mask: Optional[np.ndarray] = None,
    ):
        n = self.num_envs
        m = np.ones(n, bool) if mask is None else np.asarray(mask, bool).reshape(n)
        reseeded = self._seed_rngs(seed, m)
        draws = None
        if self.device_autoreset and self._produced.any():
            self._sync_staged()
            by = np.zeros(n, np.int32)
            draws = {}
            for i in np.nonzero(m)[0]:
                if reseeded[i]:
                    by[i] = -1
                    self._popped[i] += len(self._staged[i])
                    self._staged[i].clear()
                elif self._staged[i]:
                    by[i] = 1
                    draws[i] = self._staged[i].popleft()
                    self._popped[i] += 1
            self.backend.queue_advance(by)
        self._reset_backend(m, mask is not None, draws)
        if self._reset_shapes:
            self._apply_reset_shapes(m if mask is not None else None, reseeded)
        self._steps[m] = 0
        self._needs_reset[m] = False
        obs = self.backend.observe(None)
        if self.device_autoreset:
            self._top_up()
        if self.config_generate_video and not self.is_octo:
            from ..diagnostics import RodRecorder

            self.recorder = RodRecorder(self.backend, self.record_envs)
        elif self.is_octo and (self.config_generate_video or getattr(self, "config_save_head_data", False)):
            from ..diagnostics import OctoRecorder

            self.recorder = OctoRecorder(self.backend, self.record_envs[0], rods=self.config_generate_video,
                                         head=self.config_save_head_data)
        return self._out(obs), {}

    @property
    def is_octo(self) -> bool:
        return int(self.cfg.env_kind) == _capi.ENV_OCTO_FLAT

    @property
    def rod_parameters_dict(self):
        return None if self.recorder is None or self.is_octo else self.recorder.params[0]

    @property
    def rod_parameters_dict_list(self):
        return getattr(self.recorder, "rod_parameters_dict_list", None)

    @property
    def head_dict(self):
        return getattr(self.recorder, "head_dict", None)

    def _step_device_autoreset(self, a):
        import torch

        obs, reward, term, trunc = self.backend.step(a)
        self._top_up_tick()
        if getattr(self, "_dev_time", None) is None:
            self._dev_time = self.backend.state()["time"]
        tl = self.backend.time_limit() if getattr(self.cfg, "early_termination", 0) else trunc.view(torch.bool)
        infos = {"time": self._out(self._dev_time), "TimeLimit.truncated": self._out(tl)}
        if self.same_step:
            infos.update(self._final_infos(term, trunc))
        return (self._out(obs), self._out(reward), self._out(term.view(torch.bool)),
                self._out(trunc.view(torch.bool)), infos)

    aux_info_key: Optional[str] = None

    def _final_infos(self, term, trunc) -> Dict[str, Any]:
        import torch

        be = self.backend
        final_info = {"time": self._out(be.final_time)}
        out = {"final_obs": self._out(be.final_obs), "_final_obs": self._out((term | trunc).view(torch.bool)),
               "final_info": final_info}
        if self.aux_info_key is not None:
            out[self.aux_info_key] = self._out(be.aux[:, 0])
            final_info[self.aux_info_key] = self._out(be.final_aux)
        return out

    def step(self, actions):
        import torch

        self._validate_actions(actions)
        a = torch.as_tensor(actions, dtype=torch.float32, device=self.backend.device)
        a = a.reshape(self.num_envs, self.action_dim)
        if self.device_autoreset:
            return self._step_device_autoreset(a)
        pending = self._needs_reset.copy() if self.autoreset else None
        saved_prev = None
        if pending is not None and pending.any():
            saved_prev = self.backend.prev_action_rows()[torch.from_numpy(pending)].clone()
        obs, reward, term, trunc = self.backend.step(a)
        self._steps += 1
        if pending is not None and pending.any():
            keep = obs.clone()
            self.backend.prev_action_rows()[torch.from_numpy(pending)] = saved_prev
            self._seed_rngs(None, pending)
            self._reset_backend(pending, True)
            if self._reset_shapes:
                self._apply_reset_shapes(pending)
            self._steps[pending] = 0
            robs = self.backend.observe(None)
            pm = torch.from_numpy(pending).to(robs.device)
            obs = torch.where(pm[:, None], robs, keep)
            reward = torch.where(pm, torch.zeros_like(reward), reward)
            term = torch.where(pm, torch.zeros_like(term), term)
            trunc = torch.where(pm, torch.zeros_like(trunc), trunc)
        if self.autoreset:
            self._needs_reset = (term | trunc).cpu().numpy().astype(bool)
        if self.recorder is not None:
            self.recorder.record()
        times = self._times()
        infos = self._infos(times)
        return (
            self._out(obs),
            self._out(reward),
            self._out(term.view(torch.bool)),
            self._out(trunc.view(torch.bool)),
            infos,
        )

    def rod_energies(self):
        return self._out(self.backend.rod_energies())

    def ground_reaction(self):
        be = self.backend
        if not hasattr(be, "ground_reaction"):
            raise NotImplementedError(f"ground reaction needs the HIP backend, not {type(be).__name__}")
        why = _capi.ground_reaction_refusal(self.cfg)
        if why is not None:
            raise NotImplementedError(why)
        force, torque = be.ground_reaction()
        return self._out(force), self._out(torque)

    def rod_strains(self):
        be = self.backend
        if not hasattr(be, "rod_strains"):
            raise NotImplementedError(f"rod strains need the HIP backend, not {type(be).__name__}")
        r = be.rod_strains()
        return type(r)(*(self._out(t) for t in r))

# ... 340 lines not shown
```

### include/softrod.h

```cpp
#ifndef SOFTROD_H
#define SOFTROD_H

#include <stddef.h>
#include <stdint.h>

#ifdef __cplusplus
extern "C" {
#endif

#define SOFTROD_ABI_VERSION 17

#define SOFTROD_OK 0
#define SOFTROD_EINVAL (-1)
#define SOFTROD_ENOMEM (-2)
#define SOFTROD_EHIP (-3)
#define SOFTROD_ENODEV (-4)

enum softrod_feature {
    SOFTROD_FEAT_GRAVITY = 1u << 0,
    SOFTROD_FEAT_POINT_FORCE_NODE0_X = 1u << 1,
    SOFTROD_FEAT_PENDULUM_BC = 1u << 2,
    SOFTROD_FEAT_ANALYTICAL_DAMPER = 1u << 3,
    SOFTROD_FEAT_FIXED_BC = 1u << 4,
    SOFTROD_FEAT_TIP_FORCE = 1u << 5,
// ... 209 lines not shown
int softrod_queue_status(softrod_handle* h, int32_t* consumed, int32_t* underflow,
                         void* stream);
int softrod_queue_status_begin(softrod_handle* h, void* stream);
int softrod_queue_status_poll(softrod_handle* h, int wait, int32_t* consumed, int32_t* underflow);
int softrod_queue_advance(softrod_handle* h, const int32_t* by, void* stream);

#define SOFTROD_MAX_PEERS 16
int softrod_scatter_rows(softrod_handle* h, const float* packed, const uint64_t* peer_buffers,
                         int n_peers, int row_words, int64_t first_row, int64_t tag_word,
                         uint32_t tag, void* stream);

#define SOFTROD_IPC_HANDLE_BYTES 64
#define SOFTROD_EXCHANGE_UNCACHED 1
#define SOFTROD_EXCHANGE_FINEGRAINED 2
int softrod_exchange_alloc(int device, uint64_t bytes, void** dev_ptr, uint8_t* ipc_handle,
                           int* memory_kind);
int softrod_exchange_open(int device, const uint8_t* ipc_handle, int owner_device, void** dev_ptr);
int softrod_exchange_close(int device, void* dev_ptr);
int softrod_exchange_free(int device, void* dev_ptr);

int softrod_observe(softrod_handle* h, const float* prev_action, float* obs,
                    void* stream);

int softrod_rod_energies(softrod_handle* h, double* out, void* stream);

int softrod_ground_reaction(softrod_handle* h, double* out, void* stream);

int softrod_rod_strains(softrod_handle* h, double* out, void* stream);

int softrod_muscle_loads(softrod_handle* h, double* out, void* stream);

int softrod_joint_loads(softrod_handle* h, double* out, void* stream);

int softrod_rod_dynamics(softrod_handle* h, double* out, void* stream);

int softrod_set_env_material(softrod_handle* h, const double* material, const uint8_t* mask, void* stream);

int softrod_set_env_contact(softrod_handle* h, const double* contact, const uint8_t* mask, void* stream);

int softrod_copy_envs(softrod_handle* h, const int32_t* src, const int32_t* dst, int count, void* stream);

int softrod_bank_create(softrod_handle* h, int slots);

int softrod_bank_save(softrod_handle* h, const int32_t* envs, const int32_t* slots, int count, void* stream);

int softrod_bank_load(softrod_handle* h, const int32_t* slots, const int32_t* envs, int count, void* stream);

int softrod_bank_info(softrod_handle* h, int32_t* slots, uint64_t* bytes_per_slot, uint8_t* filled);

typedef struct softrod_camera {
    uint32_t struct_size;
    int32_t width, height;
    int32_t follow;
    double center[3];
    double right[3];
    double up[3];
    double half_width;
    double target_radius;
    double light[3];
    double ambient;
} softrod_camera;
#define SOFTROD_RENDER_PALETTE                                                                             \
    { 0x1F77B4u, 0xFF7F0Eu, 0x2CA02Cu, 0xD62728u, 0x9467BDu, 0x8C564Bu, 0xE377C2u, 0x17BECFu, 0x7F7F7Fu, 0xBCBD22u }
#define SOFTROD_RENDER_BACKGROUND 0xF5F5F5u
int softrod_camera_default(const softrod_config* cfg, softrod_camera* cam);
int softrod_camera_check(const softrod_camera* cam);
int softrod_render(softrod_handle* h, const softrod_camera* cam, uint8_t* rgb, float* depth, void* stream);

int softrod_rod_clearance(softrod_handle* h, int self_gap, double* out, void* stream);

int softrod_set_rod_shape(softrod_handle* h, const double* kappa, const double* sigma, const double* velocity,
                          const double* omega, const uint8_t* mask, void* stream);

int softrod_set_reset_shapes(softrod_handle* h, int count, const double* kappa, const double* sigma, const double* velocity,
                             const double* omega, uint64_t seed, void* stream);
int softrod_apply_reset_shapes(softrod_handle* h, const uint8_t* mask, void* stream);
int softrod_reset_shapes_view(softrod_handle* h, int32_t** index, int32_t** episode);
uint32_t softrod_reset_shape_index(uint64_t seed, uint32_t env, uint32_t episode, uint32_t count);

int softrod_substeps(softrod_handle* h, const float* actions, int n, void* stream);

int softrod_state_view_get(softrod_handle* h, softrod_state_view* out);

int softrod_set_timing(softrod_handle* h, int n_launches);
int softrod_kernel_times_ms(softrod_handle* h, float* out_ms, int cap, int* count);
int softrod_last_kernel_ms(softrod_handle* h, float* ms);

const char* softrod_kernel_tier(softrod_handle* h);

const char* softrod_last_error(softrod_handle* h);
int softrod_destroy(softrod_handle* h);
int softrod_abi_version(void);
const char* softrod_source_hash(void);

#ifdef __cplusplus
}
#endif
#endif
```

Baseline: 14.33 million.

## Add per-env planar certificates to skip the full 3D load and planarity proof in softpendulum

```diff
diff --git a/gym_softrobot_amd/_capi.py b/gym_softrobot_amd/_capi.py
--- a/gym_softrobot_amd/_capi.py
+++ b/gym_softrobot_amd/_capi.py
@@ -992,6 +992,8 @@
     "softrod_reset_shape_index": (C.c_uint32, [C.c_uint64, C.c_uint32, C.c_uint32, C.c_uint32]),
     "softrod_substeps": (C.c_int, [_VP, _VP, C.c_int, _VP]),
     "softrod_state_view_get": (C.c_int, [_VP, C.POINTER(SoftrodStateView)]),
+    "softrod_set_planar_certificates": (C.c_int, [_VP, C.c_int]),
+    "softrod_planar_certificates": (C.c_int, [_VP, _VP, _VP]),
     "softrod_set_timing": (C.c_int, [_VP, C.c_int]),
     "softrod_kernel_times_ms": (C.c_int, [_VP, _VP, C.c_int, C.POINTER(C.c_int)]),
     "softrod_last_kernel_ms": (C.c_int, [_VP, C.POINTER(C.c_float)]),
diff --git a/gym_softrobot_amd/backend.py b/gym_softrobot_amd/backend.py
--- a/gym_softrobot_amd/backend.py
+++ b/gym_softrobot_amd/backend.py
@@ -1,5 +1,6 @@
 from __future__ import annotations
 
+import contextlib
 import ctypes as C
 from typing import Dict, Optional, Tuple
 
@@ -518,12 +519,32 @@
 
     def prev_action_rows(self) -> torch.Tensor:
         if getattr(self, "_prev_rows", None) is None:
-            self._prev_rows = self.state()["prev_action"]
+            with self._views() as st:
+                self._prev_rows = st["prev_action"]
             if not self.is_octo and not self.is_mocto:
                 self._prev_rows = self._prev_rows[:, : self.action_dim]
         return self._prev_rows
 
+    def set_planar_certificates(self, on: bool) -> None:
+        check(self._lib.softrod_set_planar_certificates(self._h, int(bool(on))), self._h)
+        self._planar_cert_on = bool(on)
+
+    def planar_certificates(self) -> torch.Tensor:
+        out = torch.empty((self.n_envs,), dtype=torch.uint8, device=self.device)
+        check(self._lib.softrod_planar_certificates(self._h, C.c_void_p(out.data_ptr()), self._stream()), self._h)
+        return out
+
+    @contextlib.contextmanager
+    def _views(self):
+        was_on = getattr(self, "_planar_cert_on", True)
+        try:
+            yield self.state()
+        finally:
+            if was_on:
+                self.set_planar_certificates(True)
+
     def state(self) -> Dict[str, torch.Tensor]:
+        self._planar_cert_on = False
         v = SoftrodStateView()
         check(self._lib.softrod_state_view_get(self._h, C.byref(v)), self._h)
         n, s = self.n_envs, int(v.lane_stride)
@@ -585,9 +606,9 @@
         if getattr(self, "queue_depth", 0):
             raise _capi.SoftrodError("snapshot/restore of a handle with device-side auto-reset is not supported: "
                                      "the pending-reset flags and the staged queue are not part of the state view")
-        st = self.state()
-        torch.cuda.synchronize(self.device)
-        snap = {k: st[k].cpu().clone() for k in self._snapshot_keys()}
+        with self._views() as st:
+            torch.cuda.synchronize(self.device)
+            snap = {k: st[k].cpu().clone() for k in self._snapshot_keys()}
         if getattr(self, "_env_material", None) is not None:
             snap["env_material"] = torch.from_numpy(self._env_material.copy())
         if getattr(self, "_env_contact", None) is not None:
@@ -607,11 +628,12 @@
             raise ValueError("snapshot was taken under a different softrod_config / ABI version / table set "
                              "(dt, n_substeps, features, env_kind, material, radius profile, spline table, "
                              "action basis ...): refusing to load it")
-        st = self.state()
-        for k in self._snapshot_keys():
-            if tuple(snap[k].shape) != tuple(st[k].shape):
-                raise ValueError(f"snapshot field {k!r} has shape {tuple(snap[k].shape)}, expected {tuple(st[k].shape)}")
-            st[k].copy_(snap[k].to(self.device))
+        with self._views() as st:
+            for k in self._snapshot_keys():
+                if tuple(snap[k].shape) != tuple(st[k].shape):
+                    raise ValueError(f"snapshot field {k!r} has shape {tuple(snap[k].shape)}, expected {tuple(st[k].shape)}")
+            for k in self._snapshot_keys():
+                st[k].copy_(snap[k].to(self.device))
         if "env_material" in snap:
             self.set_env_material(snap["env_material"].numpy())
         elif getattr(self, "_env_material", None) is not None:
@@ -626,18 +648,17 @@
         torch.cuda.synchronize(self.device)
 
     def rod_snapshot(self, env_indices) -> Dict[str, np.ndarray]:
-        st = self.state()
         idx = torch.as_tensor(list(env_indices), dtype=torch.long, device=self.device)
         ne = int(self.cfg.n_elem)
-
-        def rows(name, width):
-            return st[name].index_select(1, idx)[:, :, :width].permute(1, 0, 2).cpu().numpy()
-
-        return {
-            "x": rows("position", ne + 1), "v": rows("velocity", ne + 1), "w": rows("omega", ne),
-            "Q": rows("director", ne).reshape(len(env_indices), 3, 3, ne),
-            "time": st["time"].index_select(0, idx).cpu().numpy(),
-        }
+        with self._views() as st:
+            def rows(name, width):
+                return st[name].index_select(1, idx)[:, :, :width].permute(1, 0, 2).cpu().numpy()
+
+            return {
+                "x": rows("position", ne + 1), "v": rows("velocity", ne + 1), "w": rows("omega", ne),
+                "Q": rows("director", ne).reshape(len(env_indices), 3, 3, ne),
+                "time": st["time"].index_select(0, idx).cpu().numpy(),
+            }
 
     def kernel_tier(self) -> str:
         return self._lib.softrod_kernel_tier(self._h).decode()
@@ -666,19 +687,19 @@
         }
 
     def state_numpy(self) -> Dict[str, np.ndarray]:
-        st = self.state()
         ne = int(self.cfg.n_elem)
-        torch.cuda.synchronize(self.device)
-        out = {
-            "x": st["position"][:, :, : ne + 1].permute(1, 0, 2).cpu().numpy(),
-            "v": st["velocity"][:, :, : ne + 1].permute(1, 0, 2).cpu().numpy(),
-            "w": st["omega"][:, :, :ne].permute(1, 0, 2).cpu().numpy(),
-            "tangents": st["tangents"][:, :, :ne].permute(1, 0, 2).cpu().numpy(),
-            "time": st["time"].cpu().numpy(),
-            "control": st["control"].permute(1, 0).cpu().numpy(),
-            "kappa": st["kappa"][:, :, : ne - 1].permute(1, 0, 2).cpu().numpy(),
-            "rest_kappa": st["rest_kappa"][:, :, : ne - 1].permute(1, 0, 2).cpu().numpy(),
-        }
-        q = st["director"][:, :, :ne].permute(1, 0, 2).cpu().numpy()
+        with self._views() as st:
+            torch.cuda.synchronize(self.device)
+            out = {
+                "x": st["position"][:, :, : ne + 1].permute(1, 0, 2).cpu().numpy(),
+                "v": st["velocity"][:, :, : ne + 1].permute(1, 0, 2).cpu().numpy(),
+                "w": st["omega"][:, :, :ne].permute(1, 0, 2).cpu().numpy(),
+                "tangents": st["tangents"][:, :, :ne].permute(1, 0, 2).cpu().numpy(),
+                "time": st["time"].cpu().numpy(),
+                "control": st["control"].permute(1, 0).cpu().numpy(),
+                "kappa": st["kappa"][:, :, : ne - 1].permute(1, 0, 2).cpu().numpy(),
+                "rest_kappa": st["rest_kappa"][:, :, : ne - 1].permute(1, 0, 2).cpu().numpy(),
+            }
+            q = st["director"][:, :, :ne].permute(1, 0, 2).cpu().numpy()
         out["Q"] = q.reshape(self.n_envs, 3, 3, ne)
         return out
diff --git a/gym_softrobot_amd/csrc/softrod_capi.hip b/gym_softrobot_amd/csrc/softrod_capi.hip
--- a/gym_softrobot_amd/csrc/softrod_capi.hip
+++ b/gym_softrobot_amd/csrc/softrod_capi.hip
@@ -123,6 +123,8 @@
     hipEvent_t ev_pairs = nullptr;
     std::vector<uint8_t> is_dst;
     StateBank bank;
+    bool cert_on = true;
+    bool cert_live = false;
     std::string err;
 };
 
@@ -325,6 +327,13 @@
     R.stat_am[0] = 0.5 * (R.stat_mu[0] + R.stat_mu[1]); R.stat_am[1] = 0.5 * (R.stat_mu[0] - R.stat_mu[1]);
 }
 
+int clear_planar_certs(softrod_handle* h, hipStream_t st, bool always = true) {
+    if (!h->S.planar_cert || !(always || h->cert_live)) return SOFTROD_OK;
+    SR_HIP(h, hipMemsetAsync(h->S.planar_cert, 0, (size_t)h->cfg.n_envs, st));
+    h->cert_live = false;
+    return SOFTROD_OK;
+}
+
 int launch_autoreset(softrod_handle* h, float* obs, double* reward, uint8_t* term, uint8_t* trunc, double* aux, int pack,
                      hipStream_t st) {
     const dim3 grid((unsigned)h->cfg.n_envs), block(kLanes * h->nw);
@@ -393,6 +402,7 @@
     bool windowed;
     unsigned needs, honours;
     StepKernel step; OctoKernel octo; WindowKernel window;
+    bool cert;
     int epb, waves;
     const char* label;
 };
@@ -412,6 +422,7 @@
 constexpr StepRow fast_row(const char* label) {
     StepRow r = compiled_row(F, E, EPL, TAPER, 1, 1, label);
     r.step = softrod_step_fast_kernel<F, E, EPL, TAPER>;
+    r.cert = (F & ~kFeatEnvMaterial) == SOFTROD_FEATURES_SOFTPENDULUM;
     return r;
 }
 template <unsigned F, int MAXW, int EPB>
@@ -631,6 +642,8 @@
     if (!c.row) return fail(h, SOFTROD_EINVAL, c.why);
     const StepChoice after = c.row->windowed ? select_step(h, 0) : StepChoice{nullptr, nullptr};
     if (c.row->windowed && !after.row) return fail(h, SOFTROD_EINVAL, after.why);
+    if (c.row->cert) h->cert_live = true;
+    else if (const int rc = clear_planar_certs(h, st, false)) return rc;
     auto launch = [&](const StepRow& r, int n, int epi, hipEvent_t t0, hipEvent_t t1) {
         const dim3 grid((unsigned)((h->cfg.n_envs + r.epb - 1) / r.epb)), block(kLanes * (r.waves ? r.waves : h->nw));
         if (r.window) launch_stamped(r.window, grid, block, st, t0, t1, h->P, h->S, actions, n, h->window_refresh);
@@ -660,6 +673,7 @@
 
 int upload_and_reset(softrod_handle* h, hipStream_t st, bool use_mask) {
     const size_t N = (size_t)h->cfg.n_envs;
+    if (const int rc = clear_planar_certs(h, st)) return rc;
     SR_HIP(h, hipMemcpyAsync(h->d_init, h->h_init, N * h->init_stride * sizeof(double), hipMemcpyHostToDevice, st));
     if (use_mask)
         SR_HIP(h, hipMemcpyAsync(h->d_mask, h->h_mask, N, hipMemcpyHostToDevice, st));
@@ -931,7 +945,8 @@
     add(h->env_mat.dev, 1, sizeof(EnvMaterial));
     add(h->env_contact.dev, 1, sizeof(EnvContact));
     add(h->d_rs_index, 1, sizeof(int)); add(h->d_rs_episode, 1, sizeof(int));
-    static_assert(kCopyMaxArrays >= 22, "copy_table adds up to 22 arrays");
+    add(S.planar_cert, 1, sizeof(uint8_t));
+    static_assert(kCopyMaxArrays >= 23, "copy_table adds up to 23 arrays");
     return T;
 }
 
@@ -1052,6 +1067,7 @@
     hipLaunchKernelGGL(softrod_bank_copy_kernel, dim3((unsigned)count), dim3(kCopyThreads), 0, st,
                        load ? twin : batch, load ? batch : twin, bank.d_pairs);
     SR_HIP(h, hipGetLastError());
+    if (load && h->S.planar_cert) h->cert_live = true;
     if (!load)
         for (int i = 0; i < count; ++i) bank.filled[slots[i]] = 1;
     return SOFTROD_OK;
@@ -1355,6 +1371,12 @@
     alloc(h->S.envmem, rowb);
     alloc(h->S.prev_action, N * (adim > 7 ? adim : 7) * sizeof(float));
     alloc(h->S.head, 20 * N * sizeof(double));
+    if (cfg->math_mode == SOFTROD_MATH_FAST && cfg->features == SOFTROD_FEATURES_SOFTPENDULUM &&
+        cfg->env_kind == SOFTROD_ENV_SOFTPENDULUM) {
+        alloc(h->S.planar_cert, N + 1);
+        const uint8_t on = 1;
+        if (h->S.planar_cert) upload(h->S.planar_cert + N, &on, 1);
+    }
     alloc(h->d_spline, (size_t)(SOFTROD_MAX_SPLINE_PIECES + 1 + SOFTROD_MAX_SPLINE_PIECES * 4 * 4) * sizeof(double));
     h->P.spline = h->d_spline;
     alloc(h->d_ticket, sizeof(unsigned));
@@ -2127,6 +2149,7 @@
     SR_HIP(h, hipEventRecord(h->ev_pairs, st));
     hipLaunchKernelGGL(softrod_copy_envs_kernel, dim3((unsigned)n), dim3(kCopyThreads), 0, st, copy_table(h), h->d_pairs);
     SR_HIP(h, hipGetLastError());
+    if (h->S.planar_cert) h->cert_live = true;
     return SOFTROD_OK;
 }
 
@@ -2313,6 +2336,7 @@
                           const double* omega, const uint8_t* mask, void* stream) {
     if (!h) return fail(h, SOFTROD_EINVAL, "set rod shape: null handle");
     SR_ON_DEVICE(h);
+    if (const int rc = clear_planar_certs(h, (hipStream_t)stream)) return rc;
     const RodLayout y = rod_layout(h);
     const RodShapeArgs args{kappa, sigma, velocity, omega, mask, nullptr};
     hipLaunchKernelGGL(by_epl(h, softrod_rod_shape_kernel<1>, softrod_rod_shape_kernel<2>), dim3((unsigned)(h->cfg.n_envs * y.rods)),
@@ -2386,6 +2410,7 @@
     if (!h) return fail(h, SOFTROD_EINVAL, "apply reset shapes: null handle");
     if (!h->rs_count) return fail(h, SOFTROD_EINVAL, "apply reset shapes: no pool is set (softrod_set_reset_shapes)");
     SR_ON_DEVICE(h);
+    if (const int rc = clear_planar_certs(h, (hipStream_t)stream)) return rc;
     return launch_reset_shapes(h, kPickMask, mask, nullptr, nullptr, nullptr, nullptr, 0, (hipStream_t)stream);
 }
 
@@ -2400,6 +2425,8 @@
 
 int softrod_state_view_get(softrod_handle* h, softrod_state_view* out) {
     if (!h || !out) return fail(h, SOFTROD_EINVAL, "null argument");
+    if (h->S.planar_cert && h->cert_on)
+        if (const int rc = softrod_set_planar_certificates(h, 0)) return rc;
     out->n_envs = h->cfg.n_envs;
     out->n_elem = h->cfg.n_elem;
     const RodLayout y = rod_layout(h);
@@ -2427,6 +2454,28 @@
     return SOFTROD_OK;
 }
 
+int softrod_set_planar_certificates(softrod_handle* h, int on) {
+    if (!h) return fail(h, SOFTROD_EINVAL, "set planar certificates: null handle");
+    if (!h->S.planar_cert) return SOFTROD_OK;
+    SR_ON_DEVICE(h);
+    SR_HIP(h, hipDeviceSynchronize());
+    std::vector<uint8_t> bytes((size_t)h->cfg.n_envs + 1, 0);
+    bytes.back() = on ? 1 : 0;
+    SR_HIP(h, hipMemcpy(h->S.planar_cert, bytes.data(), bytes.size(), hipMemcpyHostToDevice));
+    h->cert_live = false;
+    h->cert_on = on != 0;
+    return SOFTROD_OK;
+}
+
+int softrod_planar_certificates(softrod_handle* h, uint8_t* out, void* stream) {
+    if (!h || !out) return fail(h, SOFTROD_EINVAL, "planar certificates: null argument");
+    SR_ON_DEVICE(h);
+    const size_t N = (size_t)h->cfg.n_envs;
+    if (!h->S.planar_cert) SR_HIP(h, hipMemsetAsync(out, 0, N, (hipStream_t)stream));
+    else SR_HIP(h, hipMemcpyAsync(out, h->S.planar_cert, N, hipMemcpyDeviceToDevice, (hipStream_t)stream));
+    return SOFTROD_OK;
+}
+
 int softrod_set_timing(softrod_handle* h, int n_launches) {
     if (!h || n_launches < 0 || n_launches > (1 << 20)) return fail(h, SOFTROD_EINVAL, "bad argument");
     SR_ON_DEVICE(h);
diff --git a/gym_softrobot_amd/csrc/softrod_copy_envs.hpp b/gym_softrobot_amd/csrc/softrod_copy_envs.hpp
--- a/gym_softrobot_amd/csrc/softrod_copy_envs.hpp
+++ b/gym_softrobot_amd/csrc/softrod_copy_envs.hpp
@@ -31,13 +31,20 @@
                 const size_t off = (size_t)c * comp_stride + ((size_t)u << 4);
                 *reinterpret_cast<uint4*>(to + off) = *reinterpret_cast<const uint4*>(from + off);
             }
-        } else {
+        } else if ((A.row_bytes & 3u) == 0) {
             const unsigned per = A.row_bytes >> 2, total = A.comps * per;
             for (unsigned i = threadIdx.x; i < total; i += kCopyThreads) {
                 const unsigned c = i / per, u = i - c * per;
                 const size_t off = (size_t)c * comp_stride + ((size_t)u << 2);
                 *reinterpret_cast<unsigned*>(to + off) = *reinterpret_cast<const unsigned*>(from + off);
             }
+        } else {
+            const unsigned per = A.row_bytes, total = A.comps * per;
+            for (unsigned i = threadIdx.x; i < total; i += kCopyThreads) {
+                const unsigned c = i / per, u = i - c * per;
+                const size_t off = (size_t)c * comp_stride + (size_t)u;
+                to[off] = from[off];
+            }
         }
     }
 }
diff --git a/gym_softrobot_amd/csrc/softrod_fast.hpp b/gym_softrobot_amd/csrc/softrod_fast.hpp
--- a/gym_softrobot_amd/csrc/softrod_fast.hpp
+++ b/gym_softrobot_amd/csrc/softrod_fast.hpp
@@ -598,18 +598,34 @@
     SR_PHASE(0);
     constexpr bool kPlanarKernel = (F & ~kFeatEnvMaterial) == SOFTROD_FEATURES_SOFTPENDULUM;
     LaneN<EPL> L;
-    load_lane<EPL, F, !kPlanarKernel>(S, N, rod, lane, L);
-    SR_PHASE(1);
-    if (has<F>(P, SOFTROD_FEAT_LAPLACE_FILTER)) sanitize_unused_rates<EPL>(P, lane, L);
-    if (has<F>(P, SOFTROD_FEAT_PLANE_CONTACT_ANISO)) sanitize_unused_slots<EPL>(P, lane, L);
     BcTargets B;
-    load_bc(S, N, rod, B);
-    load_suckers<F>(P, S, N, rod, B);
     EnvAction A;
-    set_action_n<F, E, EPL>(P, S, N, rod, lane, actions, A, B, L);
-    if (epilogue) push_store_prev_com<F, E, EPL>(P, S, N, rod, lane, L, n_sub);
-    if (has<F>(P, SOFTROD_FEAT_SPLINE_MUSCLE_TORQUES)) muscle_load<EPL>(P, S, rod, actions != nullptr, A, L);
-    {
+    [[maybe_unused]] bool certified = false, cert_on = false, proof_ok = true, proof_nan = false;
+    [[maybe_unused]] double s2w = 1.0;
+    bool blown_up = false;
+    if constexpr (kPlanarKernel) {
+        unsigned cert = 0, on = 0;
+        if (S.planar_cert) { on = S.planar_cert[N]; cert = S.planar_cert[rod]; }
+        double bc_in_plane[3];
+        planar_load_state<EPL>(S, N, rod, lane, L, bc_in_plane);
+        set_action_n<F, E, EPL>(P, S, N, rod, lane, actions, A, B, L);
+        cert_on = __builtin_amdgcn_readfirstlane((int)on) != 0;
+        cert = cert_on ? (unsigned)__builtin_amdgcn_readfirstlane((int)cert) : 0u;
+        certified = cert != 0;
+        if (certified) s2w = cert == 1u ? 1.0 : -1.0;
+        else planar_prove<EPL>(P, S, N, rod, lane, L, bc_in_plane, s2w, proof_ok, proof_nan);
+        planar_constrain_state<EPL>(lane, bc_in_plane, L);
+        SR_PHASE(1);
+    } else {
+        load_lane<EPL, F>(S, N, rod, lane, L);
+        SR_PHASE(1);
+        if (has<F>(P, SOFTROD_FEAT_LAPLACE_FILTER)) sanitize_unused_rates<EPL>(P, lane, L);
+        if (has<F>(P, SOFTROD_FEAT_PLANE_CONTACT_ANISO)) sanitize_unused_slots<EPL>(P, lane, L);
+        load_bc(S, N, rod, B);
+        load_suckers<F>(P, S, N, rod, B);
+        set_action_n<F, E, EPL>(P, S, N, rod, lane, actions, A, B, L);
+        if (epilogue) push_store_prev_com<F, E, EPL>(P, S, N, rod, lane, L, n_sub);
+        if (has<F>(P, SOFTROD_FEAT_SPLINE_MUSCLE_TORQUES)) muscle_load<EPL>(P, S, rod, actions != nullptr, A, L);
         BcTargets B0 = B;
         if (has<F>(P, SOFTROD_FEAT_MOVING_BASE_BC)) {
             B0.vel[0] = __shfl(L.v[0][0], 0); B0.vel[1] = __shfl(L.v[0][1], 0); B0.vel[2] = __shfl(L.v[0][2], 0);
@@ -626,17 +642,17 @@
     RodParams Pk = P;
     if (!has<F>(P, SOFTROD_FEAT_ANALYTICAL_DAMPER)) Pk.damp_t = 1.0;
 
-    bool blown_up = false;
-    if (n_sub > 0 && epilogue && rod_has_nan<EPL>(P, lane, L)) {
+    if constexpr (kPlanarKernel) {
+        blown_up = n_sub > 0 && epilogue && __any(proof_nan || planar_has_nan<EPL>(P, lane, L));
+    } else if (n_sub > 0 && epilogue && rod_has_nan<EPL>(P, lane, L)) {
         blown_up = true;
-        if constexpr (!kPlanarKernel) {
-            poison_rod<EPL>(L);
-            time = clock_after(P, S, time, n_sub);
-        }
+        poison_rod<EPL>(L);
+        time = clock_after(P, S, time, n_sub);
     }
     if constexpr (kPlanarKernel) {
         PlanarN<EPL> Z;
-        if (n_sub > 0 && !blown_up && planar_from_lane<EPL>(P, B, lane, L, Z)) {
+        const bool planar = n_sub > 0 && !blown_up && !__any(!(planar_from_lane<EPL>(P, lane, L, s2w, Z) && proof_ok));
+        if (__builtin_expect(planar, 1)) {
             PlanarC<EPL> K;
             planar_build_const<EPL, kEnvMaterial<F>>(Pk, C, lane, K);
             const double ta = P.time_two_half_adds ? P.half_dt : P.dt;
@@ -681,7 +697,8 @@
             else
                 for (int s = 0; s < n_sub; ++s) time = (time + ta) + tb;
             SR_PHASE(3);
-            planar_store<EPL>(S, N, rod, lane, Z, !SOFTROD_PLANAR_EXEC_MASK || lane * EPL <= P.n_elem);
+            planar_store<EPL>(S, N, rod, lane, Z, !SOFTROD_PLANAR_EXEC_MASK || lane * EPL <= P.n_elem, !certified);
+            if (cert_on && !certified && lane == 0) S.planar_cert[rod] = Z.s2 > 0.0 ? 1 : 2;
 #pragma unroll
             for (int s = 0; s < EPL; ++s) {
 #pragma unroll
@@ -691,6 +708,7 @@
             }
             planar_to_lane<EPL>(Z, L);
         } else {
+            if (cert_on && lane == 0) S.planar_cert[rod] = 0;
             general_step_cold<F, E, EPL>(S.params, S.self, rod, lane, actions, n_sub, blown_up);
             __builtin_amdgcn_fence(__ATOMIC_ACQUIRE, "wavefront");
             load_lane<EPL, F>(S, N, rod, opaque_lane(lane), L);
diff --git a/gym_softrobot_amd/csrc/softrod_kernels.hpp b/gym_softrobot_amd/csrc/softrod_kernels.hpp
--- a/gym_softrobot_amd/csrc/softrod_kernels.hpp
+++ b/gym_softrobot_amd/csrc/softrod_kernels.hpp
@@ -119,6 +119,7 @@
     float* prev_kappa;
     const EnvMaterial* env_mat;
     const EnvContact* env_contact;
+    uint8_t* planar_cert;
 };
 
 __device__ __forceinline__ double from_next(double x) {
@@ -1804,6 +1805,7 @@
     if (lane == 0) {
         S.time[rod] = 0.0;
         if (S.needs_reset) S.needs_reset[rod] = 0;
+        if (S.planar_cert) S.planar_cert[rod] = 0;
         if (P.env_kind == SOFTROD_ENV_SOFTPENDULUM3D) {
 #pragma unroll
             for (int i = 0; i < 7; ++i) S.prev_action[7 * (size_t)rod + i] = 0.0f;
diff --git a/gym_softrobot_amd/csrc/softrod_planar.hpp b/gym_softrobot_amd/csrc/softrod_planar.hpp
--- a/gym_softrobot_amd/csrc/softrod_planar.hpp
+++ b/gym_softrobot_amd/csrc/softrod_planar.hpp
@@ -83,23 +83,116 @@
     return e;
 }
 
-template <int EPL>
-__device__ __forceinline__ bool planar_from_lane(const RodParams& P, const BcTargets& B, int lane,
-                                                 const LaneN<EPL>& L, PlanarN<EPL>& Z) {
+
+template <int EPL>
+__device__ __forceinline__ void planar_load_state(const StatePtrs& S, size_t N, int rod, int lane, LaneN<EPL>& L,
+                                                  double (&bc)[3]) {
+    constexpr size_t W = (size_t)kLanes * EPL;
+    const size_t base = (size_t)rod * W + (size_t)lane * EPL;
+    bc[0] = S.bc[(size_t)1 * N + rod];
+    bc[1] = S.bc[(size_t)(3 + 6) * N + rod];
+    bc[2] = S.bc[(size_t)(3 + 7) * N + rod];
+#pragma unroll
+    for (int s = 0; s < EPL; ++s) {
+#pragma unroll
+        for (int c = 0; c < 3; ++c) { L.x[s][c] = 0.0; L.v[s][c] = 0.0; L.w[s][c] = 0.0; L.t[s][c] = 0.0; L.kap[s][c] = 0.0; L.rk[s][c] = 0.0; }
+#pragma unroll
+        for (int c = 0; c < 9; ++c) L.Q[s][c] = 0.0;
+#pragma unroll
+        for (int c = 0; c < 2; ++c) {
+            L.x[s][c] = S.pos[c * N * W + base + s];
+            L.v[s][c] = S.vel[c * N * W + base + s];
+            L.Q[s][6 + c] = S.dir[(6 + c) * N * W + base + s];
+        }
+        L.w[s][1] = S.omg[1 * N * W + base + s];
+    }
+}
+template <int EPL>
+__device__ __forceinline__ void planar_constrain_state(int lane, const double (&bc)[3], LaneN<EPL>& L) {
+    const bool l0 = (lane == 0);
+    L.x[0][1] = l0 ? bc[0] : L.x[0][1];
+    L.v[0][1] = l0 ? 0.0 : L.v[0][1];
+    L.Q[0][6] = l0 ? bc[1] : L.Q[0][6];
+    L.Q[0][7] = l0 ? bc[2] : L.Q[0][7];
+}
+
+template <int EPL>
+__device__ __forceinline__ bool planar_has_nan(const RodParams& P, int lane, const LaneN<EPL>& L) {
+    bool bad = false;
+#pragma unroll
+    for (int s = 0; s < EPL; ++s) {
+        const int idx = lane * EPL + s;
+        const bool b = isnan(L.x[s][0]) || isnan(L.x[s][1]) || isnan(L.v[s][0]) || isnan(L.v[s][1]);
+        const bool q = isnan(L.w[s][1]) || isnan(L.Q[s][6]) || isnan(L.Q[s][7]);
+        bad = bad || (idx <= P.n_elem && b) || (idx < P.n_elem && q);
+    }
+    return bad;
+}
+
+template <int EPL>
+__device__ __forceinline__ void planar_prove(const RodParams& P, const StatePtrs& S, size_t N, int rod, int lane,
+                                             const LaneN<EPL>& L, const double (&bc)[3], double& s2_out, bool& ok_out,
+                                             bool& nan_out) {
+    constexpr size_t W = (size_t)kLanes * EPL;
+    const size_t base = (size_t)rod * W + (size_t)lane * EPL;
     const int n = P.n_elem;
-    bool ok = (P.gravity[2] == 0.0) && (B.pos[2] == 0.0) && (B.Q[2] == 0.0) && (B.Q[8] == 0.0);
-    Z.s2 = __shfl((L.Q[0][5] < 0.0) ? -1.0 : 1.0, 0);
+    const bool l0 = (lane == 0);
+    const double bpz = S.bc[(size_t)2 * N + rod];
+    double bq[9];
+#pragma unroll
+    for (int i = 0; i < 9; ++i) bq[i] = (i < 3 || i == 8) ? S.bc[(size_t)(3 + i) * N + rod] : 0.0;
+    double xz[EPL], vz[EPL], w0[EPL], w2[EPL], Q[EPL][9];
+#pragma unroll
+    for (int s = 0; s < EPL; ++s) {
+        xz[s] = S.pos[2 * N * W + base + s];
+        vz[s] = S.vel[2 * N * W + base + s];
+        w0[s] = S.omg[0 * N * W + base + s];
+        w2[s] = S.omg[2 * N * W + base + s];
+#pragma unroll
+        for (int c = 0; c < 9; ++c) Q[s][c] = (c == 6 || c == 7) ? L.Q[s][c] : S.dir[c * N * W + base + s];
+    }
+    xz[0] = l0 ? bpz : xz[0];
+    vz[0] = l0 ? 0.0 : vz[0];
+    w0[0] = l0 ? 0.0 : w0[0];
+    w2[0] = l0 ? 0.0 : w2[0];
+#pragma unroll
+    for (int j = 0; j < 3; ++j) Q[0][j] = l0 ? bq[j] : Q[0][j];
+    Q[0][6] = l0 ? bc[1] : Q[0][6];
+    Q[0][7] = l0 ? bc[2] : Q[0][7];
+    Q[0][8] = l0 ? bq[8] : Q[0][8];
+    bool ok = (P.gravity[2] == 0.0) && (bpz == 0.0) && (bq[2] == 0.0) && (bq[8] == 0.0);
+    const double s2w = __shfl((Q[0][5] < 0.0) ? -1.0 : 1.0, 0);
+    bool bad = false;
 #pragma unroll
     for (int s = 0; s < EPL; ++s) {
         const int idx = lane * EPL + s;
-        const double* Q = L.Q[s];
-        const double s2 = (Q[5] < 0.0) ? -1.0 : 1.0, c = Q[6], sn = Q[7];
-        const bool node_ok = (L.x[s][2] == 0.0) && (L.v[s][2] == 0.0);
-        const bool elem_ok = (Q[2] == 0.0) && (Q[3] == 0.0) && (Q[4] == 0.0) && (Q[8] == 0.0) && (s2 == Z.s2) &&
-                             (fabs(fabs(Q[5]) - 1.0) <= 1.0e-12) && (L.w[s][0] == 0.0) && (L.w[s][2] == 0.0) &&
-                             (fabs(fma(s2, sn, Q[0])) <= 1.0e-12) && (fabs(fma(-s2, c, Q[1])) <= 1.0e-12) &&
-                             (fabs(fma(c, c, fma(sn, sn, -1.0))) <= 1.0e-12);
+        const double s2 = (Q[s][5] < 0.0) ? -1.0 : 1.0, c = Q[s][6], sn = Q[s][7];
+        const bool node_ok = (xz[s] == 0.0) && (vz[s] == 0.0);
+        const bool elem_ok = (Q[s][2] == 0.0) && (Q[s][3] == 0.0) && (Q[s][4] == 0.0) && (Q[s][8] == 0.0) && (s2 == s2w) &&
+                             (fabs(fabs(Q[s][5]) - 1.0) <= 1.0e-12) && (w0[s] == 0.0) && (w2[s] == 0.0) &&
+                             (fabs(fma(s2, sn, Q[s][0])) <= 1.0e-12) && (fabs(fma(-s2, c, Q[s][1])) <= 1.0e-12);
         ok = ok && (idx > n || node_ok) && (idx >= n || elem_ok);
+        bool q = isnan(w0[s]) || isnan(w2[s]);
+#pragma unroll
+        for (int k = 0; k < 9; ++k) q = q || (k != 6 && k != 7 && isnan(Q[s][k]));
+        bad = bad || (idx <= n && (isnan(xz[s]) || isnan(vz[s]))) || (idx < n && q);
+    }
+    s2_out = s2w;
+    ok_out = ok;
+    nan_out = bad;
+}
+
+template <int EPL>
+__device__ __forceinline__ bool planar_from_lane(const RodParams& P, int lane, const LaneN<EPL>& L, double s2w,
+                                                 PlanarN<EPL>& Z) {
+    const int n = P.n_elem;
+    bool ok = true;
+    Z.s2 = s2w;
+#pragma unroll
+    for (int s = 0; s < EPL; ++s) {
+        const int idx = lane * EPL + s;
+        const double c = L.Q[s][6], sn = L.Q[s][7];
+        ok = ok && (idx >= n || fabs(fma(c, c, fma(sn, sn, -1.0))) <= 1.0e-12);
         Z.x[s][0] = L.x[s][0]; Z.x[s][1] = L.x[s][1];
         Z.v[s][0] = L.v[s][0]; Z.v[s][1] = L.v[s][1];
         Z.c[s] = c; Z.s[s] = sn;
@@ -131,7 +224,7 @@
 #ifdef SOFTROD_DIAG_NO_PLANAR
     return false;
 #endif
-    return !__any(!ok);
+    return ok;
 }
 
 template <int EPL>
@@ -149,12 +242,15 @@
 
 template <int EPL>
 __device__ __forceinline__ void planar_store(const StatePtrs& S, size_t N, int rod, int lane, const PlanarN<EPL>& Z,
-                                             bool stepped) {
+                                             bool stepped, bool tan_z) {
     constexpr size_t W = (size_t)kLanes * EPL;
     const size_t base = (size_t)rod * W + (size_t)opaque_lane(lane) * EPL;
-#pragma unroll
-    for (int s = 0; s < EPL; ++s) {
-        S.tan[2 * N * W + base + s] = 0.0;
+    if (tan_z) {
+#pragma unroll
+        for (int s = 0; s < EPL; ++s) S.tan[2 * N * W + base + s] = 0.0;
+    }
+#pragma unroll
+    for (int s = 0; s < EPL; ++s) {
         S.dir[0 * N * W + base + s] = -Z.s2 * Z.s[s];
         S.dir[1 * N * W + base + s] = Z.s2 * Z.c[s];
         S.omg[1 * N * W + base + s] = Z.s2 * Z.wz[s];
diff --git a/gym_softrobot_amd/csrc/softrod_shape.hpp b/gym_softrobot_amd/csrc/softrod_shape.hpp
--- a/gym_softrobot_amd/csrc/softrod_shape.hpp
+++ b/gym_softrobot_amd/csrc/softrod_shape.hpp
@@ -51,6 +51,7 @@
     const int n = P.n_elem;
     const size_t NW = R.N * R.W;
     const size_t rod = A.pool_index ? (size_t)A.pool_index[R.env] * (size_t)rods + (size_t)R.arm : (size_t)R.rod;
+    if (lane == 0 && S.planar_cert) S.planar_cert[R.env] = 0;
 
     double M[EPL][9];
 #pragma unroll
diff --git a/gym_softrobot_amd/csrc/softrod_state_bank.hpp b/gym_softrobot_amd/csrc/softrod_state_bank.hpp
--- a/gym_softrobot_amd/csrc/softrod_state_bank.hpp
+++ b/gym_softrobot_amd/csrc/softrod_state_bank.hpp
@@ -23,7 +23,7 @@
                 *reinterpret_cast<uint4*>(to + (size_t)c * to_stride + in) =
                     *reinterpret_cast<const uint4*>(from + (size_t)c * from_stride + in);
             }
-        } else {
+        } else if ((A.row_bytes & 3u) == 0) {
             const unsigned per = A.row_bytes >> 2, total = A.comps * per;
             for (unsigned i = threadIdx.x; i < total; i += kCopyThreads) {
                 const unsigned c = i / per, u = i - c * per;
@@ -31,6 +31,12 @@
                 *reinterpret_cast<unsigned*>(to + (size_t)c * to_stride + in) =
                     *reinterpret_cast<const unsigned*>(from + (size_t)c * from_stride + in);
             }
+        } else {
+            const unsigned per = A.row_bytes, total = A.comps * per;
+            for (unsigned i = threadIdx.x; i < total; i += kCopyThreads) {
+                const unsigned c = i / per, u = i - c * per;
+                to[(size_t)c * to_stride + u] = from[(size_t)c * from_stride + u];
+            }
         }
     }
 }
diff --git a/gym_softrobot_amd/envs/base.py b/gym_softrobot_amd/envs/base.py
--- a/gym_softrobot_amd/envs/base.py
+++ b/gym_softrobot_amd/envs/base.py
@@ -494,7 +494,12 @@
         obs, reward, term, trunc = self.backend.step(a)
         self._top_up_tick()
         if getattr(self, "_dev_time", None) is None:
-            self._dev_time = self.backend.state()["time"]
+            views = getattr(self.backend, "_views", None)
+            if views is None:
+                self._dev_time = self.backend.state()["time"]
+            else:
+                with views() as st:
+                    self._dev_time = st["time"]
         tl = self.backend.time_limit() if getattr(self.cfg, "early_termination", 0) else trunc.view(torch.bool)
         infos = {"time": self._out(self._dev_time), "TimeLimit.truncated": self._out(tl)}
         if self.same_step:
diff --git a/include/softrod.h b/include/softrod.h
--- a/include/softrod.h
+++ b/include/softrod.h
@@ -315,6 +315,9 @@
 
 int softrod_state_view_get(softrod_handle* h, softrod_state_view* out);
 
+int softrod_set_planar_certificates(softrod_handle* h, int on);
+int softrod_planar_certificates(softrod_handle* h, uint8_t* out, void* stream);
+
 int softrod_set_timing(softrod_handle* h, int n_launches);
 int softrod_kernel_times_ms(softrod_handle* h, float* out_ms, int cap, int* count);
 int softrod_last_kernel_ms(softrod_handle* h, float* ms);
```

After: 14.51 million, median of 6. No clear change (+1.2%).
